# brown-palm/goal-force

Measured on AMD Instinct MI355X. Metric: frames_per_sec (81-frame video / (50-step denoise loop + VAE decode), Wan2.2-I2V-A14B 832x480x81f), higher is better.
Workload: dtype bf16

## Files before the change

### goal_force_amd/csrc/gf_cross_fold.hip

```cpp
#include "gf_common.h"

namespace {

constexpr int CF_HD = 128;
constexpr int CF_MAXK = 64;
constexpr int CF_THREADS = 256;
constexpr int CF_QB = 128;

__device__ __forceinline__ void cf_mfma32(f32x16& acc, const bf16x8& a, const bf16x8& b) {
    acc = __builtin_amdgcn_mfma_f32_32x32x16_bf16(a, b, acc, 0, 0, 0);
}

__global__ __launch_bounds__(CF_THREADS) void cross_probs_kernel(const u16* __restrict__ q, const u16* __restrict__ k, u16* __restrict__ pout,
                                                                 int q_len, int n_keys, int n_pad, int heads, long q_stride, long k_stride,
                                                                 long p_stride, float c, float last_key_bias) {
    __shared__ __attribute__((aligned(16))) char lds[CF_MAXK * 256];
    const int tid = threadIdx.x;
    const int lane = tid & 63, wave = tid >> 6;
    const int r = lane & 31, h = lane >> 5;
    const int head = blockIdx.y;
    const int q0 = blockIdx.x * CF_QB + wave * 32;
    const int halves = n_keys > 32 ? 2 : 1;

#pragma unroll
    for (int i = 0; i < (CF_MAXK * 16) / CF_THREADS; ++i) {
        const int idx = tid + CF_THREADS * i;
        const int row = idx >> 4, ch = idx & 15;
        u16x8 v8 = {0, 0, 0, 0, 0, 0, 0, 0};
        if (row < n_keys) v8 = *reinterpret_cast<const u16x8*>(k + (long)row * k_stride + head * CF_HD + ch * 8);
        const int sk = ((row & 3) << 2) | ((row >> 2) & 3);
        *(u16x8*)(lds + row * 256 + ((ch ^ sk) << 4)) = v8;
    }

    bf16x8 qf[8];
    {
        const int qr = min(q0 + r, q_len - 1);
        const u16* qp = q + (long)qr * q_stride + head * CF_HD + 8 * h;
#pragma unroll
        for (int kd = 0; kd < 8; ++kd) qf[kd] = *reinterpret_cast<const bf16x8*>(qp + 16 * kd);
    }
    __syncthreads();

    f32x16 sc[2];
#pragma unroll
    for (int e = 0; e < 16; ++e) {
        sc[0][e] = 0.f;
        sc[1][e] = 0.f;
    }
    const int sK = ((r & 3) << 2) | ((r >> 2) & 3);
#pragma unroll
    for (int kd = 0; kd < 8; ++kd) {
        const int off = 256 * r + 16 * ((2 * kd + h) ^ sK);
        cf_mfma32(sc[0], *(const bf16x8*)(lds + off), qf[kd]);
        if (halves == 2) cf_mfma32(sc[1], *(const bf16x8*)(lds + off + 32 * 256), qf[kd]);
    }

#pragma unroll
    for (int e = 0; e < 16; ++e) {
        const int key = 4 * h + (e & 3) + 8 * (e >> 2);
        if (key >= n_keys) sc[0][e] = -INFINITY;
        if (key + 32 >= n_keys) sc[1][e] = -INFINITY;
        if (key == n_keys - 1) sc[0][e] += last_key_bias;
        if (key + 32 == n_keys - 1) sc[1][e] += last_key_bias;
    }
    float mx = sc[0][0];
#pragma unroll
    for (int e = 1; e < 16; ++e) mx = fmaxf(mx, sc[0][e]);
#pragma unroll
    for (int e = 0; e < 16; ++e) mx = fmaxf(mx, sc[1][e]);
    mx = fmaxf(mx, __shfl_xor(mx, 32));
    const float mc = mx * c;
    float rs = 0.f;
#pragma unroll
    for (int e = 0; e < 16; ++e) {
        sc[0][e] = __builtin_amdgcn_exp2f(__builtin_fmaf(sc[0][e], c, -mc));
        sc[1][e] = __builtin_amdgcn_exp2f(__builtin_fmaf(sc[1][e], c, -mc));
        rs += sc[0][e] + sc[1][e];
    }
    const float l_tot = rs + __shfl_xor(rs, 32);
    const float inv = 1.0f / l_tot;
    float pl = 0.f;
#pragma unroll
    for (int e = 0; e < 16; ++e) {
        const int key = 4 * h + (e & 3) + 8 * (e >> 2);
        if (key == n_keys - 1) pl = sc[0][e];
        if (key + 32 == n_keys - 1) pl = sc[1][e];
    }
    pl += __shfl_xor(pl, 32);
    const float wl = pl * inv;
    const float wl_lo = wl - bf2f(f2bf(wl));

    const int qrow = q0 + r;
    if (qrow < q_len) {
        u16* prow = pout + (long)qrow * p_stride + (long)head * n_pad;
#pragma unroll
        for (int half = 0; half < 2; ++half)
#pragma unroll
            for (int g = 0; g < 4; ++g) {
                const int key = 32 * half + 8 * g + 4 * h;
                if (key < n_pad) {
                    float w4[4];
#pragma unroll
                    for (int i = 0; i < 4; ++i) w4[i] = key + i == n_keys ? wl_lo : sc[half][4 * g + i] * inv;
                    u32x2 pk;
                    pk[0] = pack2bf(w4[0], w4[1]);
                    pk[1] = pack2bf(w4[2], w4[3]);
                    *reinterpret_cast<u32x2*>(prow + key) = pk;
                }
            }
    }
}

constexpr int CFT_ROWS = 64;
__global__ __launch_bounds__(CF_THREADS) void cross_fold_table_kernel(const u16* __restrict__ v, const u16* __restrict__ w, u16* __restrict__ u,
                                                                      int n_keys, int n_pad, int n_out, long v_stride, long w_stride,
                                                                      long u_stride) {
    __shared__ __attribute__((aligned(16))) u16 vs[CF_MAXK * CF_HD];
    const int tid = threadIdx.x;
    const int head = blockIdx.y;
    for (int idx = tid; idx < n_pad * 16; idx += CF_THREADS) {
        const int row = idx >> 4, ch = idx & 15;
        u16x8 v8 = {0, 0, 0, 0, 0, 0, 0, 0};
        if (row <= n_keys) v8 = *reinterpret_cast<const u16x8*>(v + (long)min(row, n_keys - 1) * v_stride + head * CF_HD + ch * 8);
        *reinterpret_cast<u16x8*>(vs + row * CF_HD + ch * 8) = v8;
    }
    __syncthreads();
    const int n = blockIdx.x * CFT_ROWS + (tid >> 2), jg = tid & 3;
    if (n >= n_out) return;
    const int nj = n_pad >> 2;
    float acc[CF_MAXK / 4];
#pragma unroll
    for (int i = 0; i < CF_MAXK / 4; ++i) acc[i] = 0.f;
    const u16* wr = w + (long)n * w_stride + head * CF_HD;
    for (int d0 = 0; d0 < CF_HD; d0 += 8) {
        const u16x8 w8 = *reinterpret_cast<const u16x8*>(wr + d0);
        float wf[8];
#pragma unroll
        for (int e = 0; e < 8; ++e) wf[e] = bf2f(w8[e]);
#pragma unroll
        for (int i = 0; i < CF_MAXK / 4; ++i) {
            if (i < nj) {
                const u16x8 v8 = *reinterpret_cast<const u16x8*>(vs + (jg + 4 * i) * CF_HD + d0);
#pragma unroll
                for (int e = 0; e < 8; ++e) acc[i] = __builtin_fmaf(bf2f(v8[e]), wf[e], acc[i]);
            }
        }
    }
    u16* ur = u + (long)n * u_stride + (long)head * n_pad;
#pragma unroll
    for (int i = 0; i < CF_MAXK / 4; ++i) {
        const int j = jg + 4 * i;
        if (i < nj) ur[j] = j <= n_keys ? f2bf(acc[i]) : (u16)0;
    }
}

}

extern "C" GF_API int gf_cross_probs(const void* q, const void* k, void* p, int64_t q_len, int64_t n_keys, int64_t n_pad, int64_t heads,
                                     int64_t head_dim, int64_t q_stride, int64_t k_stride, int64_t p_stride, float scale,
                                     float last_key_multiplicity, void* stream) {
    GF_CHECK_ARG(q && k && p, "gf_cross_probs: null pointer");
    if (head_dim != CF_HD) {
        gf_set_error("gf_cross_probs: head_dim=%ld unsupported (kernel is built for 128)", (long)head_dim);
        return GF_ERR_UNSUPPORTED;
    }
    GF_CHECK_ARG(q_len >= 0 && q_len < (1 << 30) && heads > 0 && heads < 65536, "gf_cross_probs: bad sizes q=%ld heads=%ld", (long)q_len,
                 (long)heads);
    GF_CHECK_ARG(n_keys >= 1 && n_pad % 16 == 0 && n_pad > n_keys && n_pad <= CF_MAXK,
                 "gf_cross_probs: 1 <= n_keys=%ld < n_pad=%ld <= 64, n_pad a multiple of 16", (long)n_keys, (long)n_pad);
    GF_CHECK_ARG(q_stride % 8 == 0 && k_stride % 8 == 0 && p_stride % 4 == 0 && q_stride >= heads * CF_HD && k_stride >= heads * CF_HD &&
                     p_stride >= heads * n_pad,
                 "gf_cross_probs: strides must cover the rows (q, k: multiples of 8; p: of 4, >= heads * n_pad)");
    GF_CHECK_ARG(gf_aligned16(q) && gf_aligned16(k) && ((uintptr_t)p & 7u) == 0, "gf_cross_probs: alignment (q, k 16 bytes, p 8 bytes)");
    GF_CHECK_ARG(scale > 0.f && last_key_multiplicity >= 1.0f, "gf_cross_probs: scale > 0, multiplicity >= 1");
    if (q_len == 0) return GF_OK;
    const float c = scale * 1.4426950408889634f;
    const float bias = last_key_multiplicity != 1.0f ? log2f(last_key_multiplicity) / c : 0.f;
    const dim3 grid((unsigned)((q_len + CF_QB - 1) / CF_QB), (unsigned)heads);
    hipLaunchKernelGGL(cross_probs_kernel, grid, dim3(CF_THREADS), 0, (hipStream_t)stream, (const u16*)q, (const u16*)k, (u16*)p,
                       (int)q_len, (int)n_keys, (int)n_pad, (int)heads, (long)q_stride, (long)k_stride, (long)p_stride, c, bias);
    GF_CHECK_LAUNCH("gf_cross_probs");
    return GF_OK;
}

extern "C" GF_API int gf_cross_fold_table(const void* v, const void* w_o, void* u, int64_t n_keys, int64_t n_pad, int64_t heads,
                                          int64_t head_dim, int64_t n_out, int64_t v_stride, int64_t w_stride, int64_t u_stride,
                                          void* stream) {
    GF_CHECK_ARG(v && w_o && u, "gf_cross_fold_table: null pointer");
    if (head_dim != CF_HD) {
        gf_set_error("gf_cross_fold_table: head_dim=%ld unsupported (kernel is built for 128)", (long)head_dim);
        return GF_ERR_UNSUPPORTED;
    }
    GF_CHECK_ARG(heads > 0 && heads < 65536 && n_out > 0 && n_out < (1 << 30), "gf_cross_fold_table: bad sizes heads=%ld N=%ld", (long)heads,
                 (long)n_out);
    GF_CHECK_ARG(n_keys >= 1 && n_pad % 16 == 0 && n_pad > n_keys && n_pad <= CF_MAXK,
                 "gf_cross_fold_table: 1 <= n_keys=%ld < n_pad=%ld <= 64, n_pad a multiple of 16", (long)n_keys, (long)n_pad);
    GF_CHECK_ARG(v_stride % 8 == 0 && w_stride % 8 == 0 && v_stride >= heads * CF_HD && w_stride >= heads * CF_HD && u_stride >= heads * n_pad,
                 "gf_cross_fold_table: strides must cover the rows (v, w_o: multiples of 8; u >= heads * n_pad)");
    GF_CHECK_ARG(gf_aligned16(v) && gf_aligned16(w_o) && ((uintptr_t)u & 1u) == 0, "gf_cross_fold_table: alignment");
    const dim3 grid((unsigned)((n_out + CFT_ROWS - 1) / CFT_ROWS), (unsigned)heads);
    hipLaunchKernelGGL(cross_fold_table_kernel, grid, dim3(CF_THREADS), 0, (hipStream_t)stream, (const u16*)v, (const u16*)w_o, (u16*)u,
                       (int)n_keys, (int)n_pad, (int)n_out, (long)v_stride, (long)w_stride, (long)u_stride);
    GF_CHECK_LAUNCH("gf_cross_fold_table");
    return GF_OK;
}
```

### goal_force_amd/csrc/gf_gemm.hip

```cpp
#include "gf_mfma_frame.h"
#include <cstdlib>


namespace {

constexpr int BM = 256, BN = 256, BK = 64;
constexpr int GEMM_THREADS = 512;
constexpr int TILE_BYTES = BM * BK * 2;
constexpr int STAGE_BYTES = 2 * TILE_BYTES;
constexpr int GEMM_LDS = 2 * STAGE_BYTES;
constexpr int GROUP_M = 8;

struct ConvGeom {
    const u16* src;
    const u16* cache;
    const u16* zero;
    int H, W, C, Ho, Wo, kt, ks, mode, t_stride, t_off, taps;
    int hist_front;
    int c64;
    long frame;
    float inv_c, inv_ks2;
};

struct GemmArgs {
    const u16* A;
    const u16* W;
    const u16* bias;
    u16* C;
    const u16* R;
    const u16* gate;
    const float* row_scale;
    int M, N, K;
    long lda, ldw, ldc, ldr;
    long sA = 0, sW = 0, sC = 0;
    int tiles_m, tiles_n;
    unsigned long long* rsv0 = nullptr;
    ConvGeom cv;
    int rsv1 = 0;
    int stagger;
    int wrows;
    int stagger_rows;
    int group_m;
    int rsv2 = 0;
};

constexpr int GF_EPI_VT32 = 6;

typedef __attribute__((ext_vector_type(8))) int i32x8;

template <int EPI>
__device__ __forceinline__ float gf_epi_act(float lin) {
    if constexpr (EPI == GF_EPI_BIAS_GELU_TANH) return gelu_tanh_f(rbf(lin));
    else if constexpr (EPI == GF_EPI_BIAS_SILU) {
        const float y = rbf(lin);
        return y / (1.0f + expf(-y));
    } else return lin;
}

template <int EPI, bool FP8>
__global__ __launch_bounds__(GEMM_THREADS, 2) void gemm_kernel(const GemmArgs p) {
    static_assert(FP8, "only the fp8 form of this kernel ships (launch_gemm); bf16 with M < 512 runs gemm_ph_kernel");
    extern __shared__ __attribute__((aligned(16))) char smem[];
    GF_LDS char* lds = (GF_LDS char*)smem;

    const int tid = threadIdx.x;
    const int lane = tid & 63;
    const int wave = __builtin_amdgcn_readfirstlane(tid >> 6);

    const int v = gf_xcd_tile_order(p.tiles_m * p.tiles_n);
    const int per_group = GROUP_M * p.tiles_n;
    const int group = v / per_group;
    const int first_m = group * GROUP_M;
    const int gsz = min(p.tiles_m - first_m, GROUP_M);
    const int in_group = v - group * per_group;
    const int tile_m = first_m + in_group % gsz;
    const int tile_n = in_group / gsz;
    const int m0 = tile_m * BM, n0 = tile_n * BN;

    const int srow = lane >> 3;
    const int schunk = (lane & 7) ^ srow;
    const char* a_src[4];
    const char* b_src[4];
#pragma unroll
    for (int i = 0; i < 4; ++i) {
        const int row = (wave * 4 + i) * 8 + srow;
        const int am = min(m0 + row, p.M - 1);
        const int bn = min(n0 + row, p.N - 1);
        a_src[i] = (const char*)p.A + (long)am * p.lda + schunk * 16;
        b_src[i] = (const char*)p.W + (long)bn * p.ldw + schunk * 16;
    }
    auto stage = [&](int buf, int kt) {
        GF_LDS char* sa = lds + buf * STAGE_BYTES + wave * 4096;
        GF_LDS char* sb = sa + TILE_BYTES;
        const int koff = kt * 128;
#pragma unroll
        for (int i = 0; i < 4; ++i) {
            glds16(a_src[i] + koff, sa + i * 1024);
            glds16(b_src[i] + koff, sb + i * 1024);
        }
    };

    const int wm = wave >> 2, wn = wave & 3;
    const int frow = lane & 15;
    const int fq = lane >> 4;
    const int sw = frow & 7;
    const int a_base = (wm * 128 + frow) * 128;
    const int b_base = TILE_BYTES + (wn * 64 + frow) * 128;

    f32x4 acc[8][4];
#pragma unroll
    for (int i = 0; i < 8; ++i)
#pragma unroll
        for (int j = 0; j < 4; ++j) acc[i][j] = f32x4{0.f, 0.f, 0.f, 0.f};

    const int nk = p.K / 128;
    stage(0, 0);
    for (int kt = 0; kt < nk; ++kt) {
        asm volatile("s_waitcnt vmcnt(0)" ::: "memory");
        __syncthreads();
        if (kt + 1 < nk) stage((kt + 1) & 1, kt + 1);
        GF_LDS char* sbuf = lds + (kt & 1) * STAGE_BYTES;
        const int c0 = ((2 * fq) ^ sw) << 4, c1 = ((2 * fq + 1) ^ sw) << 4;
        i32x8 bfr[4];
#pragma unroll
        for (int j = 0; j < 4; ++j) {
            const u32x4 lo = *(GF_LDS u32x4*)(sbuf + b_base + j * 2048 + c0);
            const u32x4 hi = *(GF_LDS u32x4*)(sbuf + b_base + j * 2048 + c1);
            bfr[j] = i32x8{(int)lo[0], (int)lo[1], (int)lo[2], (int)lo[3], (int)hi[0], (int)hi[1], (int)hi[2], (int)hi[3]};
        }
#pragma unroll
        for (int i = 0; i < 8; ++i) {
            const u32x4 lo = *(GF_LDS u32x4*)(sbuf + a_base + i * 2048 + c0);
            const u32x4 hi = *(GF_LDS u32x4*)(sbuf + a_base + i * 2048 + c1);
            const i32x8 af = i32x8{(int)lo[0], (int)lo[1], (int)lo[2], (int)lo[3], (int)hi[0], (int)hi[1], (int)hi[2], (int)hi[3]};
#pragma unroll
            for (int j = 0; j < 4; ++j)
                acc[i][j] = __builtin_amdgcn_mfma_scale_f32_16x16x128_f8f6f4(bfr[j], af, acc[i][j], 0, 0, 0, 0x7F7F7F7F, 0, 0x7F7F7F7F);
        }
    }

    __syncthreads();
    GF_LDS char* ep = lds + wave * 16384;
    {
        const int nb = n0 + wn * 64 + fq * 4;
#pragma unroll
        for (int j = 0; j < 4; ++j) {
            float bv[4] = {0.f, 0.f, 0.f, 0.f};
            const int n = nb + j * 16;
            if (p.bias && n < p.N) {
                const u16x4 b4 = *reinterpret_cast<const u16x4*>(p.bias + n);
#pragma unroll
                for (int r = 0; r < 4; ++r) bv[r] = bf2f(b4[r]);
            }
#pragma unroll
            for (int i = 0; i < 8; ++i) {
                float y[4];
                const float rs = p.row_scale[min(m0 + wm * 128 + i * 16 + frow, p.M - 1)];
#pragma unroll
                for (int r = 0; r < 4; ++r) y[r] = gf_epi_act<EPI>(acc[i][j][r] * rs + bv[r]);
                u32x2 pk;
                pk[0] = pack2bf(y[0], y[1]);
                pk[1] = pack2bf(y[2], y[3]);
                const int row = i * 16 + frow;
                const int slot = (j * 4 + fq) ^ ((row & 7) << 1);
                *(GF_LDS u32x2*)(ep + row * 128 + slot * 8) = pk;
            }
        }
    }
    asm volatile("s_waitcnt lgkmcnt(0)" ::: "memory");
    {
        const int rr = lane >> 3, cc = lane & 7;
        const int n = n0 + wn * 64 + cc * 8;
        const bool n_ok = n < p.N;
        u16x8 g8;
        if (EPI == GF_EPI_BIAS_GATE_RESID && n_ok) g8 = *reinterpret_cast<const u16x8*>(p.gate + n);
#pragma unroll 4
        for (int it = 0; it < 16; ++it) {
            const int row = it * 8 + rr;
            const int m = m0 + wm * 128 + row;
            const u16x8 yv = *(GF_LDS u16x8*)(ep + row * 128 + ((cc ^ (row & 7)) << 4));
            if (m < p.M && n_ok) {
                u16x8 o = yv;
                if (EPI == GF_EPI_BIAS_GATE_RESID || EPI == GF_EPI_BIAS_RESID || EPI == GF_EPI_BIAS_MUL) {
                    const u16x8 r8 = *reinterpret_cast<const u16x8*>(p.R + (long)m * p.ldr + n);
#pragma unroll
                    for (int e = 0; e < 8; ++e) {
                        float t = bf2f(yv[e]);
                        if (EPI == GF_EPI_BIAS_GATE_RESID) t = rbf(bf2f(g8[e]) * t);
                        o[e] = (EPI == GF_EPI_BIAS_MUL) ? f2bf(t * bf2f(r8[e]))
                                                        : f2bf(bf2f(r8[e]) + t);
                    }
                }
                *reinterpret_cast<u16x8*>(p.C + (long)m * p.ldc + n) = o;
            }
        }
    }
}

template <int EPI, bool FP8, int CONV = 0, int NB = 2>
__global__ __launch_bounds__(GEMM_THREADS, 2) void gemm_ph_kernel(const GemmArgs p) {
    static_assert(!(CONV && FP8), "the implicit-GEMM convolution is bf16 only");
    static_assert(NB == 2 || ((NB == 1 || NB == 3) && !FP8), "NB = 1 and 3 are built for bf16");
    constexpr bool WIDE = NB >= 2;
    constexpr int NBH = WIDE ? 2 : 1;
    constexpr int J1 = NB == 3 ? 1 : 2;
    constexpr int BNT = NB == 3 ? 192 : NB * 128;
    constexpr int ESZ = FP8 ? 1 : 2;
    constexpr int BKE = 128 / ESZ;
    constexpr int HALF_BYTES = 128 * 128;
    extern __shared__ __attribute__((aligned(16))) char smem[];
    GF_LDS char* lds = (GF_LDS char*)smem;

    const u16* const pA = p.A + (long)blockIdx.y * p.sA;
    const u16* const pW = p.W + (long)blockIdx.y * p.sW;
    u16* const pC = p.C + (long)blockIdx.y * p.sC;
    const int tid = threadIdx.x;
    const int lane = tid & 63;
    const int wave = __builtin_amdgcn_readfirstlane(tid >> 6);
    const int wr = wave >> 2, wc = wave & 3;

    const int v = gf_xcd_tile_order(p.tiles_m * p.tiles_n);
    const int per_group = GROUP_M * p.tiles_n;
    const int group = v / per_group;
    const int first_m = group * GROUP_M;
    const int gsz = min(p.tiles_m - first_m, GROUP_M);
    const int in_group = v - group * per_group;
    const int m0 = (first_m + in_group % gsz) * BM, n0 = (in_group / gsz) * BNT;

    const int srow = lane >> 3;
    const int schunk = (lane & 7) ^ srow;
    const char* srcp[4][2];
#pragma unroll
    for (int i = 0; i < 2; ++i) {
        const int row = (wave * 2 + i) * 8 + srow;
        const long a0 = min(m0 + row, p.M - 1), a1 = min(m0 + 128 + row, p.M - 1);
        const long b0 = min(n0 + row, p.N - 1), b1 = min(n0 + 128 + row, p.N - 1);
        srcp[0][i] = (const char*)pA + (a0 * p.lda) * ESZ + schunk * 16;
        srcp[3][i] = (const char*)pA + (a1 * p.lda) * ESZ + schunk * 16;
        srcp[1][i] = (const char*)pW + (b0 * p.ldw) * ESZ + schunk * 16;
        srcp[2][i] = (const char*)pW + (b1 * p.ldw) * ESZ + schunk * 16;
    }
    const char* srcp_b1h = (const char*)pW + (min((long)(n0 + 128 + wave * 8 + srow), (long)p.N - 1) * p.ldw) * ESZ + schunk * 16;
    int cyx[2][2], cf[2][2];
    const u16* rowp[2][2];
    int rmask[2][2];
    if constexpr (CONV != 0) {
#pragma unroll
        for (int a = 0; a < 2; ++a)
#pragma unroll
            for (int i = 0; i < 2; ++i) {
                const int m = min(m0 + a * 128 + (wave * 2 + i) * 8 + srow, p.M - 1);
                const int X = m % p.cv.Wo, t = m / p.cv.Wo;
                const int Y = t % p.cv.Ho, j = t / p.cv.Ho;
                const int f0 = p.cv.t_off + j * p.cv.t_stride - (p.cv.kt - 1);
                if constexpr (CONV == 2) {
                    rowp[a][i] = p.cv.src + ((long)f0 * p.cv.frame + ((long)Y * p.cv.W + X) * p.cv.C);
                    rmask[a][i] = 16 | (Y == 0 ? 1 : 0) | (Y == p.cv.H - 1 ? 2 : 0) | (X == 0 ? 4 : 0) | (X == p.cv.W - 1 ? 8 : 0);
                } else {
                    cyx[a][i] = (Y << 16) | X;
                    cf[a][i] = f0;
                }
            }
    }
    int s_c0[2] = {0, 0}, s_dt[2] = {0, 0}, s_dy[2] = {0, 0}, s_dx[2] = {0, 0};
    if constexpr (CONV == 2) {
        if (p.cv.c64) {
#pragma unroll
            for (int a = 0; a < 2; ++a)
#pragma unroll
                for (int i = 0; i < 2; ++i) rowp[a][i] += schunk * 8;
        }
    }
    const int nk = p.K / BKE;
    auto region = [](int kind) { return kind == 0 ? 0 : (kind == 3 ? HALF_BYTES : (kind == 1 ? 2 * HALF_BYTES : 3 * HALF_BYTES)); };
    auto stage = [&](int tile, int kind) {
        GF_LDS char* dst = lds + (tile & 1) * STAGE_BYTES + region(kind) + wave * 2048;
        if constexpr (CONV != 0) {
            if (kind == 0 || kind == 3) {
                const ConvGeom& g = p.cv;
                const int a = kind == 3;
                if constexpr (CONV == 2) {
                    if (g.c64) {
                        const int hf = g.ks >> 1;
                        const long toff = (long)s_dt[a] * g.frame + (long)(((s_dy[a] - hf) * g.W + (s_dx[a] - hf)) * g.C + s_c0[a]);
                        int need = 0;
                        if (g.ks == 3) need = (s_dy[a] == 0 ? 1 : 0) | (s_dy[a] == 2 ? 2 : 0) | (s_dx[a] == 0 ? 4 : 0) | (s_dx[a] == 2 ? 8 : 0);
#pragma unroll
                        for (int i = 0; i < 2; ++i) glds16((need & rmask[a][i]) ? g.zero : rowp[a][i] + toff, dst + i * 1024);
                        s_c0[a] += 64;
                        if (s_c0[a] == g.C) {
                            s_c0[a] = 0;
                            if (++s_dx[a] == g.ks) {
                                s_dx[a] = 0;
                                if (++s_dy[a] == g.ks) {
                                    s_dy[a] = 0;
                                    ++s_dt[a];
                                }
                            }
                        }
                        return;
                    }
                }
                const int ke = tile * 64 + schunk * 8;
                const int tap = (int)(((float)ke + 0.5f) * g.inv_c);
                const int c = ke - tap * g.C;
                const int dt = (int)(((float)tap + 0.5f) * g.inv_ks2);
                const int rem = tap - dt * g.ks * g.ks;
                int dy = 0, dx = 0;
                if (g.ks == 3) {
                    dy = (rem * 11) >> 5;
                    dx = rem - 3 * dy;
                }
                const int half = g.ks >> 1;
                if constexpr (CONV == 2) {
                    const long toff = (long)dt * g.frame + (long)(((dy - half) * g.W + (dx - half)) * g.C + c);
                    int need = tap < g.taps ? 0 : 16;
                    if (g.ks == 3) need |= (dy == 0 ? 1 : 0) | (dy == 2 ? 2 : 0) | (dx == 0 ? 4 : 0) | (dx == 2 ? 8 : 0);
#pragma unroll
                    for (int i = 0; i < 2; ++i) glds16((need & rmask[a][i]) ? g.zero : rowp[a][i] + toff, dst + i * 1024);
                    return;
                }
#pragma unroll
                for (int i = 0; i < 2; ++i) {
                    const int Y = cyx[a][i] >> 16, X = cyx[a][i] & 0xffff;
                    int sy, sx;
                    bool ok;
                    if (g.mode == 2) {
                        sy = 2 * Y + dy;
                        sx = 2 * X + dx;
                        ok = sy < g.H && sx < g.W;
                    } else {
                        const int yy = Y + dy - half, xx = X + dx - half;
                        ok = yy >= 0 && yy < g.Ho && xx >= 0 && xx < g.Wo;
                        sy = g.mode == 1 ? (yy >> 1) : yy;
                        sx = g.mode == 1 ? (xx >> 1) : xx;
                    }
                    const int f = cf[a][i] + dt;
                    const u16* base = (f >= 0 || g.hist_front) ? g.src + (long)f * g.frame : g.cache + (long)(2 + f) * g.frame;
                    const u16* src = (ok && tap < g.taps) ? base + ((long)sy * g.W + sx) * g.C + c : g.zero;
                    glds16(src, dst + i * 1024);
                }
                return;
            }
        }
        const long koff = (long)tile * 128;
        if constexpr (NB == 3) {
            if (kind == 2) {
                glds16(srcp_b1h + koff, lds + (tile & 1) * STAGE_BYTES + region(2) + wave * 1024);
                return;
            }
        }
        glds16(srcp[kind][0] + koff, dst);
        glds16(srcp[kind][1] + koff, dst + 1024);
    };

    const int frow = lane & 15, fq = lane >> 4, sw = frow & 7;
    const int a_off = (wr * 64 + frow) * 128;
    const int b_off = (wc * 32 + frow) * 128;
    const int b_off1 = NB == 3 ? (wc * 16 + frow) * 128 : b_off;
    int chb[4];
    if constexpr (!FP8) {
        chb[0] = ((0 + fq) ^ sw) << 4;
        chb[1] = ((4 + fq) ^ sw) << 4;
        chb[2] = chb[3] = 0;
    } else {
        chb[0] = ((2 * fq) ^ sw) << 4;
        chb[1] = ((2 * fq + 1) ^ sw) << 4;
        chb[2] = chb[3] = 0;
    }
    typedef u32x4 frag_t[2];
    frag_t afr[4], bfr[2][2];
    auto read_a = [&](GF_LDS char* buf, int a) {
#pragma unroll
        for (int i = 0; i < 4; ++i) {
            afr[i][0] = *(GF_LDS u32x4*)(buf + region(a ? 3 : 0) + a_off + i * 2048 + chb[0]);
            afr[i][1] = *(GF_LDS u32x4*)(buf + region(a ? 3 : 0) + a_off + i * 2048 + chb[1]);
        }
    };
    auto read_b = [&](GF_LDS char* buf, int b) {
#pragma unroll
        for (int j = 0; j < 2; ++j) {
            if (b && j >= J1) continue;
            bfr[b][j][0] = *(GF_LDS u32x4*)(buf + region(b ? 2 : 1) + (b ? b_off1 : b_off) + j * 2048 + chb[0]);
            bfr[b][j][1] = *(GF_LDS u32x4*)(buf + region(b ? 2 : 1) + (b ? b_off1 : b_off) + j * 2048 + chb[1]);
        }
    };

    f32x4 acc[2][NBH][4][2];
#pragma unroll
    for (int a = 0; a < 2; ++a)
#pragma unroll
        for (int b = 0; b < NBH; ++b)
#pragma unroll
            for (int i = 0; i < 4; ++i)
#pragma unroll
                for (int j = 0; j < 2; ++j) acc[a][b][i][j] = f32x4{0.f, 0.f, 0.f, 0.f};

    auto mma = [&](int a, int b) {
        __builtin_amdgcn_s_setprio(1);
#pragma unroll
        for (int i = 0; i < 4; ++i)
#pragma unroll
            for (int j = 0; j < 2; ++j) {
                if (b && j >= J1) continue;
                if constexpr (!FP8) {
#pragma unroll
                    for (int ks = 0; ks < 2; ++ks)
                        acc[a][b][i][j] = __builtin_amdgcn_mfma_f32_16x16x32_bf16(
                            __builtin_bit_cast(bf16x8, bfr[b][j][ks]), __builtin_bit_cast(bf16x8, afr[i][ks]),
                            acc[a][b][i][j], 0, 0, 0);
                } else {
                    const i32x8 bw = i32x8{(int)bfr[b][j][0][0], (int)bfr[b][j][0][1], (int)bfr[b][j][0][2], (int)bfr[b][j][0][3],
                                           (int)bfr[b][j][1][0], (int)bfr[b][j][1][1], (int)bfr[b][j][1][2], (int)bfr[b][j][1][3]};
                    const i32x8 aw = i32x8{(int)afr[i][0][0], (int)afr[i][0][1], (int)afr[i][0][2], (int)afr[i][0][3],
                                           (int)afr[i][1][0], (int)afr[i][1][1], (int)afr[i][1][2], (int)afr[i][1][3]};
                    acc[a][b][i][j] = __builtin_amdgcn_mfma_scale_f32_16x16x128_f8f6f4(bw, aw, acc[a][b][i][j], 0, 0, 0,
                                                                                         0x7F7F7F7F, 0, 0x7F7F7F7F);
                }
            }
        __builtin_amdgcn_s_setprio(0);
    };

    const int total = (WIDE ? 4 : 3) * nk;
    if constexpr (WIDE) {
        stage(0, 0);
        stage(0, 1);
        stage(0, 2);
        stage(0, 3);
        if (nk > 1) {
            stage(1, 0);
            stage(1, 1);
            if constexpr (NB == 3) asm volatile("s_waitcnt vmcnt(7)" ::: "memory");
            else asm volatile("s_waitcnt vmcnt(8)" ::: "memory");
        } else {
            asm volatile("s_waitcnt vmcnt(0)" ::: "memory");
        }
        __builtin_amdgcn_s_barrier();
    } else {
        stage(0, 0);
        stage(0, 1);
        stage(0, 3);
        if (nk > 1) {
            stage(1, 0);
            stage(1, 1);
            asm volatile("s_waitcnt vmcnt(6)" ::: "memory");
        } else {
            asm volatile("s_waitcnt vmcnt(0)" ::: "memory");
        }
        __builtin_amdgcn_s_barrier();
    }
    if (wr == 1) __builtin_amdgcn_s_barrier();

#define GF_PHASE_END(SEQ_ISSUED)                                                  \
    if ((SEQ_ISSUED) >= total) asm volatile("s_waitcnt vmcnt(0)" ::: "memory");  \
    else if constexpr (NB == 3) asm volatile("s_waitcnt vmcnt(7)" ::: "memory"); \
    else if constexpr (NB == 2) asm volatile("s_waitcnt vmcnt(8)" ::: "memory"); \
    else asm volatile("s_waitcnt vmcnt(6)" ::: "memory");                        \
    asm volatile("s_waitcnt lgkmcnt(0)" ::: "memory");                           \
    __builtin_amdgcn_sched_barrier(0);                                           \
    __builtin_amdgcn_s_barrier();

#define GF_AFTER_MMA                       \
    __builtin_amdgcn_sched_barrier(0);     \
    __builtin_amdgcn_s_barrier();
    if constexpr (NB == 1) {
        for (int c = 0; c < nk; ++c) {
            GF_LDS char* buf = lds + (c & 1) * STAGE_BYTES;
            const int g = 3 * c;
            if (g + 5 < total) stage(c + 1, 3);
            read_b(buf, 0);
            read_a(buf, 0);
            GF_PHASE_END(g + 5)
            mma(0, 0);
            GF_AFTER_MMA
            if (g + 6 < total) {
                stage(c + 2, 0);
                stage(c + 2, 1);
            }
            read_a(buf, 1);
            GF_PHASE_END(g + 7)
            mma(1, 0);
            GF_AFTER_MMA
        }
    } else
    for (int c = 0; c < nk; ++c) {
        GF_LDS char* buf = lds + (c & 1) * STAGE_BYTES;
        const int g = 4 * c;
        if (g + 6 < total) stage(c + 1, 2);
        read_b(buf, 0);
        read_a(buf, 0);
        GF_PHASE_END(g + 6)
        mma(0, 0);
        GF_AFTER_MMA
        if (g + 7 < total) stage(c + 1, 3);
        read_b(buf, 1);
        GF_PHASE_END(g + 7)
        mma(0, 1);
        GF_AFTER_MMA
        if (g + 8 < total) stage(c + 2, 0);
        read_a(buf, 1);
        GF_PHASE_END(g + 8)
        mma(1, 1);
        GF_AFTER_MMA
        if (g + 9 < total) stage(c + 2, 1);
        GF_PHASE_END(g + 9)
        mma(1, 0);
        GF_AFTER_MMA
    }
#undef GF_AFTER_MMA
#undef GF_PHASE_END
    if (wr == 0) __builtin_amdgcn_s_barrier();

    constexpr bool HAS_R = EPI == GF_EPI_BIAS_GATE_RESID || EPI == GF_EPI_BIAS_RESID || EPI == GF_EPI_BIAS_MUL;
    u16x8 rpre[HAS_R ? 16 : 1];
    if constexpr (HAS_R) {
        const int cc = lane & 31, n = n0 + cc * 8;
        const bool n_ok = n < p.N && cc * 8 < BNT;
#pragma unroll
        for (int it = 0; it < 16; ++it) {
            const int m = m0 + wave * 32 + it * 2 + (lane >> 5);
            rpre[it] = u16x8{0, 0, 0, 0, 0, 0, 0, 0};
            if (m < p.M && n_ok) rpre[it] = *reinterpret_cast<const u16x8*>(p.R + (long)m * p.ldr + n);
        }
    }

#pragma unroll
    for (int b = 0; b < NBH; ++b)
#pragma unroll
        for (int j = 0; j < 2; ++j) {
            if (b && j >= J1) continue;
            const int ncol = (NB == 3 && b) ? 128 + wc * 16 + fq * 4 : b * 128 + wc * 32 + j * 16 + fq * 4;
            float bv[4] = {0.f, 0.f, 0.f, 0.f};
            if (p.bias && n0 + ncol < p.N) {
                const u16x4 b4 = *reinterpret_cast<const u16x4*>(p.bias + n0 + ncol);
#pragma unroll
                for (int r = 0; r < 4; ++r) bv[r] = bf2f(b4[r]);
            }
#pragma unroll
            for (int a = 0; a < 2; ++a)
#pragma unroll
                for (int i = 0; i < 4; ++i) {
                    const int row = a * 128 + wr * 64 + i * 16 + frow;
                    float rs = 1.0f;
                    if constexpr (FP8) rs = p.row_scale[min(m0 + row, p.M - 1)];
                    float y[4];
#pragma unroll
                    for (int r = 0; r < 4; ++r) {
                        y[r] = gf_epi_act<EPI>(acc[a][b][i][j][r] * rs + bv[r]);
                    }
                    u32x2 pk;
                    pk[0] = pack2bf(y[0], y[1]);
                    pk[1] = pack2bf(y[2], y[3]);
                    const int slot = (ncol >> 2) ^ ((row & 15) << 1);
                    *(GF_LDS u32x2*)(lds + row * 512 + slot * 8) = pk;
                }
        }
    __syncthreads();
    {
        const int cc = lane & 31;
        const int n = n0 + cc * 8;
        const bool n_ok = n < p.N && cc * 8 < BNT;
        u16x8 g8;
        if (EPI == GF_EPI_BIAS_GATE_RESID && n_ok) g8 = *reinterpret_cast<const u16x8*>(p.gate + n);
#pragma unroll
        for (int it = 0; it < 16; ++it) {
            const int row = wave * 32 + it * 2 + (lane >> 5);
            const int m = m0 + row;
            const u16x8 yv = *(GF_LDS u16x8*)(lds + row * 512 + ((cc ^ (row & 15)) << 4));
            if (m < p.M && n_ok) {
                u16x8 o = yv;
                if (EPI == GF_EPI_BIAS_GATE_RESID || EPI == GF_EPI_BIAS_RESID || EPI == GF_EPI_BIAS_MUL) {
                    const u16x8 r8 = rpre[HAS_R ? it : 0];
#pragma unroll
                    for (int e = 0; e < 8; ++e) {
                        float t = bf2f(yv[e]);
                        if (EPI == GF_EPI_BIAS_GATE_RESID) t = rbf(bf2f(g8[e]) * t);
                        o[e] = (EPI == GF_EPI_BIAS_MUL) ? f2bf(t * bf2f(r8[e]))
                                                        : f2bf(bf2f(r8[e]) + t);
                    }
                }
                *reinterpret_cast<u16x8*>(pC + (long)m * p.ldc + n) = o;
            }
        }
    }
}

#include "gf_gemm_a4_loop.inc"
#include "gf_gemm_a4f8_loop.inc"
constexpr int A4_THREADS = 256;

template <int EPI, bool FP8 = false>
__global__ __launch_bounds__(A4_THREADS, 1) void gemm_a4_kernel(const GemmArgs p) {
    constexpr unsigned ESZ = FP8 ? 1u : 2u;
    extern __shared__ __attribute__((aligned(16))) char smem[];
    GF_LDS char* lds = (GF_LDS char*)smem;
    const int tid = threadIdx.x;
    const int lane = tid & 63;
    const int wave = __builtin_amdgcn_readfirstlane(tid >> 6);
    const int wm = wave >> 1, wn = wave & 1;

    const int v = gf_xcd_tile_order(p.tiles_m * p.tiles_n);
    const int gm = p.group_m;
    const int per_group = gm * p.tiles_n;
    const int group = v / per_group;
    const int first_m = group * gm;
    const int gsz = min(p.tiles_m - first_m, gm);
    const int in_group = v - group * per_group;
    const int m0 = (first_m + in_group % gsz) * BM, n0 = (in_group / gsz) * BN;

    unsigned voffA = gf_a4_voff<ESZ>(lane, (unsigned)p.lda), voffB = gf_a4_voff<ESZ>(lane, (unsigned)p.ldw);
    unsigned pfA = (unsigned)lane * (unsigned)p.lda * ESZ, pfB = (unsigned)lane * (unsigned)p.ldw * ESZ;
    const unsigned long baseA = (unsigned long)((const char*)p.A + (long)m0 * p.lda * ESZ);
    const unsigned long baseB = (unsigned long)((const char*)p.W + (long)n0 * p.ldw * ESZ);
    const unsigned aLo = (unsigned)baseA, aHi = (unsigned)(baseA >> 32) & 0xffffu;
    const unsigned bLo = (unsigned)baseB, bHi = (unsigned)(baseB >> 32) & 0xffffu;
    const unsigned nrA = (unsigned)(((long)(min(p.M - m0, BM) - 1) * p.lda + p.K) * ESZ);
    const int wvalid = min(p.wrows - n0, BN);
    const unsigned nrB = wvalid > 0 ? (unsigned)(((long)(wvalid - 1) * p.ldw + p.K) * ESZ) : 0u;
    const unsigned stA = 32u * (unsigned)p.lda * ESZ, stB = 32u * (unsigned)p.ldw * ESZ;
    const unsigned soA = (unsigned)wave * 8u * (unsigned)p.lda * ESZ, soB = (unsigned)wave * 8u * (unsigned)p.ldw * ESZ;
    const unsigned ldsW = (unsigned)(unsigned long)lds + (unsigned)wave * 1024u;
    const unsigned nk = (unsigned)(p.K * (int)ESZ / 128);
    const unsigned k0 = p.stagger ? (unsigned)((p.stagger * (p.stagger_rows ? m0 / BM : n0 / BN)) % (int)nk) : 0u;
    const unsigned kb = (unsigned)p.K * ESZ;

    const int frow = lane & 15, fq = lane >> 4, sw = frow & 7;
    const unsigned lbase = (unsigned)(unsigned long)lds;
    unsigned rdA0 = lbase + (unsigned)((wm * 128 + frow) * 128 + (((0 + fq) ^ sw) << 4));
    unsigned rdA1 = lbase + (unsigned)((wm * 128 + frow) * 128 + (((4 + fq) ^ sw) << 4));
    unsigned rdB0 = lbase + (unsigned)(TILE_BYTES + (wn * 128 + frow) * 128 + (((0 + fq) ^ sw) << 4));
    unsigned rdB1 = lbase + (unsigned)(TILE_BYTES + (wn * 128 + frow) * 128 + (((4 + fq) ^ sw) << 4));

    u16x4 bpre[8];
    u16x8 gpre = {0, 0, 0, 0, 0, 0, 0, 0};
    {
        const int fq_ = lane >> 4;
#pragma unroll
        for (int j = 0; j < 8; ++j) {
            const int n = n0 + wn * 128 + j * 16 + fq_ * 4;
            bpre[j] = (EPI != GF_EPI_VT32 && p.bias && n < p.N) ? *reinterpret_cast<const u16x4*>(p.bias + n) : u16x4{0, 0, 0, 0};
        }
        const int ng = n0 + wn * 128 + (lane & 15) * 8;
        if (EPI == GF_EPI_BIAS_GATE_RESID && ng < p.N) gpre = *reinterpret_cast<const u16x8*>(p.gate + ng);
        if (EPI == GF_EPI_VT32 && p.bias) {
#pragma unroll
            for (int i = 0; i < 8; ++i) {
                const int mrow = m0 + wm * 128 + i * 16 + (lane & 15);
                if (mrow < p.M) bpre[i][0] = p.bias[mrow];
            }
        }
    }
    float rsc[FP8 ? 8 : 1];
    if constexpr (FP8 && EPI != GF_EPI_VT32) {
#pragma unroll
        for (int i = 0; i < 8; ++i) rsc[i] = p.row_scale[min(m0 + wm * 128 + i * 16 + (lane & 15), p.M - 1)];
    }
    if constexpr (FP8) {
        GF_A4F8_LOOP_ASM(voffA, voffB, rdA0, rdA1, rdB0, rdB1, aLo, aHi, nrA, bLo, bHi, nrB, soA, stA, soB, stB, ldsW, nk, k0, kb);
    } else
    {
        GF_A4_LOOP_ASM(voffA, voffB, pfA, pfB, rdA0, rdA1, rdB0, rdB1, aLo, aHi, nrA, bLo, bHi, nrB, soA, stA, soB, stB, ldsW, nk, k0, kb);
    }

    GF_LDS char* ep = lds + wave * 32768;
    constexpr bool HAS_R = EPI == GF_EPI_BIAS_GATE_RESID || EPI == GF_EPI_BIAS_RESID || EPI == GF_EPI_BIAS_MUL;
    u16x8 rres[HAS_R ? 32 : 1];
    if constexpr (HAS_R) {
        const int nr = n0 + wn * 128 + (lane & 15) * 8;
#pragma unroll
        for (int it = 0; it < 32; ++it) {
            const int mr = m0 + wm * 128 + it * 4 + (lane >> 4);
            if (mr < p.M && nr < p.N) {
                rres[it] = __builtin_nontemporal_load(reinterpret_cast<const u16x8*>(p.R + (long)mr * p.ldr + nr));
            } else {
                rres[it] = u16x8{0, 0, 0, 0, 0, 0, 0, 0};
            }
        }
    }
    f32x4 csc[(FP8 && EPI == GF_EPI_VT32) ? 8 : 1];
    if constexpr (FP8 && EPI == GF_EPI_VT32) {
#pragma unroll
        for (int j = 0; j < 8; ++j) {
            const int n = n0 + wn * 128 + j * 16 + fq * 4;
#pragma unroll
            for (int r = 0; r < 4; ++r) csc[j][r] = (n + r < p.wrows) ? p.row_scale[n + r] : 0.f;
        }
    }
    gf_static_for<0, 8>([&](auto j_c) {
        constexpr int j = decltype(j_c)::value;
        const int n = n0 + wn * 128 + j * 16 + fq * 4;
        const float bv[4] = {bf2f(bpre[j][0]), bf2f(bpre[j][1]), bf2f(bpre[j][2]), bf2f(bpre[j][3])};
        gf_static_for<0, 8>([&](auto i_c) {
            constexpr int i = decltype(i_c)::value;
            constexpr int A0 = (i * 8 + j) * 4;
            float y[4] = {gf_agpr_read<A0>(), gf_agpr_read<A0 + 1>(), gf_agpr_read<A0 + 2>(), gf_agpr_read<A0 + 3>()};
            if constexpr (FP8 && EPI != GF_EPI_VT32) {
#pragma unroll
                for (int r = 0; r < 4; ++r) y[r] = y[r] * rsc[i] + bv[r];
            }
            if constexpr (EPI == GF_EPI_VT32) {
                const float bm = bf2f(bpre[i][0]);
                if constexpr (FP8) {
#pragma unroll
                    for (int r = 0; r < 4; ++r) y[r] = (n + r < p.wrows) ? y[r] * csc[j][r] + bm : 0.f;
                } else {
#pragma unroll
                    for (int r = 0; r < 4; ++r) y[r] = (n + r < p.wrows) ? y[r] + bm : 0.f;
                }
            } else if constexpr (EPI == GF_EPI_BIAS_GELU_TANH) {
                const unsigned l01 = FP8 ? pack2bf(y[0], y[1]) : pack2bf(y[0] + bv[0], y[1] + bv[1]);
                const unsigned l23 = FP8 ? pack2bf(y[2], y[3]) : pack2bf(y[2] + bv[2], y[3] + bv[3]);
                gf_f32x2 g01 = {__uint_as_float(l01 << 16), __uint_as_float(l01 & 0xffff0000u)};
                gf_f32x2 g23 = {__uint_as_float(l23 << 16), __uint_as_float(l23 & 0xffff0000u)};
                gelu_tanh_f4(g01, g23);
                y[0] = g01[0];
                y[1] = g01[1];
                y[2] = g23[0];
                y[3] = g23[1];
            } else {
#pragma unroll
                for (int r = 0; r < 4; ++r) {
                    y[r] = gf_epi_act<EPI>(FP8 ? y[r] : y[r] + bv[r]);
                }
            }
            u32x2 pk;
            pk[0] = pack2bf(y[0], y[1]);
            pk[1] = pack2bf(y[2], y[3]);
            const int row = i * 16 + frow;
            const int slot = (j * 4 + fq) ^ ((row & 15) << 1);
            *(GF_LDS u32x2*)(ep + row * 256 + slot * 8) = pk;
        });
    });
    asm volatile("s_waitcnt lgkmcnt(0)" ::: "memory");
    {
        const int cc = lane & 15;
        const int n = n0 + wn * 128 + cc * 8;
        const bool n_ok = n < p.N;
        const u16x8 g8 = gpre;
#pragma unroll
        for (int it = 0; it < 32; ++it) {
            const int row = it * 4 + (lane >> 4);
            const int m = m0 + wm * 128 + row;
            u16x8 yv;
            if constexpr (EPI == GF_EPI_VT32) {
                const int G = cc >> 2, g = cc & 3, sw = (row & 15) << 1;
                const u16x4 lo = *(GF_LDS u16x4*)(ep + row * 256 + (((8 * G + g) ^ sw) << 3));
                const u16x4 hi = *(GF_LDS u16x4*)(ep + row * 256 + (((8 * G + 4 + g) ^ sw) << 3));
                yv = u16x8{lo[0], lo[1], lo[2], lo[3], hi[0], hi[1], hi[2], hi[3]};
            } else {
                yv = *(GF_LDS u16x8*)(ep + row * 256 + ((cc ^ (row & 15)) << 4));
            }
            if (m < p.M && n_ok) {
                u16x8 o = yv;
                if constexpr (HAS_R) {
                    const u16x8 r8 = rres[it];
#pragma unroll
                    for (int e = 0; e < 8; ++e) {
                        float t = bf2f(yv[e]);
                        if (EPI == GF_EPI_BIAS_GATE_RESID) t = rbf(bf2f(g8[e]) * t);
                        o[e] = (EPI == GF_EPI_BIAS_MUL) ? f2bf(t * bf2f(r8[e]))
                                                        : f2bf(bf2f(r8[e]) + t);
                    }
                }
                __builtin_nontemporal_store(o, reinterpret_cast<u16x8*>(p.C + (long)m * p.ldc + n));
            }
        }
    }
}

template <int EPI, bool FP8 = false>
int launch_gemm_a4(const GemmArgs& a0, hipStream_t stream) {
    GemmArgs a = a0;
    {
        const int g = gf_options().a4_group_m.load(std::memory_order_relaxed);
        a.group_m = g > 0 ? g : (a.K * (FP8 ? 1 : 2) >= 16384 ? 4 : GROUP_M);
    }
    return gf_launch_lds<gemm_a4_kernel<EPI, FP8>>("gf_gemm", GF_ATTR_MSG_BYTES, FP8 ? "gf_gemm_fp8" : "gf_gemm_bf16", dim3((unsigned)(a.tiles_m * a.tiles_n)),
                                                   dim3(A4_THREADS), GEMM_LDS, stream, a);
}

template <int EPI, bool FP8>
int launch_gemm(const GemmArgs& a, hipStream_t stream) {
    const bool use_a4 = gf_options().prefer_8wave.load(std::memory_order_relaxed) == 0;
    if constexpr (!FP8) {
        if (use_a4 && a.M >= 512 && a.K % 64 == 0 && 256L * a.lda * 2 + a.K * 2L < (1L << 31) &&
            256L * a.ldw * 2 + a.K * 2L < (1L << 31))
            return launch_gemm_a4<EPI>(a, stream);
    } else {
        if (use_a4 && a.M >= 512 && a.K % 128 == 0 && 256L * a.lda + a.K < (1L << 31) && 256L * a.ldw + a.K < (1L << 31))
            return launch_gemm_a4<EPI, true>(a, stream);
    }
    const dim3 grid((unsigned)(a.tiles_m * a.tiles_n)), block(GEMM_THREADS);
    if constexpr (FP8) return gf_launch_lds<gemm_kernel<EPI, true>>("gf_gemm", GF_ATTR_MSG_BYTES, "gf_gemm_fp8", grid, block, GEMM_LDS, stream, a);
    else return gf_launch_lds<gemm_ph_kernel<EPI, false>>("gf_gemm", GF_ATTR_MSG_BYTES, "gf_gemm_bf16", grid, block, GEMM_LDS, stream, a);
}

template <int EPI, int NB, int CONV>
int launch_conv(const GemmArgs& a, hipStream_t stream, int batch = 1) {
    return gf_launch_lds<gemm_ph_kernel<EPI, false, CONV, NB>>("gf_conv3d", GF_ATTR_MSG_BYTES, "gf_conv3d_bf16",
                                                               dim3((unsigned)(a.tiles_m * a.tiles_n), (unsigned)batch), dim3(GEMM_THREADS),
                                                               GEMM_LDS, stream, a);
}

}
__device__ __attribute__((used, visibility("default"))) u16 gf_conv_zero_page[128] = {};
namespace {

const u16* conv_zero_page() {
    static GfDeviceOnce once;
    static const u16* page[64] = {};
    int dev = 0;
    if (hipGetDevice(&dev) != hipSuccess || dev < 0 || dev >= 64) return nullptr;
    hipError_t e = gf_once_per_device(once, [dev] {
        void* z = nullptr;
        hipError_t r = hipGetSymbolAddress(&z, HIP_SYMBOL(gf_conv_zero_page));
        if (r == hipSuccess) page[dev] = (const u16*)z;
        return r;
    });
    return e == hipSuccess ? page[dev] : nullptr;
}

}

static int gemm_dispatch(bool fp8, const void* A, int64_t lda, const void* W, int64_t ldw, const float* row_scale,
                         const void* bias, void* C, int64_t ldc, int64_t M, int64_t N, int64_t K, int epilogue,
                         const void* resid, int64_t ldr, const void* gate, void* stream) {
    const char* fn = fp8 ? "gf_gemm_fp8" : "gf_gemm_bf16";
    const int bke = fp8 ? 128 : 64, lal = fp8 ? 16 : 8;
    GF_CHECK_ARG(A && W && C, "%s: null A/W/C", fn);
    GF_CHECK_ARG(M >= 0 && N > 0 && K > 0, "%s: bad sizes M=%ld N=%ld K=%ld", fn, (long)M, (long)N, (long)K);
    GF_CHECK_ARG(K % bke == 0, "%s: K=%ld must be a multiple of %d", fn, (long)K, bke);
    GF_CHECK_ARG(N % 8 == 0, "%s: N=%ld must be a multiple of 8", fn, (long)N);
    GF_CHECK_ARG(lda % lal == 0 && ldw % lal == 0 && ldc % 8 == 0 && lda >= K && ldw >= K && ldc >= N,
                 "%s: leading dimensions must be multiples of %d (A/W) / 8 (C) and cover the row", fn, lal);
    GF_CHECK_ARG(gf_aligned16(A) && gf_aligned16(W) && gf_aligned16(C) && (!bias || gf_aligned16(bias)),
                 "%s: 16-byte alignment required", fn);
    GF_CHECK_ARG(M < (1 << 30) && N < (1 << 30), "%s: M/N too large", fn);
    GF_CHECK_ARG(!fp8 || row_scale, "%s: row_scale is required", fn);
    const bool need_r = epilogue == GF_EPI_BIAS_GATE_RESID || epilogue == GF_EPI_BIAS_RESID || epilogue == GF_EPI_BIAS_MUL;
    GF_CHECK_ARG(!need_r || (resid && ldr % 8 == 0 && ldr >= N && gf_aligned16(resid)),
                 "%s: residual epilogue needs an aligned resid with ldr >= N", fn);
    GF_CHECK_ARG(epilogue != GF_EPI_BIAS_GATE_RESID || (gate && gf_aligned16(gate)),
                 "%s: gate epilogue needs an aligned gate vector", fn);
    if (M == 0) return GF_OK;
    GemmArgs a;
    a.A = (const u16*)A;
    a.W = (const u16*)W;
    a.bias = (const u16*)bias;
    a.C = (u16*)C;
    a.R = (const u16*)resid;
    a.gate = (const u16*)gate;
    a.row_scale = row_scale;
    a.M = (int)M;
    a.N = (int)N;
    a.K = (int)K;
    a.lda = lda;
    a.ldw = ldw;
    a.ldc = ldc;
    a.ldr = ldr;
    a.tiles_m = (int)((M + BM - 1) / BM);
    a.tiles_n = (int)((N + BN - 1) / BN);
    a.stagger = gf_options().a4_stagger.load(std::memory_order_relaxed);
    a.wrows = (int)N;
    a.stagger_rows = 0;
    hipStream_t s = (hipStream_t)stream;
#define GF_GEMM_CASE(E) case E: return fp8 ? launch_gemm<E, true>(a, s) : launch_gemm<E, false>(a, s);
    switch (epilogue) {
        GF_GEMM_CASE(GF_EPI_BIAS)
        GF_GEMM_CASE(GF_EPI_BIAS_GELU_TANH)
        GF_GEMM_CASE(GF_EPI_BIAS_GATE_RESID)
        GF_GEMM_CASE(GF_EPI_BIAS_RESID)
        GF_GEMM_CASE(GF_EPI_BIAS_SILU)
        GF_GEMM_CASE(GF_EPI_BIAS_MUL)
        default:
            gf_set_error("%s: unknown epilogue %d", fn, epilogue);
            return GF_ERR_INVALID_ARG;
    }
#undef GF_GEMM_CASE
}

extern "C" GF_API int gf_gemm_bf16(const void* A, int64_t lda, const void* W, int64_t ldw, const void* bias, void* C,
                                   int64_t ldc, int64_t M, int64_t N, int64_t K, int epilogue, const void* resid,
                                   int64_t ldr, const void* gate, void* stream) {
    return gemm_dispatch(false, A, lda, W, ldw, nullptr, bias, C, ldc, M, N, K, epilogue, resid, ldr, gate, stream);
}

extern "C" GF_API int gf_gemm_fp8(const void* A8, int64_t lda, const void* W8, int64_t ldw, const float* row_scale,
                                  const void* bias, void* C, int64_t ldc, int64_t M, int64_t N, int64_t K, int epilogue,
                                  const void* resid, int64_t ldr, const void* gate, void* stream) {
    return gemm_dispatch(true, A8, lda, W8, ldw, row_scale, bias, C, ldc, M, N, K, epilogue, resid, ldr, gate, stream);
}

extern "C" GF_API int gf_linear_vt32(const void* x, int64_t ldx, const void* w, int64_t ldw, const void* bias, void* vt,
                                     int64_t kv_len, int64_t kv_pad, int64_t N, int64_t K, void* stream) {
    GF_CHECK_ARG(x && w && vt, "gf_linear_vt32: null x/w/vt");
    GF_CHECK_ARG(kv_len > 0 && kv_pad >= kv_len && kv_pad % 64 == 0 && kv_pad - kv_len < 64, "gf_linear_vt32: kv_pad = kv_len rounded up to 64");
    GF_CHECK_ARG(N >= 512 && N % 128 == 0 && K > 0 && K % 64 == 0, "gf_linear_vt32: N=%ld (>= 512, multiple of 128), K=%ld (multiple of 64)", (long)N, (long)K);
    GF_CHECK_ARG(ldx % 8 == 0 && ldw % 8 == 0 && ldx >= K && ldw >= K, "gf_linear_vt32: leading dimensions must be multiples of 8 covering K");
    GF_CHECK_ARG(gf_aligned16(x) && gf_aligned16(w) && gf_aligned16(vt) && (!bias || ((uintptr_t)bias & 1u) == 0), "gf_linear_vt32: alignment");
    GF_CHECK_ARG(N * kv_pad < (1LL << 31) && 256L * ldx * 2 + K * 2L < (1L << 31) && 256L * ldw * 2 + K * 2L < (1L << 31),
                 "gf_linear_vt32: operand too large for 32-bit staging offsets");
    GemmArgs a;
    a.A = (const u16*)w;
    a.W = (const u16*)x;
    a.bias = (const u16*)bias;
    a.C = (u16*)vt;
    a.R = nullptr;
    a.gate = nullptr;
    a.row_scale = nullptr;
    a.M = (int)N;
    a.N = (int)kv_pad;
    a.K = (int)K;
    a.lda = ldw;
    a.ldw = ldx;
    a.ldc = kv_pad;
    a.ldr = 0;
    a.tiles_m = (int)((N + BM - 1) / BM);
    a.tiles_n = (int)((kv_pad + BN - 1) / BN);
    a.stagger = gf_options().a4_stagger.load(std::memory_order_relaxed);
    a.wrows = (int)kv_len;
    a.stagger_rows = 1;
    return launch_gemm_a4<GF_EPI_VT32>(a, (hipStream_t)stream);
}

extern "C" GF_API int gf_linear_vt32_fp8(const void* x8, int64_t ldx, const float* x_scale, const void* w8, int64_t ldw, const void* bias,
                                         void* vt, int64_t kv_len, int64_t kv_pad, int64_t N, int64_t K, void* stream) {
    GF_CHECK_ARG(x8 && w8 && vt && x_scale, "gf_linear_vt32_fp8: null x8/w8/vt/x_scale");
    GF_CHECK_ARG(kv_len > 0 && kv_pad >= kv_len && kv_pad % 64 == 0 && kv_pad - kv_len < 64, "gf_linear_vt32_fp8: kv_pad = kv_len rounded up to 64");
    GF_CHECK_ARG(N >= 512 && N % 128 == 0 && K > 0 && K % 128 == 0, "gf_linear_vt32_fp8: N=%ld (>= 512, multiple of 128), K=%ld (multiple of 128)", (long)N, (long)K);
    GF_CHECK_ARG(ldx % 16 == 0 && ldw % 16 == 0 && ldx >= K && ldw >= K, "gf_linear_vt32_fp8: leading dimensions must be multiples of 16 covering K");
    GF_CHECK_ARG(gf_aligned16(x8) && gf_aligned16(w8) && gf_aligned16(vt) && (!bias || ((uintptr_t)bias & 1u) == 0), "gf_linear_vt32_fp8: alignment");
    GF_CHECK_ARG(N * kv_pad < (1LL << 31) && 256L * ldx + K < (1L << 31) && 256L * ldw + K < (1L << 31),
                 "gf_linear_vt32_fp8: operand too large for 32-bit staging offsets");
    GemmArgs a;
    a.A = (const u16*)w8;
    a.W = (const u16*)x8;
    a.bias = (const u16*)bias;
    a.C = (u16*)vt;
    a.R = nullptr;
    a.gate = nullptr;
    a.row_scale = x_scale;
    a.M = (int)N;
    a.N = (int)kv_pad;
    a.K = (int)K;
    a.lda = ldw;
    a.ldw = ldx;
    a.ldc = kv_pad;
    a.ldr = 0;
    a.tiles_m = (int)((N + BM - 1) / BM);
    a.tiles_n = (int)((kv_pad + BN - 1) / BN);
    a.stagger = gf_options().a4_stagger.load(std::memory_order_relaxed);
    a.wrows = (int)kv_len;
    a.stagger_rows = 1;
    return launch_gemm_a4<GF_EPI_VT32, true>(a, (hipStream_t)stream);
}

extern "C" GF_API int gf_gemm_bf16_batched(const void* A, int64_t lda, int64_t strideA, const void* W, int64_t ldw, int64_t strideW,
                                           void* C, int64_t ldc, int64_t strideC, int64_t M, int64_t N, int64_t K, int64_t batch,
                                           void* stream) {
    GF_CHECK_ARG(A && W && C, "gf_gemm_bf16_batched: null A/W/C");
    GF_CHECK_ARG(M > 0 && N > 0 && K > 0 && batch > 0 && batch < 65536, "gf_gemm_bf16_batched: bad sizes");
    GF_CHECK_ARG(K % 64 == 0 && N % 8 == 0, "gf_gemm_bf16_batched: K=%ld must be a multiple of 64 and N=%ld of 8", (long)K, (long)N);
    GF_CHECK_ARG(lda >= K && ldw >= K && ldc >= N && lda % 8 == 0 && ldw % 8 == 0 && ldc % 8 == 0 && strideA % 8 == 0 && strideW % 8 == 0 &&
                     strideC % 8 == 0 && strideA >= 0 && strideW >= 0 && strideC >= 0,
                 "gf_gemm_bf16_batched: leading dimensions / strides must be multiples of 8 elements covering K / N");
    GF_CHECK_ARG(gf_aligned16(A) && gf_aligned16(W) && gf_aligned16(C), "gf_gemm_bf16_batched: 16-byte alignment required");
    GF_CHECK_ARG(M < (1L << 30) && N < (1L << 30), "gf_gemm_bf16_batched: M / N too large");
    GemmArgs a;
    a.A = (const u16*)A;
    a.W = (const u16*)W;
    a.bias = nullptr;
    a.C = (u16*)C;
    a.R = nullptr;
    a.gate = nullptr;
    a.row_scale = nullptr;
    a.M = (int)M;
    a.N = (int)N;
    a.K = (int)K;
    a.lda = lda;
    a.ldw = ldw;
    a.ldc = ldc;
    a.ldr = 0;
    a.sA = strideA;
    a.sW = strideW;
    a.sC = strideC;
    const bool narrow = N <= 128;
    a.tiles_m = (int)((M + BM - 1) / BM);
    a.tiles_n = narrow ? (int)((N + 127) / 128) : (int)((N + BN - 1) / BN);
    a.stagger = 0;
    a.wrows = (int)N;
    a.stagger_rows = 0;
    a.group_m = 0;
    a.cv = ConvGeom{};
    return narrow ? launch_conv<GF_EPI_BIAS, 1, 0>(a, (hipStream_t)stream, (int)batch) : launch_conv<GF_EPI_BIAS, 2, 0>(a, (hipStream_t)stream, (int)batch);
}

extern "C" GF_API int gf_conv3d_bf16(const void* src, const void* cache, const void* Wm, int64_t ldw, const void* bias,
                                     void* out, int64_t ldc, int64_t T_in, int64_t T_out, int64_t H, int64_t W, int64_t C,
                                     int kt, int ks, int mode, int t_stride, int t_off, int64_t N, int64_t K, int epilogue,
                                     const void* resid, int64_t ldr, void* stream) {
    GF_CHECK_ARG(src && Wm && out, "gf_conv3d_bf16: null src/W/out");
    GF_CHECK_ARG(T_in > 0 && T_out >= 0 && H > 0 && W > 0 && H < 32768 && W < 32768, "gf_conv3d_bf16: bad frame size");
    GF_CHECK_ARG(C > 0 && C % 8 == 0 && C <= 512, "gf_conv3d_bf16: C=%ld must be a multiple of 8 and <= 512", (long)C);
    GF_CHECK_ARG((kt == 1 || kt == 3) && (ks == 1 || ks == 3), "gf_conv3d_bf16: kt/ks must be 1 or 3");
    GF_CHECK_ARG(mode >= 0 && mode <= 2 && (mode == 0 || ks == 3), "gf_conv3d_bf16: bad mode");
    GF_CHECK_ARG(mode != 2 || (H % 2 == 0 && W % 2 == 0), "gf_conv3d_bf16: stride-2 mode needs even H, W");
    GF_CHECK_ARG(t_stride >= 1 && t_off >= 0 && (T_out == 0 || t_off + (T_out - 1) * t_stride < T_in),
                 "gf_conv3d_bf16: output frames reach past the input");
    const long taps = (long)kt * ks * ks;
    GF_CHECK_ARG(K % 64 == 0 && K >= taps * C && K < 65536 && ldw >= K && ldw % 8 == 0,
                 "gf_conv3d_bf16: K=%ld must be a multiple of 64 covering %ld taps x %ld channels", (long)K, taps, (long)C);
    GF_CHECK_ARG(N > 0 && N % 8 == 0 && ldc >= N && ldc % 8 == 0, "gf_conv3d_bf16: N / ldc must be multiples of 8");
    GF_CHECK_ARG(gf_aligned16(src) && gf_aligned16(Wm) && gf_aligned16(out) && (!cache || gf_aligned16(cache)) &&
                     (!bias || gf_aligned16(bias)), "gf_conv3d_bf16: 16-byte alignment required");
    GF_CHECK_ARG(epilogue == GF_EPI_BIAS || epilogue == GF_EPI_BIAS_RESID, "gf_conv3d_bf16: epilogue must be BIAS or BIAS_RESID");
    GF_CHECK_ARG(epilogue != GF_EPI_BIAS_RESID || (resid && ldr % 8 == 0 && ldr >= N && gf_aligned16(resid)),
                 "gf_conv3d_bf16: residual epilogue needs an aligned resid with ldr >= N");
    const long Ho = mode == 1 ? 2 * H : (mode == 2 ? H / 2 : H), Wo = mode == 1 ? 2 * W : (mode == 2 ? W / 2 : W);
    const long M = T_out * Ho * Wo;
    GF_CHECK_ARG(M < (1L << 30), "gf_conv3d_bf16: too many output pixels");
    if (M == 0) return GF_OK;
    GemmArgs a;
    a.A = nullptr;
    a.W = (const u16*)Wm;
    a.bias = (const u16*)bias;
    a.C = (u16*)out;
    a.R = (const u16*)resid;
    a.gate = nullptr;
    a.row_scale = nullptr;
    a.M = (int)M;
    a.N = (int)N;
    a.K = (int)K;
    a.lda = 0;
    a.ldw = ldw;
    a.ldc = ldc;
    a.ldr = ldr;
    const int force_nb = gf_options().conv_nb.load(std::memory_order_relaxed);
    const bool narrow = force_nb ? force_nb == 1 : N <= 128;
    const bool w192 = !narrow && !force_nb && ((N + 191) / 192) * 192 < ((N + BN - 1) / BN) * BN;
    a.tiles_m = (int)((M + BM - 1) / BM);
    a.tiles_n = narrow ? (int)((N + 127) / 128) : (w192 ? (int)((N + 191) / 192) : (int)((N + BN - 1) / BN));
    a.stagger = 0;
    a.wrows = (int)N;
    a.stagger_rows = 0;
    a.cv.src = (const u16*)src;
    a.cv.cache = (const u16*)cache;
    a.cv.zero = conv_zero_page();
    if (!a.cv.zero) {
        gf_set_error("gf_conv3d_bf16: could not allocate the zero page");
        return GF_ERR_LAUNCH;
    }
    a.cv.H = (int)H;
    a.cv.W = (int)W;
    a.cv.C = (int)C;
    a.cv.Ho = (int)Ho;
    a.cv.Wo = (int)Wo;
    a.cv.kt = kt;
    a.cv.ks = ks;
    a.cv.mode = mode;
    a.cv.t_stride = t_stride;
    a.cv.t_off = t_off;
    a.cv.taps = (int)taps;
    a.cv.frame = (long)H * W * C;
    a.cv.inv_c = 1.0f / (float)C;
    a.cv.inv_ks2 = 1.0f / (float)(ks * ks);
    hipStream_t s = (hipStream_t)stream;
    a.cv.hist_front = (kt == 3 && !cache) ? 1 : 0;
    a.cv.c64 = (C % 64 == 0 && K == taps * C && (ks == 1 || ks == 3)) ? 1 : 0;
    if (kt == 3 && ks == 3 && mode == 0 && !cache && t_stride == 1 && C == 96 && (N == 96 || N <= 16) && ldc == N &&
        (epilogue == GF_EPI_BIAS || ldr == N) && gf_options().conv_direct.load(std::memory_order_relaxed)) {
        const u16* walk = (const u16*)src + (long)(t_off - 2) * H * W * C;
        const int rc = gf_conv3d_direct_c96(walk, Wm, ldw, bias, out, T_out, H, W, N, epilogue, resid, a.cv.zero, stream);
        if (rc != GF_ERR_UNSUPPORTED) return rc;
    }
    if (kt == 1 && ks == 3 && mode == 1 && t_stride == 1 && C == 192 && N == 96 && ldc == N && epilogue == GF_EPI_BIAS && (H % 4) == 0 &&
        (W % 16) == 0 && gf_options().conv_direct.load(std::memory_order_relaxed)) {
        const u16* src0 = (const u16*)src + (long)t_off * H * W * C;
        const int rc = gf_conv2d_up_direct_c192(src0, Wm, ldw, bias, out, T_out, H, W, a.cv.zero, stream);
        if (rc != GF_ERR_UNSUPPORTED) return rc;
    }
    const int force_g = gf_options().conv_gather.load(std::memory_order_relaxed);
    const bool fast = force_g != 1 && mode == 0 && (kt == 1 || !cache);
#define GF_CONV_CASE(E, NBV, CV) return launch_conv<E, NBV, CV>(a, s)
    if (fast) {
        if (narrow) { if (epilogue == GF_EPI_BIAS) GF_CONV_CASE(GF_EPI_BIAS, 1, 2); else GF_CONV_CASE(GF_EPI_BIAS_RESID, 1, 2); }
        if (w192) { if (epilogue == GF_EPI_BIAS) GF_CONV_CASE(GF_EPI_BIAS, 3, 2); else GF_CONV_CASE(GF_EPI_BIAS_RESID, 3, 2); }
        if (epilogue == GF_EPI_BIAS) GF_CONV_CASE(GF_EPI_BIAS, 2, 2); else GF_CONV_CASE(GF_EPI_BIAS_RESID, 2, 2);
    }
    if (narrow) { if (epilogue == GF_EPI_BIAS) GF_CONV_CASE(GF_EPI_BIAS, 1, 1); else GF_CONV_CASE(GF_EPI_BIAS_RESID, 1, 1); }
    if (w192) { if (epilogue == GF_EPI_BIAS) GF_CONV_CASE(GF_EPI_BIAS, 3, 1); else GF_CONV_CASE(GF_EPI_BIAS_RESID, 3, 1); }
    if (epilogue == GF_EPI_BIAS) GF_CONV_CASE(GF_EPI_BIAS, 2, 1); else GF_CONV_CASE(GF_EPI_BIAS_RESID, 2, 1);
#undef GF_CONV_CASE
}
```

### goal_force_amd/csrc/gf_rowops.hip

```cpp
#include "gf_common.h"

namespace {

constexpr int ROW_THREADS = 128;
constexpr int ROW_NCH = 8;

__global__ __launch_bounds__(ROW_THREADS) void layernorm_modulate_kernel(
    const u16* __restrict__ x, u16* __restrict__ out, const u16* __restrict__ weight,
    const u16* __restrict__ bias, const u16* __restrict__ scale1p, const u16* __restrict__ shift,
    int dim, long x_stride, long out_stride, float eps) {
    __shared__ float red[ROW_THREADS / 64];
    const long row = blockIdx.x;
    const int tid = threadIdx.x;
    const int nchunks = dim >> 3;
    const u16* xr = x + row * x_stride;
    u16x8 v[ROW_NCH];
    float s = 0.f;
#pragma unroll
    for (int i = 0; i < ROW_NCH; ++i) {
        const int c = tid + i * ROW_THREADS;
        if (c < nchunks) {
            v[i] = *reinterpret_cast<const u16x8*>(xr + (c << 3));
#pragma unroll
            for (int j = 0; j < 8; ++j) s += bf2f(v[i][j]);
// ... 309 lines not shown
                sn = *reinterpret_cast<const f32x4*>(sin_tab + row * half + p0);
            }
#pragma unroll
            for (int p = 0; p < 4; ++p) {
                const float a = y[2 * p], b = y[2 * p + 1];
                o[2 * p] = f2bf(__builtin_fmaf(a, cs[p], -(b * sn[p])));
                o[2 * p + 1] = f2bf(__builtin_fmaf(a, sn[p], b * cs[p]));
            }
        } else {
#pragma unroll
            for (int j = 0; j < 8; ++j) o[j] = f2bf(y[j]);
        }
        *reinterpret_cast<u16x8*>(xr + i * 512) = o;
    }
}

__global__ __launch_bounds__(ROW_THREADS) void quant_fp8_rowscale_kernel(const u16* __restrict__ x,
                                                                         unsigned char* __restrict__ out,
                                                                         float* __restrict__ scale, int dim,
                                                                         long x_stride, long out_stride) {
    __shared__ float red[ROW_THREADS / 64];
    const long row = blockIdx.x;
    const int tid = threadIdx.x;
    const int nchunks = dim >> 3;
    const u16* xr = x + row * x_stride;
    constexpr int NCH = 14;
    u16x8 v[NCH];
    float mx = 0.f;
#pragma unroll
    for (int i = 0; i < NCH; ++i) {
        const int c = tid + i * ROW_THREADS;
        if (c < nchunks) {
            v[i] = *reinterpret_cast<const u16x8*>(xr + (c << 3));
#pragma unroll
            for (int j = 0; j < 8; ++j) mx = fmaxf(mx, fabsf(bf2f(v[i][j])));
        }
    }
#pragma unroll
    for (int o = 32; o > 0; o >>= 1) mx = fmaxf(mx, __shfl_xor(mx, o));
    if ((tid & 63) == 0) red[tid >> 6] = mx;
    __syncthreads();
    mx = fmaxf(red[0], red[1]);
    const float sc = fmaxf(rbf(mx / 448.0f), 1.0f);
    if (tid == 0) scale[row] = sc;
    const float den = sc + 1e-8f;
    unsigned char* orow = out + row * out_stride;
#pragma unroll
    for (int i = 0; i < NCH; ++i) {
        const int c = tid + i * ROW_THREADS;
        if (c < nchunks) {
            float f[8];
#pragma unroll
            for (int j = 0; j < 8; ++j) f[j] = bf2f(v[i][j]) / den;
            unsigned w0 = 0, w1 = 0;
            w0 = __builtin_amdgcn_cvt_pk_fp8_f32(f[0], f[1], w0, false);
            w0 = __builtin_amdgcn_cvt_pk_fp8_f32(f[2], f[3], w0, true);
            w1 = __builtin_amdgcn_cvt_pk_fp8_f32(f[4], f[5], w1, false);
            w1 = __builtin_amdgcn_cvt_pk_fp8_f32(f[6], f[7], w1, true);
            *reinterpret_cast<u32x2*>(orow + (c << 3)) = u32x2{w0, w1};
        }
    }
}

template <int NCH>
__global__ __launch_bounds__(64 * WROWS) void layernorm_modulate_fp8_wave_kernel(
    const u16* __restrict__ x, unsigned char* __restrict__ out8, float* __restrict__ scale, const u16* __restrict__ weight,
    const u16* __restrict__ bias, const u16* __restrict__ scale1p, const u16* __restrict__ shift, long rows, long x_stride,
    long out_stride, float eps) {
    constexpr int DIM = NCH * 512;
    const long row = (long)blockIdx.x * WROWS + (threadIdx.x >> 6);
    if (row >= rows) return;
    const int lane = threadIdx.x & 63;
    const u16* xr = x + row * x_stride + lane * 8;
    u16x8 v[NCH];
    float s = 0.f;
#pragma unroll
    for (int i = 0; i < NCH; ++i) {
        v[i] = *reinterpret_cast<const u16x8*>(xr + i * 512);
#pragma unroll
        for (int j = 0; j < 8; ++j) s += bf2f(v[i][j]);
    }
    const float mean = wave_sum(s) / (float)DIM;
    float q = 0.f;
#pragma unroll
    for (int i = 0; i < NCH; ++i)
#pragma unroll
        for (int j = 0; j < 8; ++j) {
            const float d = bf2f(v[i][j]) - mean;
            q = __builtin_fmaf(d, d, q);
        }
    const float rstd = 1.0f / sqrtf(__builtin_fmaf(wave_sum(q), 1.0f / DIM, eps));
    float mx = 0.f;
#pragma unroll
    for (int i = 0; i < NCH; ++i) {
        const int c0 = i * 512 + lane * 8;
        u16x8 w8, b8, sc8, sh8;
        if (weight) w8 = *reinterpret_cast<const u16x8*>(weight + c0);
        if (bias) b8 = *reinterpret_cast<const u16x8*>(bias + c0);
        if (scale1p) sc8 = *reinterpret_cast<const u16x8*>(scale1p + c0);
        if (shift) sh8 = *reinterpret_cast<const u16x8*>(shift + c0);
#pragma unroll
        for (int j = 0; j < 8; ++j) {
            float y = (bf2f(v[i][j]) - mean) * rstd;
            if (weight) y = y * bf2f(w8[j]);
            if (bias) y = y + bf2f(b8[j]);
            y = rbf(y);
            if (scale1p) y = rbf(y * bf2f(sc8[j]));
            if (shift) y = rbf(y + bf2f(sh8[j]));
            v[i][j] = f2bf(y);
            mx = fmaxf(mx, fabsf(y));
        }
    }
#pragma unroll
    for (int o = 32; o > 0; o >>= 1) mx = fmaxf(mx, __shfl_xor(mx, o));
    const float sc = fmaxf(rbf(mx / 448.0f), 1.0f);
    if (lane == 0) scale[row] = sc;
    const float den = sc + 1e-8f;
    const bool unit = den == 1.0f;
    unsigned char* orow = out8 + row * out_stride + lane * 8;
#pragma unroll
    for (int i = 0; i < NCH; ++i) {
        float f[8];
#pragma unroll
        for (int j = 0; j < 8; ++j) f[j] = unit ? bf2f(v[i][j]) : bf2f(v[i][j]) / den;
        unsigned w0 = 0, w1 = 0;
        w0 = __builtin_amdgcn_cvt_pk_fp8_f32(f[0], f[1], w0, false);
        w0 = __builtin_amdgcn_cvt_pk_fp8_f32(f[2], f[3], w0, true);
        w1 = __builtin_amdgcn_cvt_pk_fp8_f32(f[4], f[5], w1, false);
        w1 = __builtin_amdgcn_cvt_pk_fp8_f32(f[6], f[7], w1, true);
        *reinterpret_cast<u32x2*>(orow + i * 512) = u32x2{w0, w1};
    }
}

__global__ __launch_bounds__(256) void cast_fp8_kernel(const u16* __restrict__ x, unsigned char* __restrict__ out, long n8) {
    const long stride = (long)gridDim.x * 256;
    for (long i = (long)blockIdx.x * 256 + threadIdx.x; i < n8; i += stride) {
        const u16x8 v = reinterpret_cast<const u16x8*>(x)[i];
        unsigned w[2] = {0, 0};
        w[0] = __builtin_amdgcn_cvt_pk_fp8_f32(bf2f(v[0]), bf2f(v[1]), w[0], false);
        w[0] = __builtin_amdgcn_cvt_pk_fp8_f32(bf2f(v[2]), bf2f(v[3]), w[0], true);
        w[1] = __builtin_amdgcn_cvt_pk_fp8_f32(bf2f(v[4]), bf2f(v[5]), w[1], false);
        w[1] = __builtin_amdgcn_cvt_pk_fp8_f32(bf2f(v[6]), bf2f(v[7]), w[1], true);
#pragma unroll
        for (int j = 0; j < 8; ++j)
            if ((v[j] & 0x7fffu) > 0x43E8u) {
                const int sh = (j & 3) * 8;
                w[j >> 2] = (w[j >> 2] & ~(0xffu << sh)) | ((((unsigned)v[j] >> 8 & 0x80u) | 0x7fu) << sh);
            }
        reinterpret_cast<u32x2*>(out)[i] = u32x2{w[0], w[1]};
    }
}

}

extern "C" GF_API int gf_quant_fp8_rowscale(const void* x, void* out8, float* scale, int64_t rows, int64_t dim,
                                            int64_t x_stride, int64_t out_stride, void* stream) {
    GF_CHECK_ARG(x && out8 && scale && rows >= 0, "gf_quant_fp8_rowscale: null pointer");
    GF_CHECK_ARG(dim > 0 && dim % 8 == 0 && dim <= ROW_THREADS * 14 * 8, "gf_quant_fp8_rowscale: dim=%ld must be a multiple of 8 and <= %d",
                 (long)dim, ROW_THREADS * 14 * 8);
    GF_CHECK_ARG(x_stride % 8 == 0 && out_stride % 8 == 0 && gf_aligned16(x) && (((uintptr_t)out8) & 7u) == 0,
                 "gf_quant_fp8_rowscale: alignment");
    if (rows == 0) return GF_OK;
    hipLaunchKernelGGL(quant_fp8_rowscale_kernel, dim3((unsigned)rows), dim3(ROW_THREADS), 0, (hipStream_t)stream,
                       (const u16*)x, (unsigned char*)out8, scale, (int)dim, (long)x_stride, (long)out_stride);
    GF_CHECK_LAUNCH("gf_quant_fp8_rowscale");
    return GF_OK;
}

extern "C" GF_API int gf_cast_fp8(const void* x, void* out8, int64_t n, void* stream) {
    GF_CHECK_ARG(x && out8 && n >= 0 && n % 8 == 0, "gf_cast_fp8: n must be a multiple of 8");
    GF_CHECK_ARG(gf_aligned16(x) && (((uintptr_t)out8) & 7u) == 0, "gf_cast_fp8: alignment");
    if (n == 0) return GF_OK;
    long blocks = (n / 8 + 255) / 256;
    if (blocks > 4096) blocks = 4096;
    hipLaunchKernelGGL(cast_fp8_kernel, dim3((unsigned)blocks), dim3(256), 0, (hipStream_t)stream, (const u16*)x,
                       (unsigned char*)out8, (long)(n / 8));
    GF_CHECK_LAUNCH("gf_cast_fp8");
    return GF_OK;
}

extern "C" GF_API int gf_layernorm_modulate(const void* x, void* out, const void* weight, const void* bias,
                                     const void* scale1p, const void* shift, int64_t rows, int64_t dim,
                                     int64_t x_stride, int64_t out_stride, float eps, void* stream) {
    GF_CHECK_ARG(x && out, "gf_layernorm_modulate: null x/out");
    GF_CHECK_ARG(rows >= 0 && dim > 0 && dim % 8 == 0 && dim <= ROW_THREADS * ROW_NCH * 8,
                 "gf_layernorm_modulate: dim=%ld must be a multiple of 8 and <= %d", (long)dim,
                 ROW_THREADS * ROW_NCH * 8);
    GF_CHECK_ARG(x_stride % 8 == 0 && out_stride % 8 == 0 && gf_aligned16(x) && gf_aligned16(out),
                 "gf_layernorm_modulate: rows must be 16-byte aligned");
    GF_CHECK_ARG((!weight || gf_aligned16(weight)) && (!bias || gf_aligned16(bias)) &&
                     (!scale1p || gf_aligned16(scale1p)) && (!shift || gf_aligned16(shift)),
                 "gf_layernorm_modulate: vectors must be 16-byte aligned");
    if (rows == 0) return GF_OK;
    {
        const int mode = (!weight && !bias && !scale1p && !shift) ? 0 : (weight && bias && !scale1p && !shift) ? 1
                         : (!weight && !bias && scale1p && shift) ? 2 : -1;
        const void* av = mode == 1 ? weight : scale1p;
        const void* bv = mode == 1 ? bias : shift;
        const dim3 grid_((unsigned)((rows + WROWS - 1) / WROWS)), block_(64 * WROWS);
#define GF_LN2(NCH, M)                                                                                                   \
    if (dim == NCH * 512 && mode == M) {                                                                                 \
        hipLaunchKernelGGL((layernorm_wave2_kernel<NCH, M, false>), grid_, block_, 0, (hipStream_t)stream, (const u16*)x, out,     \
                           (float*)nullptr, (const u16*)av, (const u16*)bv, (long)rows, (long)x_stride, (long)out_stride, eps);     \
        GF_CHECK_LAUNCH("gf_layernorm_modulate");                                                                        \
        return GF_OK;                                                                                                    \
    }
        GF_LN2(10, 0) GF_LN2(10, 1) GF_LN2(10, 2) GF_LN2(8, 0) GF_LN2(8, 1) GF_LN2(8, 2) GF_LN2(3, 0) GF_LN2(3, 1) GF_LN2(3, 2)
#undef GF_LN2
    }
#define GF_LN_WAVE(NCH)                                                                                                  \
    if (dim == NCH * 512) {                                                                                              \
        hipLaunchKernelGGL(layernorm_modulate_wave_kernel<NCH>, dim3((unsigned)((rows + WROWS - 1) / WROWS)),            \
                           dim3(64 * WROWS), 0, (hipStream_t)stream, (const u16*)x, (u16*)out, (const u16*)weight,       \
                           (const u16*)bias, (const u16*)scale1p, (const u16*)shift, (long)rows, (long)x_stride,        \
                           (long)out_stride, eps);                                                                       \
        GF_CHECK_LAUNCH("gf_layernorm_modulate");                                                                        \
        return GF_OK;                                                                                                    \
    }
    GF_LN_WAVE(10) GF_LN_WAVE(8) GF_LN_WAVE(3)
#undef GF_LN_WAVE
    hipLaunchKernelGGL(layernorm_modulate_kernel, dim3((unsigned)rows), dim3(ROW_THREADS), 0,
                       (hipStream_t)stream, (const u16*)x, (u16*)out, (const u16*)weight, (const u16*)bias,
                       (const u16*)scale1p, (const u16*)shift, (int)dim, (long)x_stride, (long)out_stride, eps);
    GF_CHECK_LAUNCH("gf_layernorm_modulate");
    return GF_OK;
}

extern "C" GF_API int gf_layernorm_modulate_fp8(const void* x, void* out8, float* scale, const void* weight, const void* bias,
                                                const void* scale1p, const void* shift, int64_t rows, int64_t dim,
                                                int64_t x_stride, int64_t out_stride, float eps, void* stream) {
    GF_CHECK_ARG(x && out8 && scale, "gf_layernorm_modulate_fp8: null x/out8/scale");
    GF_CHECK_ARG(rows >= 0 && (dim == 5120 || dim == 4096 || dim == 1536),
                 "gf_layernorm_modulate_fp8: dim=%ld is not one of the wave-per-row widths (5120, 4096, 1536); use "
                 "gf_layernorm_modulate + gf_quant_fp8_rowscale", (long)dim);
    GF_CHECK_ARG(x_stride % 8 == 0 && out_stride % 8 == 0 && gf_aligned16(x) && (((uintptr_t)out8) & 7u) == 0,
                 "gf_layernorm_modulate_fp8: rows must be 16-byte (x) / 8-byte (out8) aligned");
    GF_CHECK_ARG((!weight || gf_aligned16(weight)) && (!bias || gf_aligned16(bias)) &&
                     (!scale1p || gf_aligned16(scale1p)) && (!shift || gf_aligned16(shift)),
                 "gf_layernorm_modulate_fp8: vectors must be 16-byte aligned");
    if (rows == 0) return GF_OK;
    {
        const int mode = (!weight && !bias && !scale1p && !shift) ? 0 : (weight && bias && !scale1p && !shift) ? 1
                         : (!weight && !bias && scale1p && shift) ? 2 : -1;
        const void* av = mode == 1 ? weight : scale1p;
        const void* bv = mode == 1 ? bias : shift;
        const dim3 grid_((unsigned)((rows + WROWS - 1) / WROWS)), block_(64 * WROWS);
#define GF_LN2(NCH, M)                                                                                                   \
    if (dim == NCH * 512 && mode == M) {                                                                                 \
        hipLaunchKernelGGL((layernorm_wave2_kernel<NCH, M, true>), grid_, block_, 0, (hipStream_t)stream, (const u16*)x, out8,     \
                           scale, (const u16*)av, (const u16*)bv, (long)rows, (long)x_stride, (long)out_stride, eps);   \
        GF_CHECK_LAUNCH("gf_layernorm_modulate_fp8");                                                                    \
        return GF_OK;                                                                                                    \
    }
        GF_LN2(10, 0) GF_LN2(10, 1) GF_LN2(10, 2) GF_LN2(8, 0) GF_LN2(8, 1) GF_LN2(8, 2) GF_LN2(3, 0) GF_LN2(3, 1) GF_LN2(3, 2)
#undef GF_LN2
    }
#define GF_LN8_WAVE(NCH)                                                                                                 \
    if (dim == NCH * 512) {                                                                                              \
        hipLaunchKernelGGL(layernorm_modulate_fp8_wave_kernel<NCH>, dim3((unsigned)((rows + WROWS - 1) / WROWS)),        \
                           dim3(64 * WROWS), 0, (hipStream_t)stream, (const u16*)x, (unsigned char*)out8, scale,          \
                           (const u16*)weight, (const u16*)bias, (const u16*)scale1p, (const u16*)shift, (long)rows,     \
                           (long)x_stride, (long)out_stride, eps);                                                       \
    }
    GF_LN8_WAVE(10) GF_LN8_WAVE(8) GF_LN8_WAVE(3)
#undef GF_LN8_WAVE
    GF_CHECK_LAUNCH("gf_layernorm_modulate_fp8");
    return GF_OK;
}

extern "C" GF_API int gf_rmsnorm_rope(void* x, const void* weight, const float* cos_tab, const float* sin_tab,
                               int64_t rows, int64_t dim, int64_t head_dim, int64_t x_stride, float eps,
                               void* stream) {
    GF_CHECK_ARG(x && weight, "gf_rmsnorm_rope: null x/weight");
    GF_CHECK_ARG(rows >= 0 && dim > 0 && dim % 8 == 0 && dim <= ROW_THREADS * ROW_NCH * 8,
                 "gf_rmsnorm_rope: dim=%ld must be a multiple of 8 and <= %d", (long)dim,
                 ROW_THREADS * ROW_NCH * 8);
    GF_CHECK_ARG((cos_tab == nullptr) == (sin_tab == nullptr), "gf_rmsnorm_rope: cos/sin must both be set or both NULL");
    GF_CHECK_ARG(head_dim > 0 && head_dim % 8 == 0 && dim % head_dim == 0,
                 "gf_rmsnorm_rope: head_dim=%ld must be a multiple of 8 dividing dim", (long)head_dim);
    GF_CHECK_ARG(x_stride % 8 == 0 && gf_aligned16(x) && gf_aligned16(weight) &&
                     (!cos_tab || (gf_aligned16(cos_tab) && gf_aligned16(sin_tab))),
                 "gf_rmsnorm_rope: 16-byte alignment required");
    if (rows == 0) return GF_OK;
#define GF_RMS_WAVE_ROPE(NCH, ROPE)                                                                                      \
    if (rope_ == ROPE)                                                                                                   \
        hipLaunchKernelGGL((rmsnorm_rope_wave_kernel<NCH, ROPE>), grid_, block_, 0, (hipStream_t)stream, (u16*)x,        \
                           (const u16*)weight, cos_tab, sin_tab, (long)rows, (int)head_dim, (long)x_stride, eps);
#define GF_RMS_WAVE(NCH)                                                                                                 \
    if (dim == NCH * 512) {                                                                                              \
        const dim3 grid_((unsigned)((rows + WROWS - 1) / WROWS)), block_(64 * WROWS);                                     \
        const int rope_ = !cos_tab ? 0 : (512 % head_dim == 0 ? 1 : 2);                                                  \
        GF_RMS_WAVE_ROPE(NCH, 0) GF_RMS_WAVE_ROPE(NCH, 1) GF_RMS_WAVE_ROPE(NCH, 2)                                        \
        GF_CHECK_LAUNCH("gf_rmsnorm_rope");                                                                              \
        return GF_OK;                                                                                                    \
    }
    GF_RMS_WAVE(10) GF_RMS_WAVE(8) GF_RMS_WAVE(3)
#undef GF_RMS_WAVE
#undef GF_RMS_WAVE_ROPE
    hipLaunchKernelGGL(rmsnorm_rope_kernel, dim3((unsigned)rows), dim3(ROW_THREADS), 0, (hipStream_t)stream,
                       (u16*)x, (const u16*)weight, cos_tab, sin_tab, (int)dim, (int)head_dim, (long)x_stride, eps);
    GF_CHECK_LAUNCH("gf_rmsnorm_rope");
    return GF_OK;
}
```

### goal_force_amd/dit.py

```python
from __future__ import annotations

import math
from typing import Optional, Tuple

import torch
import torch.nn as nn

from . import ops
from ._lib import GoalForceError


def precompute_freqs_cis(dim: int, end: int = 1024, theta: float = 10000.0):
    freqs = 1.0 / (theta ** (torch.arange(0, dim, 2)[: (dim // 2)].double() / dim))
    freqs = torch.outer(torch.arange(end), freqs)
    return torch.polar(torch.ones_like(freqs), freqs)


def precompute_freqs_cis_3d(dim: int, end: int = 1024, theta: float = 10000.0):
    return (precompute_freqs_cis(dim - 2 * (dim // 3), end, theta),
            precompute_freqs_cis(dim // 3, end, theta),
            precompute_freqs_cis(dim // 3, end, theta))


class RopeTable:
# ... 69 lines not shown
def rope_apply(x: torch.Tensor, freqs, num_heads: int):
    rope = _as_rope(freqs, x.device)
    hd = x.shape[-1] // num_heads
    return torch.stack([ops.rope_apply(x[b].contiguous(), rope.cos, rope.sin, hd) for b in range(x.shape[0])])


_CACHE_EPOCH = [0]


def invalidate_caches():
    _CACHE_EPOCH[0] += 1


def param_key(*tensors):
    return (_CACHE_EPOCH[0],) + tuple((id(t), str(t.device), t.data_ptr(), None if t.is_inference() else t._version) for t in tensors)


class QuantizedInput:

    def __init__(self, x2=None, x8=None, scale=None):
        self.x8, self.scale = ops.quant_fp8_rowscale(x2) if x2 is not None else (x8, scale)

    @classmethod
    def layernorm(cls, x2, **kw):
        return cls(None, *ops.layernorm_modulate_fp8(x2, **kw))

    @property
    def shape(self):
        return self.x8.shape

    @property
    def is_cuda(self):
        return self.x8.is_cuda


def linear(x2, lin: nn.Linear, epilogue=ops.EPI_BIAS, resid=None, gate=None, out=None):
    w8 = getattr(lin, "_gf_w8", None)
    if w8 is None:
        return ops.gemm(x2, lin.weight, lin.bias, epilogue=epilogue, resid=resid, gate=gate, out=out)
    if lin._gf_w8_key != param_key(lin.weight):
        w8 = lin._gf_w8 = ops.cast_fp8(lin.weight.detach().contiguous())
        lin._gf_w8_key = param_key(lin.weight)
    q = x2 if isinstance(x2, QuantizedInput) else QuantizedInput(x2)
    return ops.gemm_fp8(q.x8, q.scale, w8, lin.bias, epilogue=epilogue, resid=resid, gate=gate, out=out)


def enable_fp8(module: nn.Module, enabled=True):
    for blk in module.modules():
        if isinstance(blk, DiTBlock):
            for lin in blk.modules():
                if isinstance(lin, nn.Linear):
                    lin._gf_w8 = ops.cast_fp8(lin.weight.detach().contiguous()) if enabled else None
                    lin._gf_w8_key = param_key(lin.weight) if enabled else None
    return module



def enable_sage_attention(module: nn.Module, enabled=True):
    for blk in module.modules():
        if isinstance(blk, DiTBlock):
            blk.self_attn._gf_sage = bool(enabled)
    return module


def enable_sparse_attention(module: nn.Module, pattern, dense_blocks: int = 0):
    if pattern is not None and not callable(pattern):
        raise GoalForceError(f"enable_sparse_attention: expected a callable grid -> ops.BlockMap (or None), got {type(pattern).__name__}")
    if int(dense_blocks) != dense_blocks or dense_blocks < 0:
        raise GoalForceError(f"enable_sparse_attention: expected dense_blocks >= 0, got {dense_blocks!r}")
    in_stack = set()
    for m in module.modules():
        if isinstance(getattr(m, "blocks", None), nn.ModuleList):
            for i, blk in enumerate(m.blocks):
                if isinstance(blk, DiTBlock):
                    blk.self_attn._gf_sparse = pattern if i >= dense_blocks else None
                    in_stack.add(id(blk))
    for blk in module.modules():
        if isinstance(blk, DiTBlock) and id(blk) not in in_stack:
            blk.self_attn._gf_sparse = pattern
    return module


def sageattn(q, k, v, tensor_layout="HND", is_causal=False, sm_scale=None, return_lse=False, **kw):
    if is_causal:
        raise GoalForceError("sageattn: is_causal=True is not supported (the Wan DiT attention is non-causal)")
    if return_lse:
        raise GoalForceError("sageattn: return_lse=True is not supported")
    if tensor_layout not in ("HND", "NHD"):
        raise GoalForceError(f"sageattn: tensor_layout {tensor_layout!r} (HND or NHD)")
    if q.dim() != 4 or k.dim() != 4 or v.dim() != 4:
        raise GoalForceError("sageattn: q, k, v must be 4-D")
    if q.shape[-1] != 128 or k.shape[-1] != 128 or v.shape[-1] != 128:
        raise GoalForceError(f"sageattn: head_dim {q.shape[-1]} is not supported (the kernel is built for 128)")
    if tensor_layout == "HND":
        q, k, v = (t.transpose(1, 2) for t in (q, k, v))
    B, sq, n, _ = q.shape
    if k.shape[0] != B or v.shape != k.shape or k.shape[2] != n:
        raise GoalForceError("sageattn: q / k / v batch, head or key counts differ")
    out = torch.empty((B, sq, n, 128), dtype=torch.bfloat16, device=q.device)
    for b in range(B):
        q2, k2, v2 = (t[b].reshape(t.shape[1], n * 128) for t in (q, k, v))
        ops.sage_attn(q2, k2, v2, n, scale=sm_scale, out=out[b].view(sq, n * 128))
    return out.transpose(1, 2) if tensor_layout == "HND" else out


def pad_run(ctx2: torch.Tensor) -> int:
    L = ctx2.shape[0]
    if L < 2:
        return max(L - 1, 0)
    differs = (ctx2[1:] != ctx2[:-1]).any(dim=1)
    idx = torch.nonzero(differs)
    return int(idx[-1]) + 1 if idx.numel() else 0


def _tokens2d(x: torch.Tensor) -> torch.Tensor:
    if x.dim() == 3:
        if x.shape[0] != 1:
            raise GoalForceError("hot-path modules take batch 1 ([1,S,D]); loop over the batch")
        return x[0]
    return x


class RMSNorm(nn.Module):

    def __init__(self, dim, eps=1e-5):
        super().__init__()
        self.eps = eps
        self.weight = nn.Parameter(torch.ones(dim))

    def forward(self, x):
        y = x.clone()
        ops.rmsnorm_rope(_tokens2d(y), self.weight, None, None, head_dim=8, eps=self.eps)
        return y


class SelfAttention(nn.Module):

    def __init__(self, dim: int, num_heads: int, eps: float = 1e-6):
        super().__init__()
        self.dim, self.num_heads, self.head_dim = dim, num_heads, dim // num_heads
        self.q, self.k, self.v, self.o = (nn.Linear(dim, dim) for _ in range(4))
        self.norm_q, self.norm_k = RMSNorm(dim, eps=eps), RMSNorm(dim, eps=eps)

    def attend(self, x2: torch.Tensor, rope: RopeTable, sp=None, keep=None, dense=False) -> torch.Tensor:
        fp8 = getattr(self.q, "_gf_w8", None) is not None
        sage = getattr(self, "_gf_sage", False)
        if sage and keep is not None:
            raise GoalForceError("training through a block with enable_sage_attention is refused (the sage backend has no backward): "
                                 "call enable_sage_attention(module, False) first")
        attn = ops.sage_attn if sage else ops.flash_attn
        pattern = getattr(self, "_gf_sparse", None)
        if pattern is not None and not dense:
            if sage:
                raise GoalForceError("sparse attention with enable_sage_attention is refused (the sage kernel takes no block map): switch one off")
            if keep is not None:
                raise GoalForceError("training through a block with enable_sparse_attention is refused (there is no sparse backward): "
                                     "call enable_sparse_attention(module, None) first")
            if sp is not None:
                raise GoalForceError("sparse attention under sequence parallelism is refused (the head-parallel exchange takes no block map)")
            grid = getattr(rope, "grid", None)
            if grid is None:
                raise GoalForceError("sparse attention needs the token grid: expected a RopeTable built by WanModel.rope_table "
                                     "(RopeTable.from_grid), got rotary phases without one")
            if x2.shape[0] != grid[0] * grid[1] * grid[2]:
                raise GoalForceError(f"sparse attention: expected {grid[0] * grid[1] * grid[2]} tokens for the grid {grid}, got {x2.shape[0]}")
            if x2.shape[0] < ops.VT_MIN_KV:
                raise GoalForceError(f"sparse attention: expected at least {ops.VT_MIN_KV} tokens (ops.VT_MIN_KV, where the self-attention "
                                     f"runs on kernel 3), got {x2.shape[0]}")
            block_map = pattern(grid)
            if not isinstance(block_map, ops.BlockMap):
                raise GoalForceError(f"sparse attention: expected the pattern to return an ops.BlockMap, got {type(block_map).__name__}")
            block_map = block_map.to(rope.cos.device)

            def attn(q, k, v, num_heads, vt=None, scale=None):
                return ops.flash_attn_sparse(q, k, v, num_heads, block_map, vt=vt, scale=scale)
        xin = (x2 if isinstance(x2, QuantizedInput) else QuantizedInput(x2)) if fp8 else x2
        q_cos, q_sin, attn_scale = rope.cos, rope.sin, None
        if ops._OPT["attn_q_prescale"]:
            (q_cos, q_sin), attn_scale = rope.scaled(Q_PRESCALE(self.head_dim)), math.log(2.0)
        if sp is not None and keep is None:
            k = linear(xin, self.k)
            ops.rmsnorm_rope(k, self.norm_k.weight, rope.cos, rope.sin, self.head_dim, self.norm_k.eps)
            hk = sp.heads_start(k, self.num_heads)
            hv = sp.heads_start(linear(xin, self.v), self.num_heads)
            q = linear(xin, self.q)
            ops.rmsnorm_rope(q, self.norm_q.weight, q_cos, q_sin, self.head_dim, self.norm_q.eps)
            hq = sp.heads_start(q, self.num_heads)
            return sp.attention_started(hq, hk, hv, self.num_heads, tuple(q.shape), scale=attn_scale, backend="sage" if sage else "flash")
        q, k = linear(xin, self.q), linear(xin, self.k)
        if keep is not None and keep.get("wide"):
            keep["qp"], keep["kp"] = q, k
            q, k = q.clone(), k.clone()
        ops.rmsnorm_rope(q, self.norm_q.weight, q_cos, q_sin, self.head_dim, self.norm_q.eps)
        ops.rmsnorm_rope(k, self.norm_k.weight, rope.cos, rope.sin, self.head_dim, self.norm_k.eps)
        if sp is None and keep is None and not fp8 and x2.is_cuda and self.v.weight.shape[0] >= 512 \
                and ops.vt32_ok(x2.shape[0], self.num_heads, self.head_dim):
            return attn(q, k, None, self.num_heads, vt=ops.linear_vt32(x2, self.v.weight, self.v.bias), scale=attn_scale)
        if sp is None and keep is None and fp8 and xin.is_cuda and self.v.weight.shape[0] >= 512 and self.v.weight.shape[1] % 128 == 0 \
                and ops.vt32_ok(xin.shape[0], self.num_heads, self.head_dim):
            if self.v._gf_w8_key != param_key(self.v.weight):
                self.v._gf_w8 = ops.cast_fp8(self.v.weight.detach().contiguous())
                self.v._gf_w8_key = param_key(self.v.weight)
            return attn(q, k, None, self.num_heads, vt=ops.linear_vt32_fp8(xin.x8, xin.scale, self.v._gf_w8, self.v.bias), scale=attn_scale)
        v = linear(xin, self.v)
        if sp is not None:
            return sp.attention(q, k, v, self.num_heads, scale=attn_scale, backend="sage" if sage else "flash")
        if keep is not None:
            keep["attn"], keep["lse"] = ops.flash_attn_lse(q, k, v, self.num_heads, scale=attn_scale)
            if keep.get("wide"):
                keep["v"] = v
            return keep["attn"]
        return attn(q, k, v, self.num_heads, scale=attn_scale)

    def forward(self, x, freqs):
        x2 = _tokens2d(x)
        a = self.attend(x2, _as_rope(freqs, x.device))
        return linear(a, self.o).view(x.shape)


class CrossAttention(nn.Module):

    def __init__(self, dim: int, num_heads: int, eps: float = 1e-6, has_image_input: bool = False):
        super().__init__()
        if has_image_input:
            raise NotImplementedError("has_image_input=True (CLIP image tokens) is outside the Goal-Force path")
        self.dim, self.num_heads, self.head_dim = dim, num_heads, dim // num_heads
        self.q, self.k, self.v, self.o = (nn.Linear(dim, dim) for _ in range(4))
        self.norm_q, self.norm_k = RMSNorm(dim, eps=eps), RMSNorm(dim, eps=eps)
        self.has_image_input = False

    def context_kv(self, ctx2: torch.Tensor, fold: bool = True, pad_n: Optional[int] = None):
        m = 1
        if fold and ctx2.is_cuda and ops._OPT["fold_pad_keys"]:
            n = pad_run(ctx2) if pad_n is None else pad_n
            if ctx2.shape[0] - n >= 2 and n + 1 < ops.VT_MIN_KV:
                m = ctx2.shape[0] - n
                ctx2 = ctx2[: n + 1]
        cin = QuantizedInput(ctx2) if getattr(self.k, "_gf_w8", None) is not None else ctx2
        k, v = linear(cin, self.k), linear(cin, self.v)
        ops.rmsnorm_rope(k, self.norm_k.weight, None, None, self.head_dim, self.norm_k.eps)
        return k, v, m

    def attend(self, x2, kv):
        q = linear(x2, self.q)
        ops.rmsnorm_rope(q, self.norm_q.weight, None, None, self.head_dim, self.norm_q.eps)
        return ops.flash_attn(q, kv[0], kv[1], self.num_heads, last_key_mult=kv[2] if len(kv) > 2 else 1)

    FOLD_K_MAX = 2560

    def fold_ok(self, kv) -> bool:
        if not ops._OPT["fold_cross_o"] or torch.is_grad_enabled() or len(kv) < 3 or kv[2] == 1 or self.head_dim != 128:
            return False
        if getattr(self.o, "_gf_w8", None) is not None:
            return False
        n = kv[0].shape[0]
        k = self.num_heads * self.fold_pad(n)
        return n <= ops.CROSS_FOLD_MAX_KEYS and k <= self.FOLD_K_MAX and k % 64 == 0

    @staticmethod
    def fold_pad(n_keys: int) -> int:
        return -(-(n_keys + 1) // 16) * 16

    def fold_table(self, kv):
        return ops.cross_fold_table(kv[1], self.o.weight, self.num_heads, self.fold_pad(kv[0].shape[0]))

    def attend_probs(self, x2, kv):
        q = linear(x2, self.q)
        ops.rmsnorm_rope(q, self.norm_q.weight, None, None, self.head_dim, self.norm_q.eps)
        return ops.cross_probs(q, kv[0], self.num_heads, self.fold_pad(kv[0].shape[0]), last_key_mult=kv[2])

    def forward(self, x: torch.Tensor, y: torch.Tensor):
        x2 = _tokens2d(x)
        a = self.attend(x2, self.context_kv(_tokens2d(y)))
        return linear(a, self.o).view(x.shape)


class GateModule(nn.Module):

    def forward(self, x, gate, residual):
        if x.shape != residual.shape:
            raise GoalForceError("GateModule: x and residual must have the same shape")
        d = x.shape[-1]
        g = gate.reshape(-1, d)
        if x.dim() == 3 and g.shape[0] == x.shape[0] and x.shape[0] > 1:
            return torch.stack([ops.gate_residual(x[b], g[b].contiguous(), residual[b]) for b in range(x.shape[0])])
        if g.shape[0] != 1:
            raise GoalForceError("GateModule: gate must be [B or 1, 1, D] (per-token gates are outside the Goal-Force path)")
        return ops.gate_residual(x, g[0].contiguous(), residual)


class DiTBlock(nn.Module):

    def __init__(self, has_image_input: bool, dim: int, num_heads: int, ffn_dim: int, eps: float = 1e-6):
        super().__init__()
        self.dim, self.num_heads, self.ffn_dim, self.eps = dim, num_heads, ffn_dim, eps
        self.self_attn = SelfAttention(dim, num_heads, eps)
        self.cross_attn = CrossAttention(dim, num_heads, eps, has_image_input=has_image_input)
        self.norm1 = nn.LayerNorm(dim, eps=eps, elementwise_affine=False)
        self.norm2 = nn.LayerNorm(dim, eps=eps, elementwise_affine=False)
        self.norm3 = nn.LayerNorm(dim, eps=eps)
        self.ffn = nn.Sequential(nn.Linear(dim, ffn_dim), nn.GELU(approximate="tanh"), nn.Linear(ffn_dim, dim))
        self.modulation = nn.Parameter(torch.randn(1, 6, dim) / dim ** 0.5)
        self.gate = GateModule()

    def forward(self, x, context, t_mod, freqs, context_kv=None, out=None, sp=None, keep=None, self_attn_memo=None,
                fold_pad_keys=True, pad_n=None, dense_attn=False):
        if t_mod.dim() == 4:
            raise NotImplementedError("per-token t_mod (seperated_timestep) is outside the Goal-Force path")
        x2 = _tokens2d(x)
        rope = _as_rope(freqs, x.device)
        mod = ops.modulation(self.modulation, t_mod.contiguous(), onep_mask=0b010010)
        fp8 = getattr(self.ffn[0], "_gf_w8", None) is not None
        if self_attn_memo is not None and "x" in self_attn_memo:
            x_new = self_attn_memo.pop("x")
            ev = self_attn_memo.pop("ev", None)
            if ev is not None:
                torch.cuda.current_stream(x_new.device).wait_event(ev)
                x_new.record_stream(torch.cuda.current_stream(x_new.device))
            if out is not None:
                x_new = out.copy_(x_new)
            h = None if fp8 else torch.empty_like(x2)
        else:
            if fp8:
                h = QuantizedInput.layernorm(x2, scale1p=mod[1], shift=mod[0], eps=self.eps)
            else:
                h = ops.layernorm_modulate(x2, scale1p=mod[1], shift=mod[0], eps=self.eps)
            a = self.self_attn.attend(h, rope, sp, keep, dense=dense_attn)
            x_new = out if out is not None else torch.empty_like(x2)
            linear(a, self.self_attn.o, epilogue=ops.EPI_BIAS_GATE_RESID, resid=x2, gate=mod[2], out=x_new)
            if keep is not None and keep.get("wide"):
                keep["x1"] = x_new.clone()
            if self_attn_memo is not None:
                self_attn_memo["x"] = x_new.clone()
                if x_new.is_cuda:
                    self_attn_memo["ev"] = torch.cuda.Event()
                    self_attn_memo["ev"].record(torch.cuda.current_stream(x_new.device))
        if fp8:
            h = QuantizedInput.layernorm(x_new, weight=self.norm3.weight, bias=self.norm3.bias, eps=self.eps)
        else:
            ops.layernorm_modulate(x_new, weight=self.norm3.weight, bias=self.norm3.bias, eps=self.eps, out=h)
        if context_kv is None:
            context_kv = self.cross_attn.context_kv(_tokens2d(context), fold=fold_pad_keys and keep is None, pad_n=pad_n)
        ca = self.cross_attn
        if keep is None and not fp8 and ca.fold_ok(context_kv):
            u = context_kv[3] if len(context_kv) > 3 else ca.fold_table(context_kv)
            ops.gemm(ca.attend_probs(h, context_kv), u, ca.o.bias, epilogue=ops.EPI_BIAS_RESID, resid=x_new, out=x_new)
        else:
            a = ca.attend(h, context_kv)
            linear(a, ca.o, epilogue=ops.EPI_BIAS_RESID, resid=x_new, out=x_new)
        if keep is not None and keep.get("wide"):
            keep["x2b"] = x_new.clone()
        if fp8:
            h = QuantizedInput.layernorm(x_new, scale1p=mod[4], shift=mod[3], eps=self.eps)
        else:
            ops.layernorm_modulate(x_new, scale1p=mod[4], shift=mod[3], eps=self.eps, out=h)
        f1 = linear(h, self.ffn[0], epilogue=ops.EPI_BIAS_GELU_TANH)
        linear(f1, self.ffn[2], epilogue=ops.EPI_BIAS_GATE_RESID, resid=x_new, gate=mod[5], out=x_new)
        return x_new.view(x.shape)


class Head(nn.Module):

    def __init__(self, dim: int, out_dim: int, patch_size: Tuple[int, int, int], eps: float):
        super().__init__()
        self.dim, self.patch_size, self.eps = dim, patch_size, eps
        self.norm = nn.LayerNorm(dim, eps=eps, elementwise_affine=False)
        self.head = nn.Linear(dim, out_dim * math.prod(patch_size))
        self.modulation = nn.Parameter(torch.randn(1, 2, dim) / dim ** 0.5)

    def forward(self, x, t_mod):
        if t_mod.dim() == 3:
            raise NotImplementedError("per-token head modulation is outside the Goal-Force path")
        x2 = _tokens2d(x)
        mod = ops.modulation(self.modulation, t_mod.contiguous(), onep_mask=0b10)
        h = ops.layernorm_modulate(x2, scale1p=mod[1], shift=mod[0], eps=self.eps)
        y = ops.gemm(h, self.head.weight, self.head.bias)
        return y.view(x.shape[:-1] + (y.shape[-1],))


class WanModel(nn.Module):

    def __init__(self, dim: int, in_dim: int, ffn_dim: int, out_dim: int, text_dim: int, freq_dim: int, eps: float,
                 patch_size: Tuple[int, int, int], num_heads: int, num_layers: int, has_image_input: bool,
                 has_image_pos_emb: bool = False, has_ref_conv: bool = False, add_control_adapter: bool = False,
                 in_dim_control_adapter: int = 24, seperated_timestep: bool = False,
                 require_vae_embedding: bool = True, require_clip_embedding: bool = True,
                 fuse_vae_embedding_in_latents: bool = False):
        super().__init__()
        if has_image_input or has_ref_conv or add_control_adapter or seperated_timestep:
            raise NotImplementedError("only the Wan2.2-I2V-A14B configuration (DIT:703-718) is built")
        if tuple(patch_size) != (1, 2, 2):
            raise NotImplementedError("patch_size must be (1,2,2)")
        self.dim, self.in_dim, self.freq_dim, self.out_dim = dim, in_dim, freq_dim, out_dim
        self.has_image_input = has_image_input
        self.patch_size = tuple(patch_size)
        self.seperated_timestep = seperated_timestep
        self.require_vae_embedding = require_vae_embedding
        self.require_clip_embedding = require_clip_embedding
        self.fuse_vae_embedding_in_latents = fuse_vae_embedding_in_latents
        self.num_heads = num_heads
        self.eps = eps
        self.patch_embedding = nn.Conv3d(in_dim, dim, kernel_size=patch_size, stride=patch_size)
        self.text_embedding = nn.Sequential(nn.Linear(text_dim, dim), nn.GELU(approximate="tanh"), nn.Linear(dim, dim))
        self.time_embedding = nn.Sequential(nn.Linear(freq_dim, dim), nn.SiLU(), nn.Linear(dim, dim))
        self.time_projection = nn.Sequential(nn.SiLU(), nn.Linear(dim, dim * 6))
        self.blocks = nn.ModuleList([DiTBlock(has_image_input, dim, num_heads, ffn_dim, eps) for _ in range(num_layers)])
        self.head = Head(dim, out_dim, patch_size, eps)
        self.freqs = precompute_freqs_cis_3d(dim // num_heads)
        self.control_adapter = None
        self._rope_cache = {}
        self._patch_w, self._patch_w_key = None, None

    def rope_table(self, f, h, w, device) -> RopeTable:
        key = (f, h, w, str(device))
        if key not in self._rope_cache:
            self._rope_cache[key] = RopeTable.from_grid(self.freqs, f, h, w, device)
        return self._rope_cache[key]

    def rope_table_shard(self, f, h, w, device, sp) -> RopeTable:
        key = (f, h, w, str(device), "sp", sp.rank, sp.size)
        if key not in self._rope_cache:
            self._rope_cache[key] = sp.shard_rope(self.rope_table(f, h, w, device))
        return self._rope_cache[key]

    def time_embed(self, timestep: torch.Tensor):
        e = sinusoidal_embedding_1d(self.freq_dim, timestep)
        te = self.time_embedding
        t = ops.gemm(ops.gemm(e, te[0].weight, te[0].bias, epilogue=ops.EPI_BIAS_SILU), te[2].weight, te[2].bias)
        tp = self.time_projection[1]
        t_mod = ops.gemm(ops.act(t, "silu"), tp.weight, tp.bias).unflatten(1, (6, self.dim))
        return t, t_mod

    def embed_text(self, context: torch.Tensor):
        te = self.text_embedding
        c2 = _tokens2d(context)
        y = ops.gemm(ops.gemm(c2, te[0].weight, te[0].bias, epilogue=ops.EPI_BIAS_GELU_TANH), te[2].weight, te[2].bias)
        return y.view(context.shape[:-1] + (self.dim,))

    @staticmethod
    def padded_patch_weight(conv: nn.Conv3d) -> torch.Tensor:
        w = conv.weight
        k = w.shape[1] * 4
        kpad = -(-k // 64) * 64
        wp = torch.zeros((w.shape[0], kpad), dtype=w.dtype, device=w.device)
        wp[:, :k] = w.reshape(w.shape[0], k)
        return wp

    def patchify(self, x: torch.Tensor, control_camera_latents_input: Optional[torch.Tensor] = None, extra=None):
        if control_camera_latents_input is not None:
            raise NotImplementedError("camera control adapter is outside the Goal-Force path")
        if x.shape[0] != 1:
            raise GoalForceError("patchify takes batch 1")
        if self._patch_w is None or self._patch_w_key != param_key(self.patch_embedding.weight):
            self._patch_w = self.padded_patch_weight(self.patch_embedding)
            self._patch_w_key = param_key(self.patch_embedding.weight)
        s0 = x[0].contiguous()
        s1 = None if extra is None else extra[0].contiguous()
        f, hh, ww = s0.shape[1], s0.shape[2] // 2, s0.shape[3] // 2
        cols = ops.patchify_im2col(s0, s1, kpad=self._patch_w.shape[1])
        tok = ops.gemm(cols, self._patch_w, self.patch_embedding.bias)
        return tok.unsqueeze(0), (f, hh, ww)

    def unpatchify(self, x: torch.Tensor, grid_size):
        f, h, w = grid_size
        return ops.unpatchify(_tokens2d(x).contiguous(), self.out_dim, f, h, w).unsqueeze(0)

    def _load_from_state_dict(self, *args, **kwargs):
        self._patch_w = None
        return super()._load_from_state_dict(*args, **kwargs)

    def forward(self, x, timestep, context, clip_feature=None, y=None, **kwargs):
        from .model_fn import model_fn_wan_video
        return model_fn_wan_video(self, latents=x, timestep=timestep, context=context, clip_feature=clip_feature, y=y)

    @staticmethod
    def state_dict_converter():
        raise NotImplementedError("checkpoint key conversion is host-side I/O outside the hot path (SURVEY §2 #9)")


A14B_CONFIG = dict(has_image_input=False, patch_size=(1, 2, 2), in_dim=36, dim=5120, ffn_dim=13824, freq_dim=256,
                   text_dim=4096, out_dim=16, num_heads=40, num_layers=40, eps=1e-6,
                   require_clip_embedding=False)
```

### goal_force_amd/ops.py

```python
from __future__ import annotations

import math

import torch

from . import _lib
from ._lib import (EPI_BIAS, EPI_BIAS_GATE_RESID, EPI_BIAS_GELU_TANH, EPI_BIAS_MUL, EPI_BIAS_RESID, EPI_BIAS_SILU,
                   GoalForceError)

__all__ = [
    "modulation", "layernorm_modulate", "rmsnorm_rope", "gate_residual", "gemm", "flash_attn", "flash_attn_sparse", "BlockMap", "patchify_im2col", "unpatchify",
    "cfg_euler_step", "act", "add", "sub", "rel_l1", "force_map",
    "EPI_BIAS", "EPI_BIAS_GELU_TANH", "EPI_BIAS_GATE_RESID", "EPI_BIAS_RESID", "EPI_BIAS_SILU", "EPI_BIAS_MUL",
]

_BF16 = torch.bfloat16
_FP8 = torch.float8_e4m3fn

PROFILE_ATTN = None
PROFILE_GEMM = None
PROFILE_CONV = None


def _stream(t: torch.Tensor):
    if t.device.index != torch.cuda.current_device():
        raise GoalForceError(f"tensor lives on cuda:{t.device.index} but the current device is cuda:"
                             f"{torch.cuda.current_device()}: call torch.cuda.set_device (one process per GPU)")
    return torch.cuda.current_stream(t.device).cuda_stream


def _ptr(t):
    return None if t is None else t.data_ptr()


def _req(t: torch.Tensor, name: str, dtype=_BF16):
    if not t.is_cuda:
        raise GoalForceError(f"{name}: tensor must be on the GPU (no CPU fallback exists)")
    if t.dtype != dtype:
        raise GoalForceError(f"{name}: expected dtype {dtype}, got {t.dtype}")


def _rows2d(t: torch.Tensor, name: str):
    if t.stride(-1) != 1:
        raise GoalForceError(f"{name}: last dim must be contiguous")
    if t.dim() == 1:
        return t, 1, t.shape[0], t.shape[0]
    v = t.reshape(-1, t.shape[-1]) if t.is_contiguous() else t
    if v.dim() != 2:
        raise GoalForceError(f"{name}: cannot view as [rows, dim] without a copy")
    return v, v.shape[0], v.shape[1], v.stride(0)


def _vec(t, name: str, n: int, dtype=_BF16, required=False):
    if t is None:
        if required:
            raise GoalForceError(f"{name}: required")
        return
    _req(t, name, dtype)
    if t.numel() != n or not t.is_contiguous():
        raise GoalForceError(f"{name}: expected contiguous [{n}]")


def _mat(t: torch.Tensor, name: str, dtype=_BF16):
    _req(t, name, dtype)
    if t.dim() != 2 or t.stride(1) != 1:
        raise GoalForceError(f"{name}: expected 2-D with contiguous rows, got {tuple(t.shape)}")


def _weight(w: torch.Tensor, name: str, K: int, dtype=_BF16):
    _mat(w, name, dtype)
    if w.shape[1] != K:
        raise GoalForceError(f"{name}: expected [N, {K}] with contiguous rows, got {tuple(w.shape)}")
    return w.shape[0], w.stride(0)


def _out(out, name: str, rows: int, cols: int, device):
    if out is None:
        return torch.empty((rows, cols), dtype=_BF16, device=device)
    _mat(out, name)
    if tuple(out.shape) != (rows, cols):
        raise GoalForceError(f"{name}: expected [{rows}, {cols}], got {tuple(out.shape)}")
    return out


def _flat(op: str, **tensors):
    n = next(iter(tensors.values())).numel()
    for name, t in tensors.items():
        if t is None:
            continue
        _req(t, f"{op}.{name}")
        if not t.is_contiguous() or t.numel() != n:
            raise GoalForceError(f"{op}: {' / '.join(tensors)} must be contiguous and equal-sized")
    return n


def kv_pad(skv: int) -> int:
    return -(-skv // 64) * 64


class _timed:
    __slots__ = ("prof", "what", "e0")

    def __init__(self, prof, *what):
        self.prof, self.what = prof, what

    def __enter__(self):
        if self.prof is not None:
            self.e0 = torch.cuda.Event(enable_timing=True)
            self.e0.record()

    def __exit__(self, exc_type, *exc):
        if self.prof is not None and exc_type is None:
            e1 = torch.cuda.Event(enable_timing=True)
            e1.record()
            self.prof.append((self.e0, e1) + self.what)
        return False


def _linear_operands(a, w, scale):
    if scale is None:
        _req(a, "linear: activation")
        av, M, K, lda = _rows2d(a, "linear: activation")
        N, ldw = _weight(w, "linear: weight", K)
    else:
        _mat(a, "fp8 linear: activation", _FP8)
        av, (M, K), lda = a, a.shape, a.stride(0)
        N, ldw = _weight(w, "fp8 linear: weight", K, _FP8)
        _vec(scale, "fp8 linear: row scale", M, torch.float32)
    return av, M, K, lda, N, ldw


def modulation(param, t, onep_mask: int):
    _req(param, "modulation.param")
    _req(t, "modulation.t")
    dim = param.shape[-1]
    k = param.numel() // dim
    t_rows = t.numel() // dim
    if not param.is_contiguous() or not t.is_contiguous() or t.shape[-1] != dim:
        raise GoalForceError("modulation: param/t must be contiguous with equal last dim")
    out = torch.empty((k, dim), dtype=_BF16, device=param.device)
    _lib.check(_lib.load().gf_modulation(_ptr(param), _ptr(t), _ptr(out), k, dim, t_rows, int(onep_mask),
                                         _stream(param)), "gf_modulation")
    return out


def layernorm_modulate(x, weight=None, bias=None, scale1p=None, shift=None, eps=1e-6, out=None):
    _req(x, "layernorm_modulate.x")
    xv, rows, dim, xs = _rows2d(x, "layernorm_modulate.x")
    if out is None:
        out = torch.empty(x.shape, dtype=_BF16, device=x.device)
    ov, _, _, os_ = _rows2d(out, "layernorm_modulate.out")
    _vec(weight, "layernorm_modulate.weight", dim)
    _vec(bias, "layernorm_modulate.bias", dim)
    _vec(scale1p, "layernorm_modulate.scale1p", dim)
    _vec(shift, "layernorm_modulate.shift", dim)
    _lib.check(_lib.load().gf_layernorm_modulate(_ptr(xv), _ptr(ov), _ptr(weight), _ptr(bias), _ptr(scale1p),
                                                 _ptr(shift), rows, dim, xs, os_, float(eps), _stream(x)),
               "gf_layernorm_modulate")
    return out


def rmsnorm_rope(x, weight, cos=None, sin=None, head_dim=128, eps=1e-6):
    _req(x, "rmsnorm_rope.x")
    _req(weight, "rmsnorm_rope.weight")
    xv, rows, dim, xs = _rows2d(x, "rmsnorm_rope.x")
    if cos is not None:
        _req(cos, "rmsnorm_rope.cos", torch.float32)
        _req(sin, "rmsnorm_rope.sin", torch.float32)
        if cos.shape != (rows, head_dim // 2) or sin.shape != cos.shape or not cos.is_contiguous() \
                or not sin.is_contiguous():
            raise GoalForceError(f"rmsnorm_rope: cos/sin must be contiguous [{rows}, {head_dim // 2}]")
    _lib.check(_lib.load().gf_rmsnorm_rope(_ptr(xv), _ptr(weight), _ptr(cos), _ptr(sin), rows, dim, head_dim, xs,
                                           float(eps), _stream(x)), "gf_rmsnorm_rope")
    return x


def modulate(x, shift, scale):
    _req(x, "modulate.x")
    xv, rows, dim, xs = _rows2d(x, "modulate.x")
    _vec(shift, "modulate.shift", dim, required=True)
    _vec(scale, "modulate.scale", dim, required=True)
    out = torch.empty(x.shape, dtype=_BF16, device=x.device)
    ov, _, _, os_ = _rows2d(out, "modulate.out")
    _lib.check(_lib.load().gf_modulate(_ptr(xv), _ptr(ov), _ptr(scale), _ptr(shift), rows, dim, xs, os_, _stream(x)), "gf_modulate")
    return out


def gate_residual(x, gate, residual):
    _req(x, "gate_residual.x")
    _req(residual, "gate_residual.residual")
    xv, rows, dim, xs = _rows2d(x, "gate_residual.x")
    rv, rrows, rdim, rs = _rows2d(residual, "gate_residual.residual")
    if (rrows, rdim) != (rows, dim):
        raise GoalForceError(f"gate_residual: residual must match x [{rows}, {dim}]")
    _vec(gate, "gate_residual.gate", dim, required=True)
    out = torch.empty(x.shape, dtype=_BF16, device=x.device)
    ov, _, _, os_ = _rows2d(out, "gate_residual.out")
    _lib.check(_lib.load().gf_gate_residual(_ptr(xv), _ptr(gate), _ptr(rv), _ptr(ov), rows, dim, xs, rs, os_, _stream(x)),
               "gf_gate_residual")
    return out


def rope_apply(x, cos, sin, head_dim):
    _req(x, "rope_apply.x")
    xv, rows, dim, xs = _rows2d(x, "rope_apply.x")
    for n, t in (("cos", cos), ("sin", sin)):
        _req(t, f"rope_apply.{n}", torch.float32)
        if tuple(t.shape) != (rows, head_dim // 2) or not t.is_contiguous():
            raise GoalForceError(f"rope_apply.{n}: expected contiguous [{rows}, {head_dim // 2}] fp32")
    out = torch.empty(x.shape, dtype=_BF16, device=x.device)
    ov, _, _, os_ = _rows2d(out, "rope_apply.out")
    _lib.check(_lib.load().gf_rope_apply(_ptr(xv), _ptr(ov), _ptr(cos), _ptr(sin), rows, dim, head_dim, xs, os_, _stream(x)),
               "gf_rope_apply")
    return out


def _gemm(a, w, row_scale, bias, epilogue, resid, gate, out):
    av, M, K, lda, N, ldw = _linear_operands(a, w, row_scale)
    if out is None:
        out = torch.empty(a.shape[:-1] + (N,), dtype=_BF16, device=a.device)
    ov, Mo, No, ldc = _rows2d(out, "gemm[_fp8].out")
    if (Mo, No) != (M, N):
        raise GoalForceError(f"gemm[_fp8].out: expected [{M}, {N}], got [{Mo}, {No}]")
    ldr = 0
    if resid is not None:
        _req(resid, "gemm[_fp8].resid")
        resid, Mr, Nr, ldr = _rows2d(resid, "gemm[_fp8].resid")
        if (Mr, Nr) != (M, N):
            raise GoalForceError(f"gemm[_fp8].resid: expected [{M}, {N}], got [{Mr}, {Nr}]")
    _vec(gate, "gemm[_fp8].gate", N)
    _vec(bias, "gemm[_fp8].bias", N)
    lib = _lib.load()
    fn, scale = (lib.gf_gemm_bf16, ()) if row_scale is None else (lib.gf_gemm_fp8, (_ptr(row_scale),))
    with _timed(PROFILE_GEMM, M, N, K, int(epilogue)):
        _lib.check(fn(_ptr(av), lda, _ptr(w), ldw, *scale, _ptr(bias), _ptr(ov), ldc, M, N, K, int(epilogue), _ptr(resid), ldr,
                      _ptr(gate), _stream(a)), fn.__name__)
    return out


def gemm(a, w, bias=None, epilogue=EPI_BIAS, resid=None, gate=None, out=None):
    return _gemm(a, w, None, bias, epilogue, resid, gate, out)


VT_MIN_KV = 2048
_LIB_DEFAULTS = {"prefer_8wave": 0, "a4_stagger": 2, "a4_group_m": 0, "conv_nb": 0, "conv_gather": 0, "conv_direct": 1, "vae_rms3": 1}
_OPT = {"attn_k3": True, "vt_from_gemm": True, "conv_padded": True, "fold_pad_keys": True, "attn_q_prescale": True, "vae_attn_offset": True,
        "fold_cross_o": True}


def lib_option(name: str) -> int:
    import ctypes
    v = ctypes.c_int(0)
    _lib.check(_lib.load().gf_get_option(name.encode(), ctypes.byref(v)), f"gf_get_option({name})")
    return int(v.value)


class options:

    def __init__(self, **kv):
        for k in kv:
            if k not in _OPT and k not in _LIB_DEFAULTS:
                raise GoalForceError(f"ops.options: unknown option {k!r}")
        self.kv, self.old = kv, {}

    @staticmethod
    def _apply_one(k, v):
        if k in _OPT:
            _OPT[k] = bool(v)
        else:
            _lib.check(_lib.load().gf_set_option(k.encode(), int(v)), f"gf_set_option({k})")

    def __enter__(self):
        self.old = {}
        try:
            for k, v in self.kv.items():
                old = _OPT[k] if k in _OPT else lib_option(k)
                self._apply_one(k, v)
                self.old[k] = old
        except BaseException:
            self.__exit__(None, None, None)
            raise
        return self

    def __exit__(self, *exc):
        for k, v in reversed(list(self.old.items())):
            self._apply_one(k, v)
        self.old = {}
        return False


_VT_WS = {}


def _vt_workspace(numel, device):
    key = (device.index, torch.cuda.current_stream(device).cuda_stream)
    ws = _VT_WS.get(key)
    if ws is None or ws.numel() < numel:
        ws = _VT_WS[key] = torch.empty((numel,), dtype=_BF16, device=device)
    return ws


def _vt_shape(skv, num_heads, head_dim):
    return skv >= VT_MIN_KV and head_dim == 128 and num_heads * 128 * kv_pad(skv) < 2 ** 31


def vt32_ok(skv, num_heads, head_dim):
    return _vt_shape(skv, num_heads, head_dim) and _OPT["attn_k3"] and _OPT["vt_from_gemm"]


def _linear_vt32(x, w, x_scale, bias):
    xv, skv, K, ldx, N, ldw = _linear_operands(x, w, x_scale)
    _vec(bias, "linear_vt32[_fp8].bias", N)
    vt = _vt_workspace(N * kv_pad(skv), x.device)
    lib = _lib.load()
    fn, scale = (lib.gf_linear_vt32, ()) if x_scale is None else (lib.gf_linear_vt32_fp8, (_ptr(x_scale),))
    _lib.check(fn(_ptr(xv), ldx, *scale, _ptr(w), ldw, _ptr(bias), _ptr(vt), skv, kv_pad(skv), N, K, _stream(x)), fn.__name__)
    return vt


def linear_vt32(x, weight, bias):
    return _linear_vt32(x, weight, None, bias)


def linear_vt32_fp8(x8, x_scale, w8, bias):
    if x_scale is None:
        raise GoalForceError("linear_vt32_fp8.x_scale: required")
    return _linear_vt32(x8, w8, x_scale, bias)


def _vt_attn(lib, q, k, v, vt, out, lse, sq, skv, num_heads, head_dim, scale, k3, block_map=None):
    tr, fa = (lib.gf_transpose_v32, lib.gf_flash_attn_fwd_vt32) if k3 else (lib.gf_transpose_v, lib.gf_flash_attn_fwd_vt)
    tiles = ()
    if block_map is not None:
        fa = lib.gf_flash_attn_fwd_vt32_sparse
        tiles = (_ptr(block_map.row_ptr), _ptr(block_map.tile_idx), _ptr(block_map.head_map), block_map.n_maps)
    if vt is None:
        vt = _vt_workspace(num_heads * 128 * kv_pad(skv), q.device)
        _lib.check(tr(_ptr(v), v.stride(0), _ptr(vt), skv, kv_pad(skv), num_heads, _stream(q)), "gf_transpose_v")
    _lib.check(fa(_ptr(q), _ptr(k), _ptr(vt), _ptr(out), _ptr(lse), *tiles, sq, skv, kv_pad(skv), num_heads, head_dim,
                  q.stride(0), k.stride(0), out.stride(0), float(scale), _stream(q)), fa.__name__ if tiles else "gf_flash_attn_fwd_vt")


def flash_attn(q, k, v, num_heads, out=None, scale=None, vt=None, last_key_mult=1, finished_q=False):
    for n, t in (("q", q), ("k", k)) + ((("v", v),) if vt is None else ()):
        _mat(t, f"flash_attn.{n}")
    sq, hd_all = q.shape
    skv = k.shape[0]
    head_dim = hd_all // num_heads
    if k.shape[1] != hd_all or (vt is None and v.shape != k.shape) or head_dim * num_heads != hd_all:
        raise GoalForceError("flash_attn: q/k/v shape mismatch")
    if vt is not None and not vt32_ok(skv, num_heads, head_dim):
        raise GoalForceError("flash_attn: a pre-transposed V is only taken by kernel 3 (key length >= VT_MIN_KV, head_dim 128)")
    if out is None:
        out = torch.empty((sq, hd_all), dtype=_BF16, device=q.device)
    if scale is None:
        scale = 1.0 / math.sqrt(head_dim)
    if last_key_mult != 1 and (vt is not None or skv >= VT_MIN_KV):
        raise GoalForceError("flash_attn: last_key_mult is for short key sequences (the text context), not the V^T path")
    long_keys = _vt_shape(skv, num_heads, head_dim)
    if finished_q and vt is not None:
        raise GoalForceError("flash_attn: finished_q goes to kernel 2, which does not take kernel 3's V^T operand")
    if vt is not None and vt.numel() < num_heads * 128 * kv_pad(skv):
        raise GoalForceError("flash_attn.vt: buffer smaller than heads*128*kv_pad")
    lib = _lib.load()
    with _timed(PROFILE_ATTN, sq, skv, num_heads):
        if long_keys:
            _vt_attn(lib, q, k, v, vt, out, None, sq, skv, num_heads, head_dim, scale, _OPT["attn_k3"] and not finished_q)
        elif last_key_mult != 1:
            _lib.check(lib.gf_flash_attn_fwd_lastmult(_ptr(q), _ptr(k), _ptr(v), _ptr(out), sq, skv, num_heads, head_dim, q.stride(0),
                                                      k.stride(0), v.stride(0), out.stride(0), float(scale), float(last_key_mult),
                                                      _stream(q)), "gf_flash_attn_fwd_lastmult")
        else:
            _lib.check(lib.gf_flash_attn_fwd(_ptr(q), _ptr(k), _ptr(v), _ptr(out), sq, skv, num_heads, head_dim,
                                             q.stride(0), k.stride(0), v.stride(0), out.stride(0), float(scale),
                                             _stream(q)), "gf_flash_attn_fwd")
    return out


SPARSE_QB, SPARSE_KB = 256, 64


class BlockMap:

    def __init__(self, mask, head_map=None, device=None):
        mask = torch.as_tensor(mask)
        if mask.is_cuda or mask.dtype != torch.bool:
            raise GoalForceError(f"BlockMap.mask: expected a CPU bool array, got {mask.dtype} on {mask.device}")
        if mask.dim() == 2:
            mask = mask[None]
        if mask.dim() != 3 or min(mask.shape) < 1:
            raise GoalForceError(f"BlockMap.mask: expected [n_maps, n_qblocks, n_tiles], got {tuple(mask.shape)}")
        self.n_maps, self.n_qblocks, self.n_tiles = mask.shape
        if self.n_tiles < 2:
            raise GoalForceError(f"BlockMap.mask: expected at least 2 key tiles, got {self.n_tiles}")
        counts = mask.sum(dim=2).reshape(-1)
        if int(counts.min()) < 2:
            m, b = divmod(int(counts.argmin()), self.n_qblocks)
            raise GoalForceError(f"BlockMap.mask: expected at least 2 tiles in every row, got {int(counts.min())} in map {m}, query block {b}")
        if head_map is not None:
            head_map = torch.as_tensor(head_map).to(torch.int64).reshape(-1)
            if head_map.numel() < 1 or int(head_map.min()) < 0 or int(head_map.max()) >= self.n_maps:
                raise GoalForceError(f"BlockMap.head_map: expected map numbers in [0, {self.n_maps}), got {head_map.tolist()}")
            head_map = head_map.to(torch.int32).contiguous()
        row_ptr = torch.zeros(counts.numel() + 1, dtype=torch.int64)
        row_ptr[1:] = counts.cumsum(0)
        self.row_ptr = row_ptr.to(torch.int32)
        self.tile_idx = mask.reshape(-1, self.n_tiles).nonzero()[:, 1].to(torch.int32).contiguous()
        self.head_map = head_map
        per_map = counts.reshape(self.n_maps, -1).sum(1).double() / (self.n_qblocks * self.n_tiles)
        self.density = float(per_map.mean() if head_map is None else per_map[head_map.long()].mean())
        self.q_len = ((self.n_qblocks - 1) * SPARSE_QB + 1, self.n_qblocks * SPARSE_QB)
        self.kv_len = ((self.n_tiles - 1) * SPARSE_KB + 1, self.n_tiles * SPARSE_KB)
        if device is not None:
            self._upload(torch.device(device))

    def _upload(self, device):
        self.row_ptr, self.tile_idx = self.row_ptr.to(device), self.tile_idx.to(device)
        if self.head_map is not None:
            self.head_map = self.head_map.to(device)

    @property
    def device(self):
        return self.row_ptr.device

    def to(self, device):
        device = torch.device(device)
        if device.type == "cuda" and device.index is None:
            device = torch.device("cuda", torch.cuda.current_device())
        if device == self.device:
            return self
        copies = self.__dict__.setdefault("_copies", {})
        if device not in copies:
            other = object.__new__(BlockMap)
            other.__dict__.update({k: v for k, v in self.__dict__.items() if k != "_copies"})
            other._upload(device)
            copies[device] = other
        return copies[device]

    def counts(self):
        rp = self.row_ptr.cpu().long()
        return (rp[1:] - rp[:-1]).reshape(self.n_maps, self.n_qblocks)

    def mask(self):
        rows = torch.repeat_interleave(torch.arange(self.n_maps * self.n_qblocks), self.counts().reshape(-1))
        m = torch.zeros((self.n_maps * self.n_qblocks, self.n_tiles), dtype=torch.bool)
        m[rows, self.tile_idx.cpu().long()] = True
        return m.reshape(self.n_maps, self.n_qblocks, self.n_tiles)


def flash_attn_sparse(q, k, v, num_heads, block_map, out=None, scale=None, vt=None, lse=False):
    for n, t in (("q", q), ("k", k)) + ((("v", v),) if vt is None else ()):
        _mat(t, f"flash_attn_sparse.{n}")
    sq, hd_all = q.shape
    skv = k.shape[0]
    if hd_all != num_heads * 128 or k.shape[1] != hd_all or (vt is None and v.shape != k.shape):
        raise GoalForceError(f"flash_attn_sparse: expected q [Sq, {num_heads}*128] and k / v [Skv, {num_heads}*128], got "
                             f"{tuple(q.shape)} / {tuple(k.shape)}")
    if skv < 2 * SPARSE_KB or sq < 1:
        raise GoalForceError(f"flash_attn_sparse: expected at least 1 query and {2 * SPARSE_KB} keys, got {sq} / {skv}")
    if num_heads * 128 * kv_pad(skv) >= 2 ** 31:
        raise GoalForceError("flash_attn_sparse: expected heads*128*kv_pad below 2^31 elements (the V^T operand's indices)")
    if not isinstance(block_map, BlockMap):
        raise GoalForceError(f"flash_attn_sparse.block_map: expected an ops.BlockMap, got {type(block_map).__name__}")
    if block_map.device != q.device:
        raise GoalForceError(f"flash_attn_sparse.block_map: expected the map on {q.device}, got {block_map.device} (BlockMap.to)")
    if (block_map.n_qblocks, block_map.n_tiles) != (-(-sq // SPARSE_QB), -(-skv // SPARSE_KB)):
        raise GoalForceError(f"flash_attn_sparse.block_map: expected [{-(-sq // SPARSE_QB)} query blocks, {-(-skv // SPARSE_KB)} tiles] for "
                             f"{sq} queries and {skv} keys, got [{block_map.n_qblocks}, {block_map.n_tiles}]")
    if block_map.head_map is not None and block_map.head_map.numel() != num_heads:
        raise GoalForceError(f"flash_attn_sparse.block_map: expected a head_map of [{num_heads}], got [{block_map.head_map.numel()}]")
    if vt is not None and vt.numel() < num_heads * 128 * kv_pad(skv):
        raise GoalForceError("flash_attn_sparse.vt: buffer smaller than heads*128*kv_pad")
    out = _out(out, "flash_attn_sparse.out", sq, hd_all, q.device)
    if scale is None:
        scale = 1.0 / math.sqrt(128)
    lse_t = torch.empty((sq, num_heads), dtype=torch.float32, device=q.device) if lse else None
    with _timed(PROFILE_ATTN, sq, max(1, round(skv * block_map.density)), num_heads):
        _vt_attn(_lib.load(), q, k, v, vt, out, lse_t, sq, skv, num_heads, 128, scale, True, block_map)
    return (out, lse_t) if lse else out


SAGE_T, SAGE_TAU, SAGE_E = 128, 0, 8
SAGE_QBLK, SAGE_KBLK = 32, 64
_SAGE_WS = {}
_SAGE_SCRATCH_PER_HEAD = 64 * 128 * 8


def _sage_rows(t, name, num_heads):
    _mat(t, name)
    if t.shape[1] != num_heads * 128:
        raise GoalForceError(f"{name}: {t.shape[1]} columns for {num_heads} heads: the sage backend is built for head_dim 128")
    if t.shape[0] < 1:
        raise GoalForceError(f"{name}: empty sequence")
    if t.stride(0) % 8 or t.data_ptr() % 16:
        raise GoalForceError(f"{name}: row stride must be a multiple of 8 elements and the data 16-byte aligned")
    return t.shape[0], t.stride(0)


def _sage_scale(scale):
    scale = 1.0 / math.sqrt(128) if scale is None else float(scale)
    if not (0.0 < scale < math.inf):
        raise GoalForceError(f"sage attention: the softmax scale must be positive and finite, got {scale}")
    return scale


def _sage_scratch(num_heads, device):
    return torch.empty((num_heads * _SAGE_SCRATCH_PER_HEAD,), dtype=torch.uint8, device=device)


def sage_k_mean(k, num_heads):
    skv, ldk = _sage_rows(k, "sage_k_mean.k", num_heads)
    mu = torch.empty((num_heads, 128), dtype=torch.float32, device=k.device)
    _lib.check(_lib.load().gf_sage_k_mean(_ptr(k), ldk, _ptr(mu), _ptr(_sage_scratch(num_heads, k.device)), skv, num_heads, _stream(k)),
               "gf_sage_k_mean")
    return mu


def sage_quant_q(q, num_heads):
    sq, ldq = _sage_rows(q, "sage_quant_q.q", num_heads)
    q8 = torch.empty((sq, num_heads * 128), dtype=torch.int8, device=q.device)
    sc = torch.empty((num_heads, -(-sq // SAGE_QBLK)), dtype=torch.float32, device=q.device)
    _lib.check(_lib.load().gf_sage_quant_q(_ptr(q), ldq, _ptr(q8), _ptr(sc), sq, num_heads, _stream(q)), "gf_sage_quant_q")
    return q8, sc


def sage_quant_k(k, num_heads, mu=None):
    skv, ldk = _sage_rows(k, "sage_quant_k.k", num_heads)
    if mu is None:
        mu = sage_k_mean(k, num_heads)
    _vec(mu, "sage_quant_k.mu", num_heads * 128, torch.float32)
    kv_pad8 = -(-skv // SAGE_T) * SAGE_T
    k8 = torch.empty((kv_pad8, num_heads * 128), dtype=torch.int8, device=k.device)
    sc = torch.empty((num_heads, kv_pad8 // SAGE_KBLK), dtype=torch.float32, device=k.device)
    _lib.check(_lib.load().gf_sage_quant_k(_ptr(k), ldk, _ptr(mu), _ptr(k8), _ptr(sc), skv, num_heads, _stream(k)), "gf_sage_quant_k")
    return k8, sc, mu


def sage_quant_vt(v, num_heads, vt=None, kv_len=None):
    if vt is None:
        skv, ldv = _sage_rows(v, "sage_quant_vt.v", num_heads)
        src, vt_in = v, 0
    else:
        _req(vt, "sage_quant_vt.vt")
        if kv_len is None or kv_len < 1:
            raise GoalForceError("sage_quant_vt: a V^T input needs kv_len")
        skv, ldv, src, vt_in = kv_len, kv_pad(kv_len), vt, 1
        if vt.numel() < num_heads * 128 * ldv:
            raise GoalForceError("sage_quant_vt.vt: buffer smaller than heads*128*kv_pad")
    kv_pad8 = -(-skv // SAGE_T) * SAGE_T
    vt8 = torch.empty((num_heads * 128, kv_pad8), dtype=torch.uint8, device=src.device)
    sc = torch.empty((num_heads, 128), dtype=torch.float32, device=src.device)
    _lib.check(_lib.load().gf_sage_quant_vt(_ptr(src), ldv, vt_in, _ptr(vt8), _ptr(sc), _ptr(_sage_scratch(num_heads, src.device)), skv,
                                            num_heads, _stream(src)), "gf_sage_quant_vt")
    return vt8, sc


def sage_attn_quantized(q8, q_scale, k8, k_scale, vt8, v_scale, kv_len, num_heads, scale=None, out=None):
    sq = q8.shape[0]
    scale = _sage_scale(scale)
    if out is None:
        out = torch.empty((sq, num_heads * 128), dtype=_BF16, device=q8.device)
    _lib.check(_lib.load().gf_sage_attn_fwd(_ptr(q8), _ptr(q_scale), _ptr(k8), _ptr(k_scale), _ptr(vt8), _ptr(v_scale), _ptr(out),
                                            out.stride(0), sq, kv_len, num_heads, scale, _stream(q8)), "gf_sage_attn_fwd")
    return out


def sage_attn(q, k, v, num_heads, scale=None, vt=None, out=None):
    scale = _sage_scale(scale)
    sq, ldq = _sage_rows(q, "sage_attn.q", num_heads)
    skv, ldk = _sage_rows(k, "sage_attn.k", num_heads)
    if vt is None:
        sv, ldv = _sage_rows(v, "sage_attn.v", num_heads)
        if sv != skv:
            raise GoalForceError(f"sage_attn: k has {skv} keys, v {sv}")
        src, vt_in = v, 0
    else:
        _req(vt, "sage_attn.vt")
        ldv, src, vt_in = kv_pad(skv), vt, 1
        if vt.numel() < num_heads * 128 * ldv:
            raise GoalForceError("sage_attn.vt: buffer smaller than heads*128*kv_pad")
    out = _out(out, "sage_attn.out", sq, num_heads * 128, q.device)
    if out.stride(0) % 8:
        raise GoalForceError("sage_attn.out: row stride must be a multiple of 8 elements")
    lib = _lib.load()
    nbytes = int(lib.gf_sage_workspace_bytes(sq, skv, num_heads))
    key = (q.device.index, torch.cuda.current_stream(q.device).cuda_stream)
    ws = _SAGE_WS.get(key)
    if ws is None or ws.numel() < nbytes:
        ws = _SAGE_WS[key] = torch.empty((nbytes,), dtype=torch.uint8, device=q.device)
    with _timed(PROFILE_ATTN, sq, skv, num_heads):
        _lib.check(lib.gf_sage_attn(_ptr(q), ldq, _ptr(k), ldk, _ptr(src), ldv, vt_in, _ptr(out), out.stride(0), sq, skv, num_heads,
                                    scale, _ptr(ws), _stream(q)), "gf_sage_attn")
    return out


CROSS_FOLD_MAX_KEYS = 63


def cross_probs(q, k, num_heads, n_pad, last_key_mult=1, scale=None, out=None):
    _mat(q, "cross_probs.q")
    _mat(k, "cross_probs.k")
    sq, hd_all = q.shape
    n_keys = k.shape[0]
    head_dim = hd_all // num_heads
    if k.shape[1] != hd_all or head_dim * num_heads != hd_all:
        raise GoalForceError("cross_probs: q/k shape mismatch")
    out = _out(out, "cross_probs.out", sq, num_heads * n_pad, q.device)
    if scale is None:
        scale = 1.0 / math.sqrt(head_dim)
    _lib.check(_lib.load().gf_cross_probs(_ptr(q), _ptr(k), _ptr(out), sq, n_keys, n_pad, num_heads, head_dim, q.stride(0), k.stride(0),
                                          out.stride(0), float(scale), float(last_key_mult), _stream(q)), "gf_cross_probs")
    return out


def cross_fold_table(v, w_o, num_heads, n_pad):
    _mat(v, "cross_fold_table.v")
    n_keys, hd_all = v.shape
    N, ldw = _weight(w_o, "cross_fold_table.w_o", hd_all)
    if hd_all % num_heads:
        raise GoalForceError(f"cross_fold_table: {hd_all} columns do not divide into {num_heads} heads")
    u = torch.empty((N, num_heads * n_pad), dtype=_BF16, device=v.device)
    _lib.check(_lib.load().gf_cross_fold_table(_ptr(v), _ptr(w_o), _ptr(u), n_keys, n_pad, num_heads, hd_all // num_heads, N, v.stride(0),
                                               ldw, u.stride(0), _stream(v)), "gf_cross_fold_table")
    return u


def flash_attn_lse(q, k, v, num_heads, scale=None):
    for n, t in (("q", q), ("k", k), ("v", v)):
        _mat(t, f"flash_attn_lse.{n}")
    sq, hd_all = q.shape
    skv = k.shape[0]
    head_dim = hd_all // num_heads
    if k.shape[1] != hd_all or v.shape != k.shape or head_dim * num_heads != hd_all:
        raise GoalForceError("flash_attn_lse: q/k/v shape mismatch")
    if scale is None:
        scale = 1.0 / math.sqrt(head_dim)
    out = torch.empty((sq, hd_all), dtype=_BF16, device=q.device)
    lse = torch.empty((sq, num_heads), dtype=torch.float32, device=q.device)
    lib = _lib.load()
    if _vt_shape(skv, num_heads, head_dim):
        _vt_attn(lib, q, k, v, None, out, lse, sq, skv, num_heads, head_dim, scale, _OPT["attn_k3"])
        return out, lse
    _lib.check(lib.gf_flash_attn_fwd_lse(_ptr(q), _ptr(k), _ptr(v), _ptr(out), _ptr(lse), sq, skv, num_heads, head_dim,
                                         q.stride(0), k.stride(0), v.stride(0), out.stride(0), float(scale),
                                         _stream(q)), "gf_flash_attn_fwd_lse")
    return out, lse


def flash_attn_bwd(q, k, v, o, dout, lse, num_heads, scale=None, need_dkv=True):
    for n, t in (("q", q), ("k", k), ("v", v), ("o", o), ("dout", dout)):
        _mat(t, f"flash_attn_bwd.{n}")
    sq, hd_all = q.shape
    skv = k.shape[0]
    head_dim = hd_all // num_heads
    if scale is None:
        scale = 1.0 / math.sqrt(head_dim)
    if lse.dtype != torch.float32 or tuple(lse.shape) != (sq, num_heads) or not lse.is_contiguous():
        raise GoalForceError("flash_attn_bwd.lse: expected contiguous fp32 [Sq, heads]")
    dq = torch.empty_like(q, memory_format=torch.contiguous_format)
    dk = torch.empty((skv, hd_all), dtype=_BF16, device=q.device) if need_dkv else None
    dv = torch.empty((skv, hd_all), dtype=_BF16, device=q.device) if need_dkv else None
    lib = _lib.load()
    ws = torch.empty((int(lib.gf_flash_attn_bwd_workspace_bytes(sq, skv, num_heads)),), dtype=torch.uint8, device=q.device)
    _lib.check(lib.gf_flash_attn_bwd(_ptr(q), _ptr(k), _ptr(v), _ptr(o), _ptr(dout), _ptr(lse), _ptr(ws), _ptr(dq),
                                             _ptr(dk) if need_dkv else None, _ptr(dv) if need_dkv else None, sq, skv, num_heads, head_dim,
                                             q.stride(0), k.stride(0), v.stride(0), o.stride(0), dout.stride(0), dq.stride(0),
                                             dk.stride(0) if need_dkv else hd_all, dv.stride(0) if need_dkv else hd_all, float(scale),
                                             _stream(q)), "gf_flash_attn_bwd")
    return dq, dk, dv


def patchify_im2col(src0, src1=None, kpad=None):
    _req(src0, "patchify.src0")
    if src0.dim() != 4 or not src0.is_contiguous():
        raise GoalForceError("patchify.src0: expected contiguous [c,F,H,W]")
    c0, F, H, W = src0.shape
    c1 = 0
    if src1 is not None:
        _req(src1, "patchify.src1")
        if src1.dim() != 4 or not src1.is_contiguous() or src1.shape[1:] != src0.shape[1:]:
            raise GoalForceError("patchify.src1: expected contiguous [c1,F,H,W] matching src0")
        c1 = src1.shape[0]
    if kpad is None:
        kpad = -(-((c0 + c1) * 4) // 64) * 64
    out = torch.empty((F * (H // 2) * (W // 2), kpad), dtype=_BF16, device=src0.device)
    _lib.check(_lib.load().gf_patchify_im2col(_ptr(src0), c0, _ptr(src1), c1, _ptr(out), F, H, W, kpad,
                                              _stream(src0)), "gf_patchify_im2col")
    return out


def unpatchify(tokens, c, f, h, w):
    _req(tokens, "unpatchify.tokens")
    if tokens.shape != (f * h * w, 4 * c) or not tokens.is_contiguous():
        raise GoalForceError(f"unpatchify.tokens: expected contiguous [{f * h * w}, {4 * c}]")
    out = torch.empty((c, f, 2 * h, 2 * w), dtype=_BF16, device=tokens.device)
    _lib.check(_lib.load().gf_unpatchify(_ptr(tokens), _ptr(out), c, f, h, w, _stream(tokens)), "gf_unpatchify")
    return out


def cfg_euler_step(latents, posi, nega, cfg_scale, dsigma):
    if posi is None:
        raise GoalForceError("cfg_euler_step.posi: required")
    n = _flat("cfg_euler_step", latents=latents, posi=posi, nega=nega)
    _lib.check(_lib.load().gf_cfg_euler_step(_ptr(latents), _ptr(posi), _ptr(nega), float(cfg_scale), float(dsigma), n,
                                             _stream(latents)), "gf_cfg_euler_step")
    return latents


def act(x, kind: str):
    n = _flat("act", x=x)
    out = torch.empty_like(x)
    _lib.check(_lib.load().gf_act(_ptr(x), _ptr(out), n, {"silu": 0, "gelu_tanh": 1}[kind], _stream(x)), "gf_act")
    return out


def add(a, b, out=None):
    n = _flat("add", a=a, b=b)
    if out is None:
        out = torch.empty_like(a)
    _lib.check(_lib.load().gf_add_bf16(_ptr(a), _ptr(b), _ptr(out), n, _stream(a)), "gf_add_bf16")
    return out


def sub(a, b, out=None):
    n = _flat("sub", a=a, b=b, out=out)
    if out is None:
        out = torch.empty_like(a)
    _lib.check(_lib.load().gf_sub_bf16(_ptr(a), _ptr(b), _ptr(out), n, _stream(a)), "gf_sub_bf16")
    return out


def rel_l1(cur, prev):
    n = _flat("rel_l1", cur=cur, prev=prev)
    if n == 0 or n % 8:
        raise GoalForceError(f"rel_l1: the element count must be a positive multiple of 8, got {n}")
    sums = torch.empty(2, dtype=torch.float32, device=cur.device)
    _lib.check(_lib.load().gf_rel_l1_bf16(_ptr(cur), _ptr(prev), n, _ptr(sums), _stream(cur)), "gf_rel_l1_bf16")
    s_diff, s_prev = sums.tolist()
    return s_diff, s_prev


def force_map(frames, H, W, channels, params, centers, clamp01, device):
    out = torch.empty((frames, H, W, 3), dtype=_BF16, device=device)
    n = int(channels.numel())
    if n:
        _req(channels, "force_map.channels", torch.int32)
        _req(params, "force_map.params", torch.float32)
        _req(centers, "force_map.centers", torch.float32)
        if params.shape != (n, 2) or centers.shape != (n, frames, 2) or not params.is_contiguous() \
                or not centers.is_contiguous():
            raise GoalForceError("force_map: params [n,2] / centers [n,frames,2] expected")
    _lib.check(_lib.load().gf_force_map(_ptr(out), frames, H, W, _ptr(channels) if n else None,
                                        _ptr(params) if n else None, _ptr(centers) if n else None, n,
                                        1 if clamp01 else 0, _stream(out)), "gf_force_map")
    return out


def vae_prep_latent(z_slice, mean, inv_std, cpad=64):
    _req(z_slice, "vae_prep_latent.z")
    _req(mean, "vae_prep_latent.mean")
    _req(inv_std, "vae_prep_latent.inv_std")
    C, T, H, W = z_slice.shape
    out = torch.empty((T, H, W, cpad), dtype=_BF16, device=z_slice.device)
    sc, st, sy, sx = z_slice.stride()
    _lib.check(_lib.load().gf_vae_prep_latent(_ptr(z_slice), sc, st, sy, sx, _ptr(mean), _ptr(inv_std), _ptr(out), C, T,
                                              H, W, cpad, _stream(z_slice)), "gf_vae_prep_latent")
    return out


def _conv_window(op, src, cache, upsample2x, downsample2, t_stride, t_off, t_out):
    _req(src, f"{op}.src")
    if src.dim() != 4 or not src.is_contiguous():
        raise GoalForceError(f"{op}.src must be contiguous [T,H,W,C]")
    T, H, W, C = src.shape
    if cache is not None:
        _req(cache, f"{op}.cache")
        if tuple(cache.shape) != (2, H, W, C) or not cache.is_contiguous():
            raise GoalForceError(f"{op}.cache must be contiguous [2,{H},{W},{C}]")
    mode = 1 if upsample2x else (2 if downsample2 else 0)
    if t_out is None:
        t_out = (T - t_off + t_stride - 1) // t_stride
    if t_off + (t_out - 1) * t_stride >= T:
        raise GoalForceError(f"{op}: temporal window exceeds the source")
    return mode, t_out, H * W * 4 if mode == 1 else ((H // 2) * (W // 2) if mode == 2 else H * W)


def _conv_resid(op, rows, bias, resid):
    if bias is not None:
        _req(bias, f"{op}.bias")
    if resid is None:
        return 0
    _mat(resid, f"{op}.resid")
    if resid.shape[0] != rows:
        raise GoalForceError(f"{op}.resid must be [{rows}, >= N] with contiguous rows")
    return resid.stride(0)


def vae_im2col(src, cache, kt, ks, kpad, upsample2x=False, downsample2=False, t_stride=1, t_off=0, t_out=None):
    mode, t_out, px = _conv_window("vae_im2col", src, cache, upsample2x, downsample2, t_stride, t_off, t_out)
    T, H, W, C = src.shape
    out = torch.empty((t_out * px, kpad), dtype=_BF16, device=src.device)
    _lib.check(_lib.load().gf_vae_im2col(_ptr(src), _ptr(cache), _ptr(out), t_out, H, W, C, kt, ks, mode, t_stride, t_off,
                                         kpad, _stream(src)), "gf_vae_im2col")
    return out


def vae_conv3d(src, cache, w, bias, kt, ks, upsample2x=False, downsample2=False, t_stride=1, t_off=0, t_out=None,
               resid=None, out=None, history_in_front=False):
    mode, t_out, px = _conv_window("vae_conv3d", src, cache, upsample2x, downsample2, t_stride, t_off, t_out)
    T, H, W, C = src.shape
    if kt == 3:
        if history_in_front:
            if cache is not None or src.storage_offset() < 2 * H * W * C:
                raise GoalForceError("vae_conv3d: history_in_front needs cache=None and src = buffer[2:] of a [2+T,H,W,C] buffer")
        elif cache is None:
            raise GoalForceError("vae_conv3d: a temporal kernel needs its 2-frame cache (or history_in_front)")
    _mat(w, "vae_conv3d.w")
    n, k = w.shape
    out = _out(out, "vae_conv3d.out", t_out * px, n, src.device)
    ldr = _conv_resid("vae_conv3d", t_out * px, bias, resid)
    with _timed(PROFILE_CONV, t_out * px, n, C, kt, ks, mode, resid is not None):
        _lib.check(_lib.load().gf_conv3d_bf16(_ptr(src), _ptr(cache), _ptr(w), w.stride(0), _ptr(bias), _ptr(out), out.stride(0),
                                              T, t_out, H, W, C, kt, ks, mode, t_stride, t_off, n, k,
                                              EPI_BIAS if resid is None else EPI_BIAS_RESID, _ptr(resid), ldr, _stream(src)),
                   "gf_conv3d_bf16")
    return out


PADDED_CONV_CHANNELS = (192, 384)


def padded_conv_fits(T, H, W, C, history=True):
    rows = (T + (2 if history else 0)) * (H + 2) * (W + 2)
    return C in PADDED_CONV_CHANNELS and rows * C * 2 < (1 << 32) and rows < (1 << 31)


def padded_activation(T, H, W, C, device, history=True):
    h = 2 if history else 0
    buf = torch.zeros((T + h, H + 2, W + 2, C), dtype=_BF16, device=device)
    return buf, (buf[:2, 1:H + 1, 1:W + 1] if history else None), buf[h:, 1:H + 1, 1:W + 1]


def vae_upsample2x_padded(x, buf):
    _req(x, "vae_upsample2x_padded.x")
    _req(buf, "vae_upsample2x_padded.buf")
    T, H, W, C = x.shape
    if not x.is_contiguous() or not buf.is_contiguous() or tuple(buf.shape) != (T, 2 * H + 2, 2 * W + 2, C):
        raise GoalForceError("vae_upsample2x_padded: x [T,H,W,C] contiguous, buf [T,2H+2,2W+2,C] contiguous")
    _lib.check(_lib.load().gf_vae_upsample2x_padded(_ptr(x), buf[0, 1, 1].data_ptr(), T, H, W, C, _stream(x)), "gf_vae_upsample2x_padded")
    return buf[:, 1:2 * H + 1, 1:2 * W + 1]


def vae_rmsnorm_silu_padded(x, gamma, buf, silu=True):
    _req(x, "vae_rmsnorm_silu_padded.x")
    _req(gamma, "vae_rmsnorm_silu_padded.gamma")
    _req(buf, "vae_rmsnorm_silu_padded.buf")
    T, H, W, C = x.shape
    if not x.is_contiguous() or not buf.is_contiguous() or tuple(buf.shape) != (T + 2, H + 2, W + 2, C) or gamma.numel() != C:
        raise GoalForceError("vae_rmsnorm_silu_padded: x [T,H,W,C] contiguous, buf [T+2,H+2,W+2,C] contiguous")
    interior = buf[2, 1, 1]
    _lib.check(_lib.load().gf_vae_rmsnorm_silu_padded(_ptr(x), _ptr(gamma), interior.data_ptr(), T, H, W, C, 1 if silu else 0, _stream(x)),
               "gf_vae_rmsnorm_silu_padded")
    return buf[2:, 1:H + 1, 1:W + 1]


def vae_conv3d_padded(buf, w, bias, resid=None, out=None, kt=3):
    _req(buf, "vae_conv3d_padded.buf")
    if buf.dim() != 4 or not buf.is_contiguous() or kt not in (1, 3):
        raise GoalForceError("vae_conv3d_padded.buf must be contiguous [kt-1+T, H+2, W+2, C], kt = 1 or 3")
    T, H, W, C = buf.shape[0] - (kt - 1), buf.shape[1] - 2, buf.shape[2] - 2, buf.shape[3]
    _mat(w, "vae_conv3d_padded.w")
    n = w.shape[0]
    if w.shape[1] < 9 * kt * C:
        raise GoalForceError("vae_conv3d_padded.w must be [N, >= 9 kt C] with contiguous rows")
    out = _out(out, "vae_conv3d_padded.out", T * H * W, n, buf.device)
    ldr = _conv_resid("vae_conv3d_padded", T * H * W, bias, resid)
    with _timed(PROFILE_CONV, T * H * W, n, C, kt, 3, 3, resid is not None):
        _lib.check(_lib.load().gf_conv3d_padded_bf16(_ptr(buf), _ptr(w), w.stride(0), _ptr(bias), _ptr(out), out.stride(0), T, H, W, C, n,
                                                     kt, EPI_BIAS if resid is None else EPI_BIAS_RESID, _ptr(resid), ldr, _stream(buf)),
                   "gf_conv3d_padded_bf16")
    return out


def vae_finish_latent(x, mean, inv_std, C):
    _mat(x, "vae_finish_latent.x")
    out = torch.empty((x.shape[0], C), dtype=_BF16, device=x.device)
    _lib.check(_lib.load().gf_vae_finish_latent(_ptr(x), x.stride(0), _ptr(mean), _ptr(inv_std), _ptr(out), x.shape[0], C,
                                                _stream(x)), "gf_vae_finish_latent")
    return out


def vae_rmsnorm_silu(x, gamma, silu=True, out=None):
    _req(x, "vae_rmsnorm_silu.x")
    _req(gamma, "vae_rmsnorm_silu.gamma")
    if not x.is_contiguous() or gamma.numel() != x.shape[-1]:
        raise GoalForceError("vae_rmsnorm_silu: x must be contiguous and gamma match the channel dim")
    if out is None:
        out = torch.empty_like(x)
    else:
        _req(out, "vae_rmsnorm_silu.out")
        if out.shape != x.shape or not out.is_contiguous():
            raise GoalForceError("vae_rmsnorm_silu.out must be contiguous with the shape of x")
    C = x.shape[-1]
    _lib.check(_lib.load().gf_vae_rmsnorm_silu(_ptr(x), _ptr(gamma), _ptr(out), x.numel() // C, C, 1 if silu else 0,
                                               _stream(x)), "gf_vae_rmsnorm_silu")
    return out


def softmax_rows(x, scale, ldo, bias=None, nvalid=None):
    _mat(x, "softmax_rows.x")
    ldb = 0
    if bias is not None:
        _mat(bias, "softmax_rows.bias")
        if bias.shape != x.shape:
            raise GoalForceError("softmax_rows.bias must match x")
        ldb = bias.stride(0)
    out = torch.empty((x.shape[0], ldo), dtype=_BF16, device=x.device)
    _lib.check(_lib.load().gf_softmax_rows(_ptr(x), x.stride(0), _ptr(bias), ldb, _ptr(out), ldo, x.shape[0], x.shape[1],
                                           x.shape[1] if nvalid is None else int(nvalid), float(scale), _stream(x)),
               "gf_softmax_rows")
    return out


def rowmax_neg(x, out_col):
    _mat(x, "rowmax_neg.x")
    _req(out_col, "rowmax_neg.out_col")
    if out_col.dim() != 1 or out_col.shape[0] != x.shape[0]:
# ... 215 lines not shown
```

### include/goalforce.h

```cpp
#ifndef GOALFORCE_H
#define GOALFORCE_H

#include <stdint.h>

#if defined(GF_BUILD)
#define GF_API __attribute__((visibility("default")))
#else
#define GF_API
#endif

#ifdef __cplusplus
extern "C" {
#endif

typedef enum {
    GF_OK = 0,
    GF_ERR_INVALID_ARG = -1,
    GF_ERR_UNSUPPORTED = -2,
    GF_ERR_LAUNCH = -3
} gf_status;

GF_API const char* gf_version(void);
GF_API const char* gf_last_error(void);
#define GF_ABI_VERSION 20
GF_API int gf_abi_version(void);
GF_API int gf_set_option(const char* name, int value);
GF_API int gf_get_option(const char* name, int* value);
GF_API void gf_reset_options(void);

GF_API int gf_layernorm_modulate(const void* x, void* out, const void* weight, const void* bias,
                          const void* scale1p, const void* shift,
                          int64_t rows, int64_t dim, int64_t x_stride, int64_t out_stride,
                          float eps, void* stream);

GF_API int gf_modulation(const void* param, const void* t, void* out, int64_t k, int64_t dim,
                         int64_t t_rows, uint32_t onep_mask, void* stream);

GF_API int gf_rmsnorm_rope(void* x, const void* weight, const float* cos_tab, const float* sin_tab,
                    int64_t rows, int64_t dim, int64_t head_dim, int64_t x_stride,
                    float eps, void* stream);

typedef enum {
    GF_EPI_BIAS = 0,
    GF_EPI_BIAS_GELU_TANH = 1,
    GF_EPI_BIAS_GATE_RESID = 2,
    GF_EPI_BIAS_RESID = 3,
    GF_EPI_BIAS_SILU = 4,
    GF_EPI_BIAS_MUL = 5
} gf_epilogue;

GF_API int gf_gemm_bf16(const void* A, int64_t lda, const void* W, int64_t ldw, const void* bias,
                 void* C, int64_t ldc, int64_t M, int64_t N, int64_t K,
                 int epilogue, const void* resid, int64_t ldr, const void* gate,
                 void* stream);

GF_API int gf_gemm_bf16_batched(const void* A, int64_t lda, int64_t strideA, const void* W, int64_t ldw, int64_t strideW, void* C,
                                int64_t ldc, int64_t strideC, int64_t M, int64_t N, int64_t K, int64_t batch, void* stream);

GF_API int gf_flash_attn_fwd(const void* q, const void* k, const void* v, void* o,
                      int64_t q_len, int64_t kv_len, int64_t heads, int64_t head_dim,
                      int64_t q_stride, int64_t k_stride, int64_t v_stride, int64_t o_stride,
                      float scale, void* stream);

GF_API int gf_transpose_v(const void* v, int64_t v_stride, void* vt, int64_t kv_len, int64_t kv_pad, int64_t heads, void* stream);
GF_API int gf_flash_attn_fwd_vt(const void* q, const void* k, const void* vt, void* o, float* lse,
                         int64_t q_len, int64_t kv_len, int64_t kv_pad, int64_t heads, int64_t head_dim,
                         int64_t q_stride, int64_t k_stride, int64_t o_stride, float scale, void* stream);

GF_API int gf_transpose_v32(const void* v, int64_t v_stride, void* vt, int64_t kv_len, int64_t kv_pad, int64_t heads, void* stream);
GF_API int gf_flash_attn_fwd_vt32(const void* q, const void* k, const void* vt, void* o, float* lse,
                                  int64_t q_len, int64_t kv_len, int64_t kv_pad, int64_t heads, int64_t head_dim,
                                  int64_t q_stride, int64_t k_stride, int64_t o_stride, float scale, void* stream);

GF_API int gf_flash_attn_fwd_vt32_sparse(const void* q, const void* k, const void* vt, void* o, float* lse,
                                         const int32_t* row_ptr, const int32_t* tile_idx, const int32_t* head_map, int64_t n_maps,
                                         int64_t q_len, int64_t kv_len, int64_t kv_pad, int64_t heads, int64_t head_dim,
                                         int64_t q_stride, int64_t k_stride, int64_t o_stride, float scale, void* stream);

GF_API int gf_linear_vt32(const void* x, int64_t ldx, const void* w, int64_t ldw, const void* bias, void* vt,
                          int64_t kv_len, int64_t kv_pad, int64_t N, int64_t K, void* stream);

GF_API int gf_flash_attn_fwd_lastmult(const void* q, const void* k, const void* v, void* o, int64_t q_len, int64_t kv_len,
                                      int64_t heads, int64_t head_dim, int64_t q_stride, int64_t k_stride, int64_t v_stride,
                                      int64_t o_stride, float scale, float last_key_multiplicity, void* stream);

GF_API int gf_cross_probs(const void* q, const void* k, void* p, int64_t q_len, int64_t n_keys, int64_t n_pad, int64_t heads,
                          int64_t head_dim, int64_t q_stride, int64_t k_stride, int64_t p_stride, float scale,
                          float last_key_multiplicity, void* stream);

GF_API int gf_cross_fold_table(const void* v, const void* w_o, void* u, int64_t n_keys, int64_t n_pad, int64_t heads, int64_t head_dim,
                               int64_t n_out, int64_t v_stride, int64_t w_stride, int64_t u_stride, void* stream);

GF_API int gf_flash_attn_fwd_lse(const void* q, const void* k, const void* v, void* o, float* lse,
                          int64_t q_len, int64_t kv_len, int64_t heads, int64_t head_dim,
                          int64_t q_stride, int64_t k_stride, int64_t v_stride, int64_t o_stride,
                          float scale, void* stream);
GF_API int64_t gf_flash_attn_bwd_workspace_bytes(int64_t q_len, int64_t kv_len, int64_t heads);
GF_API int gf_flash_attn_bwd(const void* q, const void* k, const void* v, const void* o, const void* dout,
                      const float* lse, void* workspace, void* dq, void* dk, void* dv,
                      int64_t q_len, int64_t kv_len, int64_t heads, int64_t head_dim,
                      int64_t q_stride, int64_t k_stride, int64_t v_stride, int64_t o_stride, int64_t do_stride,
                      int64_t dq_stride, int64_t dk_stride, int64_t dv_stride, float scale, void* stream);

GF_API int gf_layernorm_bwd(const void* x, int64_t x_stride, const void* dy, int64_t dy_stride, const void* g, void* dx,
                            int64_t dx_stride, float* dg_acc, float* db_acc, int64_t rows, int64_t dim, float eps, void* stream);
GF_API int gf_rmsnorm_rope_bwd(const void* x, int64_t x_stride, const void* dy, int64_t dy_stride, const void* weight,
                               const float* cos_tab, const float* sin_tab, void* dx, int64_t dx_stride, float* dw_acc,
                               int64_t rows, int64_t dim, int64_t head_dim, float eps, void* stream);
GF_API int gf_colsum(const void* a, int64_t lda, const void* b, int64_t ldb, const void* gate, void* out, int64_t ldo,
                     float* acc, int64_t rows, int64_t cols, void* stream);
GF_API int gf_act_bwd(const void* u, const void* df, void* du, int64_t n, int kind, void* stream);
GF_API int gf_mse_loss(const void* pred, const void* target, void* dpred, float* loss, int64_t n, float weight, void* stream);
GF_API int gf_adamw_step(void* param, const void* grad, float* exp_avg, float* exp_avg_sq, int64_t n, float lr, float beta1,
                         float beta2, float eps, float weight_decay, int64_t step, float grad_scale, void* stream);
GF_API int gf_f32_to_bf16(const float* src, void* dst, int64_t n, void* stream);
GF_API int gf_sumsq(const void* x, int64_t n, float* acc, void* stream);

GF_API int gf_patchify_im2col(const void* src0, int64_t c0, const void* src1, int64_t c1,
                       void* out, int64_t F, int64_t H, int64_t W, int64_t kpad, void* stream);

GF_API int gf_unpatchify(const void* tokens, void* out, int64_t c, int64_t f, int64_t h, int64_t w,
                  void* stream);

GF_API int gf_cfg_euler_step(void* latents, const void* posi, const void* nega,
                      float cfg_scale, float dsigma, int64_t n, void* stream);

GF_API int gf_act(const void* x, void* out, int64_t n, int kind, void* stream);

GF_API int gf_add_bf16(const void* a, const void* b, void* out, int64_t n, void* stream);

GF_API int gf_sub_bf16(const void* a, const void* b, void* out, int64_t n, void* stream);
GF_API int gf_rel_l1_bf16(const void* cur, const void* prev, int64_t n, void* sums, void* stream);

GF_API int gf_force_map(void* out, int64_t frames, int64_t H, int64_t W,
                 const int32_t* channels, const float* params, const float* centers,
                 int64_t n_blobs, int clamp01, void* stream);


GF_API int gf_vae_prep_latent(const void* z, int64_t sc, int64_t st, int64_t sy, int64_t sx,
                              const void* mean, const void* inv_std, void* out,
                              int64_t C, int64_t T, int64_t H, int64_t W, int64_t cpad, void* stream);

GF_API int gf_vae_im2col(const void* src, const void* cache, void* out, int64_t T_out, int64_t H, int64_t W,
                         int64_t C, int64_t kt, int64_t ks, int mode, int64_t t_stride, int64_t t_off,
                         int64_t kpad, void* stream);

GF_API int gf_conv3d_bf16(const void* src, const void* cache, const void* Wm, int64_t ldw, const void* bias,
                          void* out, int64_t ldc, int64_t T_in, int64_t T_out, int64_t H, int64_t W, int64_t C,
                          int kt, int ks, int mode, int t_stride, int t_off, int64_t N, int64_t K, int epilogue,
                          const void* resid, int64_t ldr, void* stream);

GF_API int gf_vae_finish_latent(const void* x, int64_t ldx, const void* mean, const void* inv_std, void* out,
                                int64_t rows, int64_t C, void* stream);

GF_API int gf_vae_rmsnorm_silu(const void* x, const void* gamma, void* out, int64_t rows, int64_t C,
                               int silu, void* stream);

GF_API int gf_softmax_rows(const void* x, int64_t ldx, const void* bias, int64_t ldb, void* out, int64_t ldo,
                           int64_t rows, int64_t ncols, int64_t nvalid, float scale, void* stream);

GF_API int gf_rowmax_neg_bf16(const void* x, int64_t ldx, void* out, int64_t ldo, int64_t rows, int64_t ncols, void* stream);

GF_API int gf_transpose_pad(const void* src, int64_t ld_src, void* dst, int64_t R, int64_t C, int64_t rpad,
                            void* stream);

GF_API int gf_transpose_pad_batched(const void* src, int64_t ld_src, int64_t stride_src, void* dst, int64_t stride_dst, int64_t R,
                                    int64_t C, int64_t rpad, int64_t batch, void* stream);

GF_API int gf_vae_tile_blend(void* values, void* weight, const void* tile, int64_t nch, int64_t T, int64_t th,
                             int64_t tw, int64_t tc, int64_t H, int64_t W, int64_t y0, int64_t x0,
                             int top, int bottom, int left, int right, int64_t border_h, int64_t border_w,
                             void* stream);
GF_API int gf_vae_tile_finalize(void* values, const void* weight, int64_t planes, int64_t hw, int clamp1, void* stream);

GF_API int gf_modulate(const void* x, void* out, const void* scale, const void* shift, int64_t rows, int64_t dim,
                       int64_t x_stride, int64_t out_stride, void* stream);

GF_API int gf_resize_lanczos4_u8(const void* src, void* dst, const int* xofs, const short* xcoef, const int* yofs, const short* ycoef,
                                 int64_t frames, int64_t H, int64_t W, int64_t Hd, int64_t Wd, void* stream);
GF_API int gf_resize_area_u8(const void* src, void* dst, const int* xstart, const int* xsrc, const float* xalpha, const int* ystart,
                             const int* ysrc, const float* yalpha, int64_t frames, int64_t H, int64_t W, int64_t Hd, int64_t Wd, int mode,
                             void* stream);
GF_API int gf_canny_u8(const void* img, void* state, void* mag_ws, void* dxy_ws, int* changed, int64_t frames, int64_t H, int64_t W,
                       int low, int high, int max_passes, void* stream);

GF_API int gf_gate_residual(const void* x, const void* gate, const void* residual, void* out, int64_t rows, int64_t dim,
                            int64_t x_stride, int64_t r_stride, int64_t out_stride, void* stream);

GF_API int gf_rope_apply(const void* x, void* out, const float* cos_tab, const float* sin_tab, int64_t rows, int64_t dim,
                         int64_t head_dim, int64_t x_stride, int64_t out_stride, void* stream);


GF_API int gf_quant_fp8_rowscale(const void* x, void* out8, float* scale, int64_t rows, int64_t dim,
                                 int64_t x_stride, int64_t out_stride, void* stream);

GF_API int gf_layernorm_modulate_fp8(const void* x, void* out8, float* scale, const void* weight, const void* bias,
                                     const void* scale1p, const void* shift, int64_t rows, int64_t dim,
                                     int64_t x_stride, int64_t out_stride, float eps, void* stream);

GF_API int gf_linear_vt32_fp8(const void* x8, int64_t ldx, const float* x_scale, const void* w8, int64_t ldw, const void* bias,
                              void* vt, int64_t kv_len, int64_t kv_pad, int64_t N, int64_t K, void* stream);

GF_API int gf_cast_fp8(const void* x, void* out8, int64_t n, void* stream);

GF_API int gf_gemm_fp8(const void* A8, int64_t lda, const void* W8, int64_t ldw, const float* row_scale,
                       const void* bias, void* C, int64_t ldc, int64_t M, int64_t N, int64_t K,
                       int epilogue, const void* resid, int64_t ldr, const void* gate, void* stream);

GF_API int gf_conv3d_padded_bf16(const void* xp, const void* Wm, int64_t ldw, const void* bias, void* out, int64_t ldo, int64_t T,
                                 int64_t H, int64_t W, int64_t C, int64_t N, int64_t kt, int epilogue, const void* resid, int64_t ldr,
                                 void* stream);
GF_API int gf_vae_rmsnorm_silu_padded(const void* x, const void* gamma, void* out_interior, int64_t T, int64_t H, int64_t W, int64_t C,
                                      int silu, void* stream);
GF_API int gf_vae_upsample2x_padded(const void* x, void* out_interior, int64_t T, int64_t H, int64_t W, int64_t C, void* stream);

GF_API int64_t gf_sage_workspace_bytes(int64_t q_len, int64_t kv_len, int64_t heads);
GF_API int gf_sage_k_mean(const void* k, int64_t ldk, float* mu, void* scratch, int64_t kv_len, int64_t heads, void* stream);
GF_API int gf_sage_quant_q(const void* q, int64_t ldq, void* q8, float* q_scale, int64_t q_len, int64_t heads, void* stream);
GF_API int gf_sage_quant_k(const void* k, int64_t ldk, const float* mu, void* k8, float* k_scale, int64_t kv_len, int64_t heads,
                           void* stream);
GF_API int gf_sage_quant_vt(const void* v, int64_t ldv, int vt_in, void* vt8, float* v_scale, void* scratch, int64_t kv_len,
                            int64_t heads, void* stream);
GF_API int gf_sage_attn_fwd(const void* q8, const float* q_scale, const void* k8, const float* k_scale, const void* vt8,
                            const float* v_scale, void* o, int64_t ldo, int64_t q_len, int64_t kv_len, int64_t heads, float scale,
                            void* stream);
GF_API int gf_sage_attn(const void* q, int64_t ldq, const void* k, int64_t ldk, const void* v, int64_t ldv, int vt_in, void* o,
                        int64_t ldo, int64_t q_len, int64_t kv_len, int64_t heads, float scale, void* ws, void* stream);

#ifdef __cplusplus
}
#endif
#endif
```

Measured before the change: 0.6071.

## Fuse row statistics into GEMM epilogues to skip LayerNorm and RMSNorm passes

Adds two GEMM epilogues. One is gate+residual that also emits per-row sum and sum-of-squares partials per 128-column half-tile. The other is a row-affine epilogue that applies a LayerNorm (folded into the weights) and emits sum-of-squares partials. Small finish kernels turn these partials into per-row mean/rstd and rsqrt, and the cross-attention probs kernel applies the q RMSNorm while loading q. The aim is to drop separate normalization passes over the large activation tensors around cross-attention, at the cost of extra epilogue reductions, extra small launches, and slightly different rounding from folding the norm into the GEMM.

```diff
diff --git a/goal_force_amd/csrc/gf_cross_fold.hip b/goal_force_amd/csrc/gf_cross_fold.hip
--- a/goal_force_amd/csrc/gf_cross_fold.hip
+++ b/goal_force_amd/csrc/gf_cross_fold.hip
@@ -11,9 +11,11 @@
     acc = __builtin_amdgcn_mfma_f32_32x32x16_bf16(a, b, acc, 0, 0, 0);
 }
 
+template <bool NORM>
 __global__ __launch_bounds__(CF_THREADS) void cross_probs_kernel(const u16* __restrict__ q, const u16* __restrict__ k, u16* __restrict__ pout,
                                                                  int q_len, int n_keys, int n_pad, int heads, long q_stride, long k_stride,
-                                                                 long p_stride, float c, float last_key_bias) {
+                                                                 long p_stride, float c, float last_key_bias, const float* __restrict__ rsq,
+                                                                 const u16* __restrict__ nw) {
     __shared__ __attribute__((aligned(16))) char lds[CF_MAXK * 256];
     const int tid = threadIdx.x;
     const int lane = tid & 63, wave = tid >> 6;
@@ -36,8 +38,21 @@
     {
         const int qr = min(q0 + r, q_len - 1);
         const u16* qp = q + (long)qr * q_stride + head * CF_HD + 8 * h;
-#pragma unroll
-        for (int kd = 0; kd < 8; ++kd) qf[kd] = *reinterpret_cast<const bf16x8*>(qp + 16 * kd);
+        if constexpr (NORM) {
+            const float rr = rsq[qr];
+            const u16* wp = nw + head * CF_HD + 8 * h;
+#pragma unroll
+            for (int kd = 0; kd < 8; ++kd) {
+                const u16x8 q8 = *reinterpret_cast<const u16x8*>(qp + 16 * kd), w8 = *reinterpret_cast<const u16x8*>(wp + 16 * kd);
+                u16x8 o;
+#pragma unroll
+                for (int e = 0; e < 8; ++e) o[e] = f2bf(rbf(bf2f(q8[e]) * rr) * bf2f(w8[e]));
+                qf[kd] = __builtin_bit_cast(bf16x8, o);
+            }
+        } else {
+#pragma unroll
+            for (int kd = 0; kd < 8; ++kd) qf[kd] = *reinterpret_cast<const bf16x8*>(qp + 16 * kd);
+        }
     }
     __syncthreads();
 
@@ -156,31 +171,52 @@
 
 }
 
-extern "C" GF_API int gf_cross_probs(const void* q, const void* k, void* p, int64_t q_len, int64_t n_keys, int64_t n_pad, int64_t heads,
-                                     int64_t head_dim, int64_t q_stride, int64_t k_stride, int64_t p_stride, float scale,
-                                     float last_key_multiplicity, void* stream) {
-    GF_CHECK_ARG(q && k && p, "gf_cross_probs: null pointer");
+static int cross_probs(const char* fn, bool norm, const void* q, const float* rs, const void* nw, const void* k, void* p, int64_t q_len,
+                       int64_t n_keys, int64_t n_pad, int64_t heads, int64_t head_dim, int64_t q_stride, int64_t k_stride, int64_t p_stride,
+                       float scale, float last_key_multiplicity, void* stream) {
+    GF_CHECK_ARG(q && k && p, "%s: null pointer", fn);
     if (head_dim != CF_HD) {
-        gf_set_error("gf_cross_probs: head_dim=%ld unsupported (kernel is built for 128)", (long)head_dim);
+        gf_set_error("%s: head_dim=%ld unsupported (kernel is built for 128)", fn, (long)head_dim);
         return GF_ERR_UNSUPPORTED;
     }
-    GF_CHECK_ARG(q_len >= 0 && q_len < (1 << 30) && heads > 0 && heads < 65536, "gf_cross_probs: bad sizes q=%ld heads=%ld", (long)q_len,
-                 (long)heads);
+    GF_CHECK_ARG(q_len >= 0 && q_len < (1 << 30) && heads > 0 && heads < 65536, "%s: bad sizes q=%ld heads=%ld", fn, (long)q_len, (long)heads);
     GF_CHECK_ARG(n_keys >= 1 && n_pad % 16 == 0 && n_pad > n_keys && n_pad <= CF_MAXK,
-                 "gf_cross_probs: 1 <= n_keys=%ld < n_pad=%ld <= 64, n_pad a multiple of 16", (long)n_keys, (long)n_pad);
+                 "%s: 1 <= n_keys=%ld < n_pad=%ld <= 64, n_pad a multiple of 16", fn, (long)n_keys, (long)n_pad);
     GF_CHECK_ARG(q_stride % 8 == 0 && k_stride % 8 == 0 && p_stride % 4 == 0 && q_stride >= heads * CF_HD && k_stride >= heads * CF_HD &&
                      p_stride >= heads * n_pad,
-                 "gf_cross_probs: strides must cover the rows (q, k: multiples of 8; p: of 4, >= heads * n_pad)");
-    GF_CHECK_ARG(gf_aligned16(q) && gf_aligned16(k) && ((uintptr_t)p & 7u) == 0, "gf_cross_probs: alignment (q, k 16 bytes, p 8 bytes)");
-    GF_CHECK_ARG(scale > 0.f && last_key_multiplicity >= 1.0f, "gf_cross_probs: scale > 0, multiplicity >= 1");
+                 "%s: strides must cover the rows (q, k: multiples of 8; p: of 4, >= heads * n_pad)", fn);
+    GF_CHECK_ARG(gf_aligned16(q) && gf_aligned16(k) && ((uintptr_t)p & 7u) == 0, "%s: alignment (q, k 16 bytes, p 8 bytes)", fn);
+    GF_CHECK_ARG(scale > 0.f && last_key_multiplicity >= 1.0f, "%s: scale > 0, multiplicity >= 1", fn);
+    GF_CHECK_ARG(!norm || (rs && nw && ((uintptr_t)rs & 3u) == 0 && gf_aligned16(nw)),
+                 "%s: the rows' rsqrt vector (fp32 [q_len]) and the norm weight (bf16 [heads*128], 16-byte aligned) are required", fn);
     if (q_len == 0) return GF_OK;
     const float c = scale * 1.4426950408889634f;
     const float bias = last_key_multiplicity != 1.0f ? log2f(last_key_multiplicity) / c : 0.f;
     const dim3 grid((unsigned)((q_len + CF_QB - 1) / CF_QB), (unsigned)heads);
-    hipLaunchKernelGGL(cross_probs_kernel, grid, dim3(CF_THREADS), 0, (hipStream_t)stream, (const u16*)q, (const u16*)k, (u16*)p,
-                       (int)q_len, (int)n_keys, (int)n_pad, (int)heads, (long)q_stride, (long)k_stride, (long)p_stride, c, bias);
-    GF_CHECK_LAUNCH("gf_cross_probs");
+    if (norm)
+        hipLaunchKernelGGL(cross_probs_kernel<true>, grid, dim3(CF_THREADS), 0, (hipStream_t)stream, (const u16*)q, (const u16*)k, (u16*)p,
+                           (int)q_len, (int)n_keys, (int)n_pad, (int)heads, (long)q_stride, (long)k_stride, (long)p_stride, c, bias, rs,
+                           (const u16*)nw);
+    else
+        hipLaunchKernelGGL(cross_probs_kernel<false>, grid, dim3(CF_THREADS), 0, (hipStream_t)stream, (const u16*)q, (const u16*)k, (u16*)p,
+                           (int)q_len, (int)n_keys, (int)n_pad, (int)heads, (long)q_stride, (long)k_stride, (long)p_stride, c, bias,
+                           (const float*)nullptr, (const u16*)nullptr);
+    GF_CHECK_LAUNCH(fn);
     return GF_OK;
+}
+
+extern "C" GF_API int gf_cross_probs(const void* q, const void* k, void* p, int64_t q_len, int64_t n_keys, int64_t n_pad, int64_t heads,
+                                     int64_t head_dim, int64_t q_stride, int64_t k_stride, int64_t p_stride, float scale,
+                                     float last_key_multiplicity, void* stream) {
+    return cross_probs("gf_cross_probs", false, q, nullptr, nullptr, k, p, q_len, n_keys, n_pad, heads, head_dim, q_stride, k_stride, p_stride,
+                       scale, last_key_multiplicity, stream);
+}
+
+extern "C" GF_API int gf_cross_probs_norm(const void* q, const float* row_rsqrt, const void* norm_weight, const void* k, void* p,
+                                          int64_t q_len, int64_t n_keys, int64_t n_pad, int64_t heads, int64_t head_dim, int64_t q_stride,
+                                          int64_t k_stride, int64_t p_stride, float scale, float last_key_multiplicity, void* stream) {
+    return cross_probs("gf_cross_probs_norm", true, q, row_rsqrt, norm_weight, k, p, q_len, n_keys, n_pad, heads, head_dim, q_stride, k_stride,
+                       p_stride, scale, last_key_multiplicity, stream);
 }
 
 extern "C" GF_API int gf_cross_fold_table(const void* v, const void* w_o, void* u, int64_t n_keys, int64_t n_pad, int64_t heads,
diff --git a/goal_force_amd/csrc/gf_gemm.hip b/goal_force_amd/csrc/gf_gemm.hip
--- a/goal_force_amd/csrc/gf_gemm.hip
+++ b/goal_force_amd/csrc/gf_gemm.hip
@@ -34,7 +34,7 @@
     long lda, ldw, ldc, ldr;
     long sA = 0, sW = 0, sC = 0;
     int tiles_m, tiles_n;
-    unsigned long long* rsv0 = nullptr;
+    float* stats = nullptr;
     ConvGeom cv;
     int rsv1 = 0;
     int stagger;
@@ -45,6 +45,19 @@
 };
 
 constexpr int GF_EPI_VT32 = 6;
+constexpr int GF_EPI_GATE_RESID_STATS = 7;
+constexpr int GF_EPI_BIAS_ROWAFFINE = 8;
+
+template <int CTRL>
+__device__ __forceinline__ float gf_row16_add(float v) {
+    return v + __int_as_float(__builtin_amdgcn_update_dpp(0, __float_as_int(v), CTRL, 0xf, 0xf, false));
+}
+__device__ __forceinline__ float gf_row16_sum(float v) {
+    v = gf_row16_add<0xB1>(v);
+    v = gf_row16_add<0x4E>(v);
+    v = gf_row16_add<0x141>(v);
+    return gf_row16_add<0x140>(v);
+}
 
 typedef __attribute__((ext_vector_type(8))) int i32x8;
 
@@ -598,6 +611,9 @@
     const int lane = tid & 63;
     const int wave = __builtin_amdgcn_readfirstlane(tid >> 6);
     const int wm = wave >> 1, wn = wave & 1;
+    constexpr bool STATS = EPI == GF_EPI_GATE_RESID_STATS, AFFINE = EPI == GF_EPI_BIAS_ROWAFFINE;
+    constexpr bool GATED = EPI == GF_EPI_BIAS_GATE_RESID || STATS;
+    static_assert(!FP8 || !(STATS || AFFINE), "the row-statistics epilogues are bf16 only");
 
     const int v = gf_xcd_tile_order(p.tiles_m * p.tiles_n);
     const int gm = p.group_m;
@@ -638,10 +654,10 @@
 #pragma unroll
         for (int j = 0; j < 8; ++j) {
             const int n = n0 + wn * 128 + j * 16 + fq_ * 4;
-            bpre[j] = (EPI != GF_EPI_VT32 && p.bias && n < p.N) ? *reinterpret_cast<const u16x4*>(p.bias + n) : u16x4{0, 0, 0, 0};
+            bpre[j] = (EPI != GF_EPI_VT32 && !AFFINE && p.bias && n < p.N) ? *reinterpret_cast<const u16x4*>(p.bias + n) : u16x4{0, 0, 0, 0};
         }
         const int ng = n0 + wn * 128 + (lane & 15) * 8;
-        if (EPI == GF_EPI_BIAS_GATE_RESID && ng < p.N) gpre = *reinterpret_cast<const u16x8*>(p.gate + ng);
+        if (GATED && ng < p.N) gpre = *reinterpret_cast<const u16x8*>(p.gate + ng);
         if (EPI == GF_EPI_VT32 && p.bias) {
 #pragma unroll
             for (int i = 0; i < 8; ++i) {
@@ -654,6 +670,11 @@
     if constexpr (FP8 && EPI != GF_EPI_VT32) {
 #pragma unroll
         for (int i = 0; i < 8; ++i) rsc[i] = p.row_scale[min(m0 + wm * 128 + i * 16 + (lane & 15), p.M - 1)];
+    }
+    gf_f32x2 rab[AFFINE ? 8 : 1];
+    if constexpr (AFFINE) {
+#pragma unroll
+        for (int i = 0; i < 8; ++i) rab[i] = *reinterpret_cast<const gf_f32x2*>(p.row_scale + 2 * min(m0 + wm * 128 + i * 16 + (lane & 15), p.M - 1));
     }
     if constexpr (FP8) {
         GF_A4F8_LOOP_ASM(voffA, voffB, rdA0, rdA1, rdB0, rdB1, aLo, aHi, nrA, bLo, bHi, nrB, soA, stA, soB, stB, ldsW, nk, k0, kb);
@@ -663,7 +684,7 @@
     }
 
     GF_LDS char* ep = lds + wave * 32768;
-    constexpr bool HAS_R = EPI == GF_EPI_BIAS_GATE_RESID || EPI == GF_EPI_BIAS_RESID || EPI == GF_EPI_BIAS_MUL;
+    constexpr bool HAS_R = GATED || EPI == GF_EPI_BIAS_RESID || EPI == GF_EPI_BIAS_MUL;
     u16x8 rres[HAS_R ? 32 : 1];
     if constexpr (HAS_R) {
         const int nr = n0 + wn * 128 + (lane & 15) * 8;
@@ -684,6 +705,16 @@
             const int n = n0 + wn * 128 + j * 16 + fq * 4;
 #pragma unroll
             for (int r = 0; r < 4; ++r) csc[j][r] = (n + r < p.wrows) ? p.row_scale[n + r] : 0.f;
+        }
+    }
+    f32x4 cvn[AFFINE ? 8 : 1], b32[AFFINE ? 8 : 1];
+    if constexpr (AFFINE) {
+#pragma unroll
+        for (int j = 0; j < 8; ++j) {
+            const int n = n0 + wn * 128 + j * 16 + fq * 4;
+            const bool ok = n < p.N;
+            cvn[j] = ok ? *reinterpret_cast<const f32x4*>(reinterpret_cast<const float*>(p.gate) + n) : f32x4{0.f, 0.f, 0.f, 0.f};
+            b32[j] = ok ? *reinterpret_cast<const f32x4*>(reinterpret_cast<const float*>(p.bias) + n) : f32x4{0.f, 0.f, 0.f, 0.f};
         }
     }
     gf_static_for<0, 8>([&](auto j_c) {
@@ -707,6 +738,9 @@
 #pragma unroll
                     for (int r = 0; r < 4; ++r) y[r] = (n + r < p.wrows) ? y[r] + bm : 0.f;
                 }
+            } else if constexpr (AFFINE) {
+#pragma unroll
+                for (int r = 0; r < 4; ++r) y[r] = __builtin_fmaf(y[r], rab[i][0], __builtin_fmaf(-rab[i][1], cvn[j][r], b32[j][r]));
             } else if constexpr (EPI == GF_EPI_BIAS_GELU_TANH) {
                 const unsigned l01 = FP8 ? pack2bf(y[0], y[1]) : pack2bf(y[0] + bv[0], y[1] + bv[1]);
                 const unsigned l23 = FP8 ? pack2bf(y[2], y[3]) : pack2bf(y[2] + bv[2], y[3] + bv[3]);
@@ -750,6 +784,7 @@
             } else {
                 yv = *(GF_LDS u16x8*)(ep + row * 256 + ((cc ^ (row & 15)) << 4));
             }
+            float s1 = 0.f, s2 = 0.f;
             if (m < p.M && n_ok) {
                 u16x8 o = yv;
                 if constexpr (HAS_R) {
@@ -757,12 +792,29 @@
 #pragma unroll
                     for (int e = 0; e < 8; ++e) {
                         float t = bf2f(yv[e]);
-                        if (EPI == GF_EPI_BIAS_GATE_RESID) t = rbf(bf2f(g8[e]) * t);
+                        if (GATED) t = rbf(bf2f(g8[e]) * t);
                         o[e] = (EPI == GF_EPI_BIAS_MUL) ? f2bf(t * bf2f(r8[e]))
                                                         : f2bf(bf2f(r8[e]) + t);
                     }
                 }
+                if constexpr (STATS || AFFINE) {
+#pragma unroll
+                    for (int e = 0; e < 8; ++e) {
+                        const float f = bf2f(o[e]);
+                        if constexpr (STATS) s1 += f;
+                        s2 = __builtin_fmaf(f, f, s2);
+                    }
+                }
                 __builtin_nontemporal_store(o, reinterpret_cast<u16x8*>(p.C + (long)m * p.ldc + n));
+            }
+            if constexpr (STATS || AFFINE) {
+                const int nh = p.N >> 7, ht = (n0 >> 7) + wn;
+                if constexpr (STATS) s1 = gf_row16_sum(s1);
+                s2 = gf_row16_sum(s2);
+                if (cc == 0 && m < p.M && ht < nh) {
+                    if constexpr (STATS) *reinterpret_cast<gf_f32x2*>(p.stats + ((long)m * nh + ht) * 2) = gf_f32x2{s1, s2};
+                    else p.stats[(long)m * nh + ht] = s2;
+                }
             }
         }
     }
@@ -889,6 +941,72 @@
                                   const void* bias, void* C, int64_t ldc, int64_t M, int64_t N, int64_t K, int epilogue,
                                   const void* resid, int64_t ldr, const void* gate, void* stream) {
     return gemm_dispatch(true, A8, lda, W8, ldw, row_scale, bias, C, ldc, M, N, K, epilogue, resid, ldr, gate, stream);
+}
+
+static int gemm_rowstats(const char* fn, int epi, const void* A, int64_t lda, const void* W, int64_t ldw, const void* bias, void* C,
+                         int64_t ldc, int64_t M, int64_t N, int64_t K, const void* resid, int64_t ldr, const void* gate,
+                         const float* row_ab, float* stats, int64_t stats_elems, void* stream) {
+    const int per = epi == GF_EPI_GATE_RESID_STATS ? 2 : 1;
+    GF_CHECK_ARG(A && W && C, "%s: null A/W/C", fn);
+    GF_CHECK_ARG(M >= 0 && N > 0 && K > 0, "%s: bad sizes M=%ld N=%ld K=%ld", fn, (long)M, (long)N, (long)K);
+    GF_CHECK_ARG(K % 64 == 0, "%s: K=%ld must be a multiple of 64", fn, (long)K);
+    GF_CHECK_ARG(N % 128 == 0, "%s: N=%ld must be a multiple of 128 (one table entry per 128-column half-tile)", fn, (long)N);
+    GF_CHECK_ARG(lda % 8 == 0 && ldw % 8 == 0 && ldc % 8 == 0 && lda >= K && ldw >= K && ldc >= N,
+                 "%s: leading dimensions must be multiples of 8 and cover the row", fn);
+    GF_CHECK_ARG(gf_aligned16(A) && gf_aligned16(W) && gf_aligned16(C) && (!bias || gf_aligned16(bias)), "%s: 16-byte alignment required", fn);
+    GF_CHECK_ARG(M < (1 << 30) && N < (1 << 30), "%s: M/N too large", fn);
+    GF_CHECK_ARG(stats && ((uintptr_t)stats & (per == 2 ? 7u : 3u)) == 0, "%s: the statistics table must be %d-byte aligned", fn, 4 * per);
+    GF_CHECK_ARG(stats_elems >= M * (N / 128) * per, "%s: the statistics table holds %ld floats, [M, N/128%s] needs %ld", fn, (long)stats_elems,
+                 per == 2 ? ", 2" : "", (long)(M * (N / 128) * per));
+    if (epi == GF_EPI_GATE_RESID_STATS) {
+        GF_CHECK_ARG(resid && ldr % 8 == 0 && ldr >= N && gf_aligned16(resid), "%s: residual epilogue needs an aligned resid with ldr >= N", fn);
+        GF_CHECK_ARG(gate && gf_aligned16(gate), "%s: gate epilogue needs an aligned gate vector", fn);
+    } else {
+        GF_CHECK_ARG(row_ab && ((uintptr_t)row_ab & 7u) == 0, "%s: the rows' (a, b) pairs must be 8-byte aligned", fn);
+        GF_CHECK_ARG(gate && gf_aligned16(gate) && bias, "%s: cvec and bias (fp32 [N]) are required, 16-byte aligned", fn);
+    }
+    if (M < 512 || 256L * lda * 2 + K * 2L >= (1L << 31) || 256L * ldw * 2 + K * 2L >= (1L << 31)) {
+        gf_set_error("%s: M=%ld, lda=%ld, ldw=%ld is outside the 4-wave kernel (M >= 512, 256 rows of either operand below 2^31 bytes)", fn,
+                     (long)M, (long)lda, (long)ldw);
+        return GF_ERR_UNSUPPORTED;
+    }
+    GemmArgs a;
+    a.A = (const u16*)A;
+    a.W = (const u16*)W;
+    a.bias = (const u16*)bias;
+    a.C = (u16*)C;
+    a.R = (const u16*)resid;
+    a.gate = (const u16*)gate;
+    a.row_scale = row_ab;
+    a.stats = stats;
+    a.M = (int)M;
+    a.N = (int)N;
+    a.K = (int)K;
+    a.lda = lda;
+    a.ldw = ldw;
+    a.ldc = ldc;
+    a.ldr = ldr;
+    a.tiles_m = (int)((M + BM - 1) / BM);
+    a.tiles_n = (int)((N + BN - 1) / BN);
+    a.stagger = gf_options().a4_stagger.load(std::memory_order_relaxed);
+    a.wrows = (int)N;
+    a.stagger_rows = 0;
+    return epi == GF_EPI_GATE_RESID_STATS ? launch_gemm_a4<GF_EPI_GATE_RESID_STATS>(a, (hipStream_t)stream)
+                                          : launch_gemm_a4<GF_EPI_BIAS_ROWAFFINE>(a, (hipStream_t)stream);
+}
+
+extern "C" GF_API int gf_gemm_bf16_gate_resid_stats(const void* A, int64_t lda, const void* W, int64_t ldw, const void* bias, void* C,
+                                                    int64_t ldc, int64_t M, int64_t N, int64_t K, const void* resid, int64_t ldr,
+                                                    const void* gate, float* stats, int64_t stats_elems, void* stream) {
+    return gemm_rowstats("gf_gemm_bf16_gate_resid_stats", GF_EPI_GATE_RESID_STATS, A, lda, W, ldw, bias, C, ldc, M, N, K, resid, ldr, gate,
+                         nullptr, stats, stats_elems, stream);
+}
+
+extern "C" GF_API int gf_gemm_bf16_rowaffine(const void* A, int64_t lda, const void* W, int64_t ldw, const float* row_ab, const float* cvec,
+                                             const float* bias, void* C, int64_t ldc, int64_t M, int64_t N, int64_t K, float* sumsq,
+                                             int64_t sumsq_elems, void* stream) {
+    return gemm_rowstats("gf_gemm_bf16_rowaffine", GF_EPI_BIAS_ROWAFFINE, A, lda, W, ldw, bias, C, ldc, M, N, K, nullptr, 0, cvec, row_ab, sumsq,
+                         sumsq_elems, stream);
 }
 
 extern "C" GF_API int gf_linear_vt32(const void* x, int64_t ldx, const void* w, int64_t ldw, const void* bias, void* vt,
diff --git a/goal_force_amd/csrc/gf_rowops.hip b/goal_force_amd/csrc/gf_rowops.hip
--- a/goal_force_amd/csrc/gf_rowops.hip
+++ b/goal_force_amd/csrc/gf_rowops.hip
@@ -635,3 +635,58 @@
     GF_CHECK_LAUNCH("gf_rmsnorm_rope");
     return GF_OK;
 }
+
+namespace {
+template <bool MOMENTS>
+__global__ __launch_bounds__(256) void row_stats_finish_kernel(const float* __restrict__ tab, float* __restrict__ out, long rows, int halves,
+                                                               float dim, float eps) {
+    const long row = (long)blockIdx.x * 256 + threadIdx.x;
+    if (row >= rows) return;
+    if constexpr (MOMENTS) {
+        const gf_f32x2* t = reinterpret_cast<const gf_f32x2*>(tab) + row * halves;
+        float s1 = 0.f, s2 = 0.f;
+        for (int i = 0; i < halves; ++i) {
+            const gf_f32x2 v = t[i];
+            s1 += v[0];
+            s2 += v[1];
+        }
+        const float mean = s1 / dim;
+        const float var = fmaxf(__builtin_fmaf(-mean, mean, s2 / dim), 0.f);
+        const float rstd = 1.0f / sqrtf(var + eps);
+        reinterpret_cast<gf_f32x2*>(out)[row] = gf_f32x2{rstd, mean * rstd};
+    } else {
+        const float* t = tab + row * halves;
+        float s2 = 0.f;
+        for (int i = 0; i < halves; ++i) s2 += t[i];
+        out[row] = 1.0f / sqrtf(s2 * (1.0f / dim) + eps);
+    }
+}
+
+int row_stats_finish(const char* fn, bool moments, const float* tab, float* out, int64_t rows, int64_t halves, int64_t dim, float eps,
+                     void* stream) {
+    GF_CHECK_ARG(tab && out, "%s: null pointer", fn);
+    GF_CHECK_ARG(rows >= 0 && rows < (1 << 30) && halves > 0 && halves < 65536 && dim == halves * 128,
+                 "%s: bad sizes rows=%ld halves=%ld dim=%ld (dim = 128 halves)", fn, (long)rows, (long)halves, (long)dim);
+    GF_CHECK_ARG(((uintptr_t)tab & (moments ? 7u : 3u)) == 0 && ((uintptr_t)out & (moments ? 7u : 3u)) == 0, "%s: %d-byte alignment required", fn,
+                 moments ? 8 : 4);
+    GF_CHECK_ARG(eps >= 0.f, "%s: eps must not be negative", fn);
+    if (rows == 0) return GF_OK;
+    const dim3 grid((unsigned)((rows + 255) / 256)), block(256);
+    if (moments)
+        hipLaunchKernelGGL(row_stats_finish_kernel<true>, grid, block, 0, (hipStream_t)stream, tab, out, (long)rows, (int)halves, (float)dim, eps);
+    else
+        hipLaunchKernelGGL(row_stats_finish_kernel<false>, grid, block, 0, (hipStream_t)stream, tab, out, (long)rows, (int)halves, (float)dim, eps);
+    GF_CHECK_LAUNCH(fn);
+    return GF_OK;
+}
+}
+
+extern "C" GF_API int gf_row_moments_finish(const float* stats, float* row_ab, int64_t rows, int64_t halves, int64_t dim, float eps,
+                                            void* stream) {
+    return row_stats_finish("gf_row_moments_finish", true, stats, row_ab, rows, halves, dim, eps, stream);
+}
+
+extern "C" GF_API int gf_row_rsqrt_finish(const float* sumsq, float* row_rsqrt, int64_t rows, int64_t halves, int64_t dim, float eps,
+                                          void* stream) {
+    return row_stats_finish("gf_row_rsqrt_finish", false, sumsq, row_rsqrt, rows, halves, dim, eps, stream);
+}
diff --git a/goal_force_amd/dit.py b/goal_force_amd/dit.py
--- a/goal_force_amd/dit.py
+++ b/goal_force_amd/dit.py
@@ -395,6 +395,29 @@
         self.ffn = nn.Sequential(nn.Linear(dim, ffn_dim), nn.GELU(approximate="tanh"), nn.Linear(ffn_dim, dim))
         self.modulation = nn.Parameter(torch.randn(1, 6, dim) / dim ** 0.5)
         self.gate = GateModule()
+        self._q_fold, self._q_fold_key = None, None
+
+    def q_fold(self):
+        ca, n3 = self.cross_attn, self.norm3
+        ps = (n3.weight, n3.bias, ca.q.weight) + (() if ca.q.bias is None else (ca.q.bias,))
+        key = param_key(*ps)
+        if self._q_fold is None or self._q_fold_key != key:
+            with torch.no_grad():
+                w32 = ca.q.weight.detach().float()
+                wf = (w32 * n3.weight.detach().float()[None, :]).to(torch.bfloat16).contiguous()
+                cvec = wf.float().sum(1).contiguous()
+                b = (w32 * n3.bias.detach().float()[None, :]).sum(1)
+                if ca.q.bias is not None:
+                    b = b + ca.q.bias.detach().float()
+                self._q_fold, self._q_fold_key = (wf, cvec, b.contiguous()), key
+        return self._q_fold
+
+    def row_stats_ok(self, x2, context_kv, keep, fp8) -> bool:
+        if not ops._OPT["cross_row_stats"] or keep is not None or fp8 or not x2.is_cuda:
+            return False
+        if getattr(self.cross_attn.q, "_gf_w8", None) is not None or getattr(self.self_attn.o, "_gf_w8", None) is not None:
+            return False
+        return self.cross_attn.fold_ok(context_kv) and ops.row_stats_ok(x2.shape[0], self.dim, self.dim)
 
     def forward(self, x, context, t_mod, freqs, context_kv=None, out=None, sp=None, keep=None, self_attn_memo=None,
                 fold_pad_keys=True, pad_n=None, dense_attn=False):
@@ -404,8 +427,13 @@
         rope = _as_rope(freqs, x.device)
         mod = ops.modulation(self.modulation, t_mod.contiguous(), onep_mask=0b010010)
         fp8 = getattr(self.ffn[0], "_gf_w8", None) is not None
+        if context_kv is None:
+            context_kv = self.cross_attn.context_kv(_tokens2d(context), fold=fold_pad_keys and keep is None, pad_n=pad_n)
+        stats_path = self.row_stats_ok(x2, context_kv, keep, fp8)
+        row_ab = q_memo = None
         if self_attn_memo is not None and "x" in self_attn_memo:
             x_new = self_attn_memo.pop("x")
+            row_ab, q_memo = self_attn_memo.pop("row_ab", None), self_attn_memo.pop("q", None)
             ev = self_attn_memo.pop("ev", None)
             if ev is not None:
                 torch.cuda.current_stream(x_new.device).wait_event(ev)
@@ -420,22 +448,47 @@
                 h = ops.layernorm_modulate(x2, scale1p=mod[1], shift=mod[0], eps=self.eps)
             a = self.self_attn.attend(h, rope, sp, keep, dense=dense_attn)
             x_new = out if out is not None else torch.empty_like(x2)
-            linear(a, self.self_attn.o, epilogue=ops.EPI_BIAS_GATE_RESID, resid=x2, gate=mod[2], out=x_new)
+            if stats_path:
+                o = self.self_attn.o
+                row_ab = ops.row_moments_finish(ops.gemm_gate_resid_stats(a, o.weight, o.bias, x2, mod[2], out=x_new)[1], self.eps)
+            else:
+                linear(a, self.self_attn.o, epilogue=ops.EPI_BIAS_GATE_RESID, resid=x2, gate=mod[2], out=x_new)
             if keep is not None and keep.get("wide"):
                 keep["x1"] = x_new.clone()
             if self_attn_memo is not None:
                 self_attn_memo["x"] = x_new.clone()
+                if row_ab is not None:
+                    self_attn_memo["row_ab"] = row_ab
                 if x_new.is_cuda:
                     self_attn_memo["ev"] = torch.cuda.Event()
                     self_attn_memo["ev"].record(torch.cuda.current_stream(x_new.device))
-        if fp8:
+        ca = self.cross_attn
+        stats_path = stats_path and row_ab is not None
+        if stats_path:
+            pass
+        elif fp8:
             h = QuantizedInput.layernorm(x_new, weight=self.norm3.weight, bias=self.norm3.bias, eps=self.eps)
         else:
             ops.layernorm_modulate(x_new, weight=self.norm3.weight, bias=self.norm3.bias, eps=self.eps, out=h)
-        if context_kv is None:
-            context_kv = self.cross_attn.context_kv(_tokens2d(context), fold=fold_pad_keys and keep is None, pad_n=pad_n)
-        ca = self.cross_attn
-        if keep is None and not fp8 and ca.fold_ok(context_kv):
+        if stats_path:
+            if q_memo is not None:
+                q, rsq = q_memo
+                if ev is not None:
+                    q.record_stream(torch.cuda.current_stream(q.device))
+                    rsq.record_stream(torch.cuda.current_stream(q.device))
+            else:
+                wq, cvec, bq = self.q_fold()
+                q, sumsq = ops.gemm_rowaffine(x_new, wq, row_ab, cvec, bq)
+                rsq = ops.row_rsqrt_finish(sumsq, ca.norm_q.eps)
+                if self_attn_memo is not None and "x" in self_attn_memo:
+                    self_attn_memo["q"] = (q, rsq)
+                    if "ev" in self_attn_memo:
+                        self_attn_memo["ev"].record(torch.cuda.current_stream(q.device))
+            u = context_kv[3] if len(context_kv) > 3 else ca.fold_table(context_kv)
+            p = ops.cross_probs(q, context_kv[0], ca.num_heads, ca.fold_pad(context_kv[0].shape[0]), last_key_mult=context_kv[2],
+                                row_rsqrt=rsq, norm_weight=ca.norm_q.weight)
+            ops.gemm(p, u, ca.o.bias, epilogue=ops.EPI_BIAS_RESID, resid=x_new, out=x_new)
+        elif keep is None and not fp8 and ca.fold_ok(context_kv):
             u = context_kv[3] if len(context_kv) > 3 else ca.fold_table(context_kv)
             ops.gemm(ca.attend_probs(h, context_kv), u, ca.o.bias, epilogue=ops.EPI_BIAS_RESID, resid=x_new, out=x_new)
         else:
diff --git a/goal_force_amd/ops.py b/goal_force_amd/ops.py
--- a/goal_force_amd/ops.py
+++ b/goal_force_amd/ops.py
@@ -245,7 +245,7 @@
 VT_MIN_KV = 2048
 _LIB_DEFAULTS = {"prefer_8wave": 0, "a4_stagger": 2, "a4_group_m": 0, "conv_nb": 0, "conv_gather": 0, "conv_direct": 1, "vae_rms3": 1}
 _OPT = {"attn_k3": True, "vt_from_gemm": True, "conv_padded": True, "fold_pad_keys": True, "attn_q_prescale": True, "vae_attn_offset": True,
-        "fold_cross_o": True}
+        "fold_cross_o": True, "cross_row_stats": True}
 
 
 def lib_option(name: str) -> int:
@@ -597,7 +597,7 @@
 CROSS_FOLD_MAX_KEYS = 63
 
 
-def cross_probs(q, k, num_heads, n_pad, last_key_mult=1, scale=None, out=None):
+def cross_probs(q, k, num_heads, n_pad, last_key_mult=1, scale=None, out=None, row_rsqrt=None, norm_weight=None):
     _mat(q, "cross_probs.q")
     _mat(k, "cross_probs.k")
     sq, hd_all = q.shape
@@ -608,6 +608,15 @@
     out = _out(out, "cross_probs.out", sq, num_heads * n_pad, q.device)
     if scale is None:
         scale = 1.0 / math.sqrt(head_dim)
+    if (row_rsqrt is None) != (norm_weight is None):
+        raise GoalForceError("cross_probs: row_rsqrt and norm_weight go together")
+    if row_rsqrt is not None:
+        _vec(row_rsqrt, "cross_probs.row_rsqrt", sq, torch.float32)
+        _vec(norm_weight, "cross_probs.norm_weight", hd_all)
+        _lib.check(_lib.load().gf_cross_probs_norm(_ptr(q), _ptr(row_rsqrt), _ptr(norm_weight), _ptr(k), _ptr(out), sq, n_keys, n_pad, num_heads,
+                                                   head_dim, q.stride(0), k.stride(0), out.stride(0), float(scale), float(last_key_mult),
+                                                   _stream(q)), "gf_cross_probs_norm")
+        return out
     _lib.check(_lib.load().gf_cross_probs(_ptr(q), _ptr(k), _ptr(out), sq, n_keys, n_pad, num_heads, head_dim, q.stride(0), k.stride(0),
                                           out.stride(0), float(scale), float(last_key_mult), _stream(q)), "gf_cross_probs")
     return out
@@ -623,6 +632,82 @@
     _lib.check(_lib.load().gf_cross_fold_table(_ptr(v), _ptr(w_o), _ptr(u), n_keys, n_pad, num_heads, hd_all // num_heads, N, v.stride(0),
                                                ldw, u.stride(0), _stream(v)), "gf_cross_fold_table")
     return u
+
+
+ROW_STATS_MIN_M = 512
+_F32 = torch.float32
+
+
+def row_stats_ok(M: int, N: int, K: int) -> bool:
+    return M >= ROW_STATS_MIN_M and N % 128 == 0 and K % 64 == 0 and 256 * K * 2 + K * 2 < (1 << 31)
+
+
+def _stats_table(t, name, M, N, per, device):
+    shape = (M, N // 128) + ((2,) if per == 2 else ())
+    if t is None:
+        return torch.empty(shape, dtype=_F32, device=device)
+    _req(t, name, _F32)
+    if not t.is_contiguous():
+        raise GoalForceError(f"{name}: expected a contiguous fp32 table")
+    return t
+
+
+def gemm_gate_resid_stats(a, w, bias, resid, gate, out=None, stats=None):
+    av, M, K, lda, N, ldw = _linear_operands(a, w, None)
+    if out is None:
+        out = torch.empty(a.shape[:-1] + (N,), dtype=_BF16, device=a.device)
+    ov, Mo, No, ldc = _rows2d(out, "gemm_gate_resid_stats.out")
+    _req(resid, "gemm_gate_resid_stats.resid")
+    rv, Mr, Nr, ldr = _rows2d(resid, "gemm_gate_resid_stats.resid")
+    if (Mo, No) != (M, N) or (Mr, Nr) != (M, N):
+        raise GoalForceError(f"gemm_gate_resid_stats: out / resid must be [{M}, {N}]")
+    _vec(gate, "gemm_gate_resid_stats.gate", N, required=True)
+    _vec(bias, "gemm_gate_resid_stats.bias", N)
+    stats = _stats_table(stats, "gemm_gate_resid_stats.stats", M, N, 2, a.device)
+    with _timed(PROFILE_GEMM, M, N, K, int(EPI_BIAS_GATE_RESID)):
+        _lib.check(_lib.load().gf_gemm_bf16_gate_resid_stats(_ptr(av), lda, _ptr(w), ldw, _ptr(bias), _ptr(ov), ldc, M, N, K, _ptr(rv), ldr,
+                                                             _ptr(gate), _ptr(stats), stats.numel(), _stream(a)),
+                   "gf_gemm_bf16_gate_resid_stats")
+    return out, stats
+
+
+def row_moments_finish(stats, eps=1e-6):
+    _req(stats, "row_moments_finish.stats", _F32)
+    if stats.dim() != 3 or stats.shape[2] != 2 or not stats.is_contiguous():
+        raise GoalForceError(f"row_moments_finish.stats: expected contiguous [M, halves, 2], got {tuple(stats.shape)}")
+    M, H = stats.shape[:2]
+    out = torch.empty((M, 2), dtype=_F32, device=stats.device)
+    _lib.check(_lib.load().gf_row_moments_finish(_ptr(stats), _ptr(out), M, H, 128 * H, float(eps), _stream(stats)), "gf_row_moments_finish")
+    return out
+
+
+def row_rsqrt_finish(sumsq, eps=1e-6):
+    _req(sumsq, "row_rsqrt_finish.sumsq", _F32)
+    if sumsq.dim() != 2 or not sumsq.is_contiguous():
+        raise GoalForceError(f"row_rsqrt_finish.sumsq: expected contiguous [M, halves], got {tuple(sumsq.shape)}")
+    M, H = sumsq.shape
+    out = torch.empty((M,), dtype=_F32, device=sumsq.device)
+    _lib.check(_lib.load().gf_row_rsqrt_finish(_ptr(sumsq), _ptr(out), M, H, 128 * H, float(eps), _stream(sumsq)), "gf_row_rsqrt_finish")
+    return out
+
+
+def gemm_rowaffine(a, w, row_ab, cvec, bias, out=None, sumsq=None):
+    av, M, K, lda, N, ldw = _linear_operands(a, w, None)
+    if out is None:
+        out = torch.empty(a.shape[:-1] + (N,), dtype=_BF16, device=a.device)
+    ov, Mo, No, ldc = _rows2d(out, "gemm_rowaffine.out")
+    if (Mo, No) != (M, N):
+        raise GoalForceError(f"gemm_rowaffine.out: expected [{M}, {N}], got [{Mo}, {No}]")
+    _req(row_ab, "gemm_rowaffine.row_ab", _F32)
+    if tuple(row_ab.shape) != (M, 2) or not row_ab.is_contiguous():
+        raise GoalForceError(f"gemm_rowaffine.row_ab: expected contiguous [{M}, 2], got {tuple(row_ab.shape)}")
+    _vec(cvec, "gemm_rowaffine.cvec", N, _F32, required=True)
+    _vec(bias, "gemm_rowaffine.bias", N, _F32, required=True)
+    sumsq = _stats_table(sumsq, "gemm_rowaffine.sumsq", M, N, 1, a.device)
+    with _timed(PROFILE_GEMM, M, N, K, int(EPI_BIAS)):
+        _lib.check(_lib.load().gf_gemm_bf16_rowaffine(_ptr(av), lda, _ptr(w), ldw, _ptr(row_ab), _ptr(cvec), _ptr(bias), _ptr(ov), ldc, M, N, K,
+                                                      _ptr(sumsq), sumsq.numel(), _stream(a)), "gf_gemm_bf16_rowaffine")
+    return out, sumsq
 
 
 def flash_attn_lse(q, k, v, num_heads, scale=None):
diff --git a/include/goalforce.h b/include/goalforce.h
--- a/include/goalforce.h
+++ b/include/goalforce.h
@@ -90,6 +90,18 @@
 
 GF_API int gf_cross_fold_table(const void* v, const void* w_o, void* u, int64_t n_keys, int64_t n_pad, int64_t heads, int64_t head_dim,
                                int64_t n_out, int64_t v_stride, int64_t w_stride, int64_t u_stride, void* stream);
+
+GF_API int gf_gemm_bf16_gate_resid_stats(const void* A, int64_t lda, const void* W, int64_t ldw, const void* bias, void* C, int64_t ldc,
+                                         int64_t M, int64_t N, int64_t K, const void* resid, int64_t ldr, const void* gate, float* stats,
+                                         int64_t stats_elems, void* stream);
+GF_API int gf_gemm_bf16_rowaffine(const void* A, int64_t lda, const void* W, int64_t ldw, const float* row_ab, const float* cvec,
+                                  const float* bias, void* C, int64_t ldc, int64_t M, int64_t N, int64_t K, float* sumsq,
+                                  int64_t sumsq_elems, void* stream);
+GF_API int gf_row_moments_finish(const float* stats, float* row_ab, int64_t rows, int64_t halves, int64_t dim, float eps, void* stream);
+GF_API int gf_row_rsqrt_finish(const float* sumsq, float* row_rsqrt, int64_t rows, int64_t halves, int64_t dim, float eps, void* stream);
+GF_API int gf_cross_probs_norm(const void* q, const float* row_rsqrt, const void* norm_weight, const void* k, void* p, int64_t q_len,
+                               int64_t n_keys, int64_t n_pad, int64_t heads, int64_t head_dim, int64_t q_stride, int64_t k_stride,
+                               int64_t p_stride, float scale, float last_key_multiplicity, void* stream);
 
 GF_API int gf_flash_attn_fwd_lse(const void* q, const void* k, const void* v, void* o, float* lse,
                           int64_t q_len, int64_t kv_len, int64_t heads, int64_t head_dim,
```

Result: no change. 0.6095 (median of 6 runs) (+0.4%).
